# Genomics-HSE/VGsim

Measured on AMD Instinct MI355X. Metric: simulated events/sec (direct + tau-leap) at 1/2/4/8 MI355X vs Cython CPU, higher is better.
Workload: dtype f64; 1 GPU; BASELINE config 3: 65536 haplotypes (8 sites) x 64 populations x 1 susceptibility group, direct Gillespie, bit-exact mode (PCG64 stream, reference summation order), index-case start, b=2.5 d=0.9 s=0.1 m=0.01/site, total migration 0.01, N=1e7; replicates_per_gpu=16384, events_per_replicate=100000, trajectory_points=1001

## Files before the change

include/vgx.h:

```cpp
#ifndef VGX_H
#define VGX_H
#include <stdint.h>

#ifdef __cplusplus
extern "C" {
#endif

typedef struct vgx_engine vgx_engine;

enum {
    VGX_OK = 0,
    VGX_ERR_ARG = 1,
    VGX_ERR_HIP = 2,
    VGX_ERR_ZERO_WEIGHT = 3,
    VGX_ERR_CAPACITY = 4,
    VGX_ERR_LOOP_GUARD = 5,
    VGX_ERR_CLASSES = 6
};

enum { VGX_BIRTH = 0, VGX_DEATH = 1, VGX_SAMPLING = 2, VGX_MUTATION = 3, VGX_SUSCCHANGE = 4,
       VGX_MIGRATION = 5, VGX_MULTITYPE = 6 };

typedef struct vgx_dims {
    int64_t sites, hapNum, popNum, susNum;
} vgx_dims;

typedef struct vgx_params {
    const double *bRate, *dRate, *sRate;
    const double *mRate;
    const double *hapMutType;
    const double *susceptibility;
    const int64_t *suscType;
    const double *suscepTransition;
    const int64_t *sizes;
    const double *contactDensityBeforeLockdown;
    const double *contactDensityAfterLockdown;
    const double *startLD, *endLD;
    const double *samplingMultiplier;
    const double *migrationRates;
} vgx_params;

typedef struct vgx_state {
    int64_t *susceptible;
    int64_t *infectious;
    int64_t *initial_susceptible;
    int64_t *initial_infectious;
    int64_t *totalSusceptible, *totalInfectious, *lockdownON;
    double *contactDensity;
    int64_t first_simulation;
    int64_t globalInfectious;
    int64_t bCounter, dCounter, sCounter, mCounter, iCounter, swapLockdown, migPlus, migNonPlus;
    int64_t good_attempt;
    double currentTime, totalRate, totalMigrationRate, tau_l;
    int64_t ev_ptr, ev_size;
} vgx_state;

typedef struct vgx_run_opts {
    int64_t record_events;
    int64_t max_loop_factor;
    int64_t traj_points;
    double traj_t0, traj_t1;
    int64_t mode;
    int64_t kernel;
    int64_t reserved[2];
} vgx_run_opts;

typedef struct vgx_counters {
    int64_t ev_ptr;
    int64_t ev_first_new;
    int64_t loop_iterations;
    int64_t restarts;
    int64_t lockdown_records;
    int64_t error;
    int64_t multievent_rows;
    int64_t reserved[5];
} vgx_counters;

int vgx_create(const vgx_dims *dims, int64_t n_replicates, int device, vgx_engine **out);
void vgx_destroy(vgx_engine *e);
const char *vgx_last_error(const vgx_engine *e);
int vgx_device_count(void);

int vgx_set_params(vgx_engine *e, const vgx_params *p);
int vgx_set_recombination(vgx_engine *e, double recombination_probability, int64_t genome_length,
                          const int64_t *sitesPosition );
int vgx_set_state(vgx_engine *e, const vgx_state *s);
int vgx_get_state(vgx_engine *e, int64_t replicate, vgx_state *out);
int vgx_set_seeds(vgx_engine *e, const int64_t *seeds );

int vgx_stage_tau(vgx_engine *e);

int vgx_simulate_direct(vgx_engine *e, int64_t iterations, int64_t sample_size, float time, int64_t attempts,
                        const vgx_run_opts *opts );
int vgx_simulate_tau(vgx_engine *e, int64_t iterations, int64_t sample_size, float time, int64_t attempts,
                     const vgx_run_opts *opts );

int vgx_get_counters(vgx_engine *e, int64_t replicate, vgx_counters *out);
int vgx_get_counters_all(vgx_engine *e, int64_t *out);
int vgx_get_events(vgx_engine *e, int64_t replicate, int64_t first, int64_t count, double *times,
                   int64_t *types, int64_t *haplotypes, int64_t *populations, int64_t *newHaplotypes,
                   int64_t *newPopulations);
int vgx_get_lockdowns(vgx_engine *e, int64_t replicate, int64_t cap, int64_t *states, int64_t *populations,
                      double *times, int64_t *n);
int vgx_get_recombinations(vgx_engine *e, int64_t replicate, int64_t cap, int64_t *idevents, int64_t *his,
                           int64_t *hi2s, int64_t *nhis, int64_t *posRecombs, int64_t *n);
int vgx_get_tau_tries(vgx_engine *e, int64_t replicate, int64_t first, int64_t count, int32_t *out);
int vgx_get_multievents(vgx_engine *e, int64_t replicate, int64_t cap, int64_t *num, double *times, int64_t *types,
                        int64_t *haplotypes, int64_t *populations, int64_t *newHaplotypes,
                        int64_t *newPopulations, int64_t *n);
int vgx_get_multievents_all(vgx_engine *e, int64_t cap, int64_t *offsets, int64_t *rows, int64_t *steps);
int vgx_get_tau_states_all(vgx_engine *e, int64_t *infectious, int64_t *susceptible, int64_t *counters, double *times);
int vgx_get_trajectories(vgx_engine *e, double *out, int out_is_device);
int vgx_get_trajectories_int(vgx_engine *e, int32_t *out_device);
int64_t vgx_clock_mismatches(const vgx_engine *e);

typedef struct vgx_genealogy_io {
    int64_t popNum, hapNum;
    int64_t sCounter;
    int64_t ev_ptr;
    const double *ev_times;
    const int64_t *ev_types, *ev_haplotypes, *ev_populations, *ev_newHaplotypes, *ev_newPopulations;
    int64_t mev_rows;
    const int64_t *mev_num; const double *mev_times;
    const int64_t *mev_types, *mev_haplotypes, *mev_populations, *mev_newHaplotypes, *mev_newPopulations;
    int64_t *infectious;
    uint64_t rng_state[4];
    int64_t rng_has_uint32;
    uint64_t rng_uinteger;
    int64_t *tree, *tree_pop; double *times;
    int64_t mut_cap, mut_n; int64_t *mut_node, *mut_AS, *mut_DS, *mut_site; double *mut_time;
    int64_t mig_cap, mig_n; int64_t *mig_node, *mig_old, *mig_new; double *mig_time;
    int64_t nodes_used;
} vgx_genealogy_io;
int vgx_get_genealogy(vgx_genealogy_io *io, char *errbuf, int64_t errcap);
void vgx_rng_position(int64_t seed, int64_t attempt, int64_t draws, uint64_t out[4]);

typedef struct vgx_genealogies_io {
    int64_t n;
    const int64_t *replicates;
    const uint64_t *rng_state;
    int64_t *node_off, *mut_off, *mig_off;
    int64_t *tree, *tree_pop; double *times;
    int64_t *mut_node, *mut_AS, *mut_DS, *mut_site; double *mut_time;
    int64_t *mig_node, *mig_old, *mig_new; double *mig_time;
    int64_t *status, *status_arg, *nodes_used, *mut_n, *mig_n;
    uint64_t *rng_out;
    int64_t layout;
    int64_t passes;
    double ms[3];
} vgx_genealogies_io;
int vgx_get_genealogies(vgx_engine *e, vgx_genealogies_io *io);
int vgx_genealogy_message(int64_t status, int64_t arg, char *errbuf, int64_t errcap);
int vgx_test_genealogy_walk(vgx_genealogy_io *io, char *errbuf, int64_t errcap);

typedef struct vgx_tau_genealogy_prefix {
    int64_t ev_ptr;
    const double *ev_times;
    const int64_t *ev_types, *ev_haplotypes, *ev_populations, *ev_newHaplotypes, *ev_newPopulations;
    int64_t mev_rows;
    const int64_t *mev_num; const double *mev_times;
    const int64_t *mev_types, *mev_haplotypes, *mev_populations, *mev_newHaplotypes, *mev_newPopulations;
} vgx_tau_genealogy_prefix;
typedef struct vgx_tau_genealogies_io {
    int64_t n;
    const int64_t *replicates;
    const uint64_t *rng_state;
    int64_t *node_off, *mut_off, *mig_off;
    int64_t *tree, *tree_pop; double *times;
    int64_t *mut_node, *mut_AS, *mut_DS, *mut_site; double *mut_time;
    int64_t *mig_node, *mig_old, *mig_new; double *mig_time;
    int64_t *status, *status_arg, *nodes_used, *mut_n, *mig_n;
    uint64_t *rng_out;
    int64_t passes;
    double ms[3];
} vgx_tau_genealogies_io;
int vgx_get_tau_genealogies(vgx_engine *e, vgx_tau_genealogies_io *io, const vgx_tau_genealogy_prefix *prefix);
int vgx_test_tau_genealogy_walk(vgx_genealogy_io *io, int64_t sites, char *errbuf, int64_t errcap);
int vgx_test_hypergeometric(int on_device, int64_t good, int64_t bad, int64_t sample, int64_t n, uint64_t state[6], int64_t *out);

typedef struct vgx_timelines_io {
    int64_t n;
    const int64_t *replicates;
    int64_t step_num, semantics;
    int64_t n_inf; const int64_t *inf_pop, *inf_hap;
    int64_t n_sus; const int64_t *sus_pop, *sus_grp;
    double *time_points;
    double *inf_data, *inf_sample;
    double *sus_data;
    int64_t *last_point;
    int64_t loc_cap;
    int64_t *loc_n, *loc_state, *loc_pop;
    double *loc_time;
    int64_t passes;
    double ms[3];
} vgx_timelines_io;
int vgx_get_timelines(vgx_engine *e, vgx_timelines_io *io);
typedef struct vgx_timelines_chain {
    int64_t popNum, hapNum, susNum;
    int64_t ev_ptr;
    const double *ev_times;
    const int64_t *ev_types, *ev_haplotypes, *ev_populations, *ev_newHaplotypes, *ev_newPopulations;
    double currentTime;
    int64_t step_num, semantics;
    int64_t n_inf; const int64_t *inf_pop, *inf_hap, *inf_start;
    int64_t n_sus; const int64_t *sus_pop, *sus_grp, *sus_start;
    double *time_points;
    double *inf_data, *inf_sample;
    double *sus_data;
    int64_t last_point;
} vgx_timelines_chain;
int vgx_test_timelines(vgx_timelines_chain *io, char *errbuf, int64_t errcap);

typedef struct vgx_timelines_prefix {
    int64_t ev_ptr;
    const double *ev_times;
    const int64_t *ev_types, *ev_haplotypes, *ev_populations, *ev_newHaplotypes, *ev_newPopulations;
    int64_t mev_rows;
    const int64_t *mev_num, *mev_types, *mev_haplotypes, *mev_populations, *mev_newHaplotypes, *mev_newPopulations;
    int64_t loc_n;
    const int64_t *loc_state, *loc_pop; const double *loc_time;
} vgx_timelines_prefix;
int vgx_get_tau_timelines(vgx_engine *e, vgx_timelines_io *io, const vgx_timelines_prefix *prefix);
typedef struct vgx_tau_timelines_chain {
    vgx_timelines_chain chain;
    int64_t mev_rows;
    const int64_t *mev_num, *mev_types, *mev_haplotypes, *mev_populations, *mev_newHaplotypes, *mev_newPopulations;
} vgx_tau_timelines_chain;
int vgx_test_tau_timelines(vgx_tau_timelines_chain *io, char *errbuf, int64_t errcap);

typedef struct vgx_direct_shape {
    int64_t P, H, S, sites;
    int64_t R;
    int64_t C, CB;
    int64_t cap;
    int64_t n_seg, n_solo_seg;
    int64_t solo_npass0, solo_npass1;
    int64_t solo_ncls, solo_maxnnz;
    int64_t start_lone_rows;
    int64_t start_max_nocc;
    int64_t max_size;
    int64_t hosts_below_2p53;
    int64_t ld_possible;
    int64_t recomb;
    int64_t fresh_state;
    int64_t suscep_cumul0_zero;
    int64_t have_counts32;
    int64_t tot_sus_is_sus;
    int64_t no_lone, solo_general;
} vgx_direct_shape;
typedef struct vgx_direct_plan {
    int64_t kernel;
    int64_t mode;
    int64_t fast, philox;
    int64_t solo_mig_in_lds;
    int64_t solo_compact;
    int64_t lone_general;
    int64_t lone_lds_bytes;
    int64_t long_lists;
    int64_t leaves32;
    int64_t fallback_kernel, fallback_mode;
} vgx_direct_plan;
int vgx_test_direct_plan(const vgx_direct_shape *shape, const vgx_run_opts *opts, vgx_direct_plan *plan, char *errbuf, int64_t errcap);

double vgx_last_kernel_ms(const vgx_engine *e);
int vgx_last_direct_kernel(const vgx_engine *e);
int64_t vgx_last_kernel_launches(const vgx_engine *e);
int64_t vgx_device_bytes(const vgx_engine *e);
int vgx_get_profile(vgx_engine *e, int64_t replicate, int64_t *out16);
int vgx_get_list_counts_quad(vgx_engine *e, int64_t replicate, int64_t population, int64_t count, int32_t *out, int64_t *list_cap);

typedef struct vgx_rowscan {
    int64_t rows, H, S;
    const int64_t *infectious;
    const double *eventRates123;
    const int64_t *numToHap;
    const double *bRate;
    const double *susceptibility;
    const double *rowSusceptible;
    const double *rowContact;
    const double *u;
    double *birthRate, *tEvent, *hapPopRate;
    double *susceptHapPopRate;
    double *rowTotal;
    int64_t *chosen;
    double *rnOut;
} vgx_rowscan;
int vgx_propensity_scan(const vgx_rowscan *io);
int vgx_propensity_scan_bench(const vgx_rowscan *first_row, int64_t rows, int repeats, double *ms_update, double *ms_choose);
const char *vgx_propensity_scan_error(void);

int vgx_test_philox(int on_device, const uint32_t ctr[4], const uint32_t key[2], uint32_t out[4]);
int vgx_test_poisson(double lam, int64_t n, uint64_t seed, int64_t *out);

int vgx_test_div_by_const(const double *n, const double *b, int64_t count, double *q_seq, double *q_lean, double *q_div);

int vgx_test_row_scans(const double *w, const double *carry, int64_t rows, double *pre16, double *tot16, double *pre64);

#ifdef __cplusplus
}
#endif
#endif
```

vgsim_amd/_capi.py:

```python
import ctypes as C
import os

import numpy as np

HERE = os.path.dirname(os.path.abspath(__file__))
LIB_PATH = os.environ.get("VGX_LIBRARY", os.path.join(HERE, "libvgx.so"))

_F = C.POINTER(C.c_double)
_I = C.POINTER(C.c_int64)

VGX_OK = 0


class VgxDims(C.Structure):
    _fields_ = [("sites", C.c_int64), ("hapNum", C.c_int64), ("popNum", C.c_int64), ("susNum", C.c_int64)]


class VgxParams(C.Structure):
    _fields_ = [("bRate", _F), ("dRate", _F), ("sRate", _F), ("mRate", _F), ("hapMutType", _F),
                ("susceptibility", _F), ("suscType", _I), ("suscepTransition", _F), ("sizes", _I),
                ("contactDensityBeforeLockdown", _F), ("contactDensityAfterLockdown", _F), ("startLD", _F),
                ("endLD", _F), ("samplingMultiplier", _F), ("migrationRates", _F)]


class VgxState(C.Structure):
    _fields_ = [("susceptible", _I), ("infectious", _I), ("initial_susceptible", _I), ("initial_infectious", _I),
                ("totalSusceptible", _I), ("totalInfectious", _I), ("lockdownON", _I), ("contactDensity", _F),
                ("first_simulation", C.c_int64), ("globalInfectious", C.c_int64),
                ("bCounter", C.c_int64), ("dCounter", C.c_int64), ("sCounter", C.c_int64), ("mCounter", C.c_int64),
                ("iCounter", C.c_int64), ("swapLockdown", C.c_int64), ("migPlus", C.c_int64), ("migNonPlus", C.c_int64),
                ("good_attempt", C.c_int64),
                ("currentTime", C.c_double), ("totalRate", C.c_double), ("totalMigrationRate", C.c_double),
                ("tau_l", C.c_double), ("ev_ptr", C.c_int64), ("ev_size", C.c_int64)]


class VgxRunOpts(C.Structure):
    _fields_ = [("record_events", C.c_int64), ("max_loop_factor", C.c_int64), ("traj_points", C.c_int64),
                ("traj_t0", C.c_double), ("traj_t1", C.c_double), ("mode", C.c_int64), ("kernel", C.c_int64),
                ("reserved", C.c_int64 * 2)]


class VgxCounters(C.Structure):
    _fields_ = [("ev_ptr", C.c_int64), ("ev_first_new", C.c_int64), ("loop_iterations", C.c_int64),
                ("restarts", C.c_int64), ("lockdown_records", C.c_int64), ("error", C.c_int64),
                ("multievent_rows", C.c_int64), ("reserved", C.c_int64 * 5)]


class VgxGenealogyIO(C.Structure):
    _fields_ = [("popNum", C.c_int64), ("hapNum", C.c_int64), ("sCounter", C.c_int64), ("ev_ptr", C.c_int64),
                ("ev_times", _F), ("ev_types", _I), ("ev_haplotypes", _I), ("ev_populations", _I),
                ("ev_newHaplotypes", _I), ("ev_newPopulations", _I),
                ("mev_rows", C.c_int64), ("mev_num", _I), ("mev_times", _F), ("mev_types", _I), ("mev_haplotypes", _I),
                ("mev_populations", _I), ("mev_newHaplotypes", _I), ("mev_newPopulations", _I),
                ("infectious", _I), ("rng_state", C.c_uint64 * 4), ("rng_has_uint32", C.c_int64), ("rng_uinteger", C.c_uint64),
                ("tree", _I), ("tree_pop", _I), ("times", _F),
                ("mut_cap", C.c_int64), ("mut_n", C.c_int64), ("mut_node", _I), ("mut_AS", _I), ("mut_DS", _I),
                ("mut_site", _I), ("mut_time", _F),
                ("mig_cap", C.c_int64), ("mig_n", C.c_int64), ("mig_node", _I), ("mig_old", _I), ("mig_new", _I),
                ("mig_time", _F), ("nodes_used", C.c_int64)]


class VgxGenealogiesIO(C.Structure):
    _fields_ = [("n", C.c_int64), ("replicates", _I), ("rng_state", C.POINTER(C.c_uint64)),
                ("node_off", _I), ("mut_off", _I), ("mig_off", _I),
                ("tree", _I), ("tree_pop", _I), ("times", _F),
                ("mut_node", _I), ("mut_AS", _I), ("mut_DS", _I), ("mut_site", _I), ("mut_time", _F),
                ("mig_node", _I), ("mig_old", _I), ("mig_new", _I), ("mig_time", _F),
                ("status", _I), ("status_arg", _I), ("nodes_used", _I), ("mut_n", _I), ("mig_n", _I),
                ("rng_out", C.POINTER(C.c_uint64)), ("layout", C.c_int64), ("passes", C.c_int64), ("ms", C.c_double * 3)]


class VgxTauGenealogyPrefix(C.Structure):
    _fields_ = [("ev_ptr", C.c_int64), ("ev_times", _F), ("ev_types", _I), ("ev_haplotypes", _I), ("ev_populations", _I),
                ("ev_newHaplotypes", _I), ("ev_newPopulations", _I),
                ("mev_rows", C.c_int64), ("mev_num", _I), ("mev_times", _F), ("mev_types", _I), ("mev_haplotypes", _I),
                ("mev_populations", _I), ("mev_newHaplotypes", _I), ("mev_newPopulations", _I)]


class VgxTauGenealogiesIO(C.Structure):
    _fields_ = [("n", C.c_int64), ("replicates", _I), ("rng_state", C.POINTER(C.c_uint64)),
                ("node_off", _I), ("mut_off", _I), ("mig_off", _I),
                ("tree", _I), ("tree_pop", _I), ("times", _F),
                ("mut_node", _I), ("mut_AS", _I), ("mut_DS", _I), ("mut_site", _I), ("mut_time", _F),
                ("mig_node", _I), ("mig_old", _I), ("mig_new", _I), ("mig_time", _F),
                ("status", _I), ("status_arg", _I), ("nodes_used", _I), ("mut_n", _I), ("mig_n", _I),
                ("rng_out", C.POINTER(C.c_uint64)), ("passes", C.c_int64), ("ms", C.c_double * 3)]


TAU_STEP_ROWS_MAX = 8192
GW_STEP_ROWS = 10


class VgxTimelinesIO(C.Structure):
    _fields_ = [("n", C.c_int64), ("replicates", _I), ("step_num", C.c_int64), ("semantics", C.c_int64),
                ("n_inf", C.c_int64), ("inf_pop", _I), ("inf_hap", _I), ("n_sus", C.c_int64), ("sus_pop", _I), ("sus_grp", _I),
                ("time_points", _F), ("inf_data", _F), ("inf_sample", _F), ("sus_data", _F), ("last_point", _I),
                ("loc_cap", C.c_int64), ("loc_n", _I), ("loc_state", _I), ("loc_pop", _I), ("loc_time", _F),
                ("passes", C.c_int64), ("ms", C.c_double * 3)]


class VgxTimelinesChain(C.Structure):
    _fields_ = [("popNum", C.c_int64), ("hapNum", C.c_int64), ("susNum", C.c_int64), ("ev_ptr", C.c_int64),
                ("ev_times", _F), ("ev_types", _I), ("ev_haplotypes", _I), ("ev_populations", _I),
                ("ev_newHaplotypes", _I), ("ev_newPopulations", _I),
                ("currentTime", C.c_double), ("step_num", C.c_int64), ("semantics", C.c_int64),
                ("n_inf", C.c_int64), ("inf_pop", _I), ("inf_hap", _I), ("inf_start", _I),
                ("n_sus", C.c_int64), ("sus_pop", _I), ("sus_grp", _I), ("sus_start", _I),
                ("time_points", _F), ("inf_data", _F), ("inf_sample", _F), ("sus_data", _F), ("last_point", C.c_int64)]


class VgxTimelinesPrefix(C.Structure):
    _fields_ = [("ev_ptr", C.c_int64), ("ev_times", _F), ("ev_types", _I), ("ev_haplotypes", _I), ("ev_populations", _I),
                ("ev_newHaplotypes", _I), ("ev_newPopulations", _I),
                ("mev_rows", C.c_int64), ("mev_num", _I), ("mev_types", _I), ("mev_haplotypes", _I), ("mev_populations", _I),
                ("mev_newHaplotypes", _I), ("mev_newPopulations", _I),
                ("loc_n", C.c_int64), ("loc_state", _I), ("loc_pop", _I), ("loc_time", _F)]


class VgxTauTimelinesChain(C.Structure):
    _fields_ = [("chain", VgxTimelinesChain), ("mev_rows", C.c_int64), ("mev_num", _I), ("mev_types", _I), ("mev_haplotypes", _I),
                ("mev_populations", _I), ("mev_newHaplotypes", _I), ("mev_newPopulations", _I)]


TIMELINE_SEMANTICS = {'reference': 0, 'compartment': 1}


class VgxDirectShape(C.Structure):
    _fields_ = [(n, C.c_int64) for n in (
        "P", "H", "S", "sites", "R", "C", "CB", "cap", "n_seg", "n_solo_seg", "solo_npass0", "solo_npass1", "solo_ncls",
        "solo_maxnnz", "start_lone_rows", "start_max_nocc", "max_size", "hosts_below_2p53", "ld_possible", "recomb",
        "fresh_state", "suscep_cumul0_zero", "have_counts32", "tot_sus_is_sus", "no_lone", "solo_general")]


class VgxDirectPlan(C.Structure):
    _fields_ = [(n, C.c_int64) for n in (
        "kernel", "mode", "fast", "philox", "solo_mig_in_lds", "solo_compact", "lone_general", "lone_lds_bytes", "long_lists",
        "leaves32", "fallback_kernel", "fallback_mode")]


class VgxRowScan(C.Structure):
    _fields_ = [("rows", C.c_int64), ("H", C.c_int64), ("S", C.c_int64), ("infectious", _I), ("eventRates123", _F),
                ("numToHap", _I), ("bRate", _F), ("susceptibility", _F), ("rowSusceptible", _F), ("rowContact", _F), ("u", _F),
                ("birthRate", _F), ("tEvent", _F), ("hapPopRate", _F), ("susceptHapPopRate", _F), ("rowTotal", _F),
                ("chosen", _I), ("rnOut", _F)]


_H = C.c_void_p
SIGNATURES = {
    "vgx_create": (C.c_int, [C.POINTER(VgxDims), C.c_int64, C.c_int, C.POINTER(_H)]),
    "vgx_destroy": (None, [_H]),
    "vgx_last_error": (C.c_char_p, [_H]),
    "vgx_device_count": (C.c_int, []),
    "vgx_set_params": (C.c_int, [_H, C.POINTER(VgxParams)]),
    "vgx_set_recombination": (C.c_int, [_H, C.c_double, C.c_int64, _I]),
    "vgx_get_recombinations": (C.c_int, [_H, C.c_int64, C.c_int64, _I, _I, _I, _I, _I, _I]),
    "vgx_set_state": (C.c_int, [_H, C.POINTER(VgxState)]),
    "vgx_get_state": (C.c_int, [_H, C.c_int64, C.POINTER(VgxState)]),
    "vgx_set_seeds": (C.c_int, [_H, _I]),
    "vgx_stage_tau": (C.c_int, [_H]),
    "vgx_simulate_direct": (C.c_int, [_H, C.c_int64, C.c_int64, C.c_float, C.c_int64, C.POINTER(VgxRunOpts)]),
    "vgx_simulate_tau": (C.c_int, [_H, C.c_int64, C.c_int64, C.c_float, C.c_int64, C.POINTER(VgxRunOpts)]),
    "vgx_get_counters": (C.c_int, [_H, C.c_int64, C.POINTER(VgxCounters)]),
    "vgx_get_counters_all": (C.c_int, [_H, _I]),
    "vgx_get_events": (C.c_int, [_H, C.c_int64, C.c_int64, C.c_int64, _F, _I, _I, _I, _I, _I]),
    "vgx_get_lockdowns": (C.c_int, [_H, C.c_int64, C.c_int64, _I, _I, _F, _I]),
    "vgx_get_tau_tries": (C.c_int, [_H, C.c_int64, C.c_int64, C.c_int64, C.POINTER(C.c_int32)]),
    "vgx_get_multievents": (C.c_int, [_H, C.c_int64, C.c_int64, _I, _F, _I, _I, _I, _I, _I, _I]),
    "vgx_get_multievents_all": (C.c_int, [_H, C.c_int64, _I, _I, _I]),
    "vgx_get_tau_states_all": (C.c_int, [_H, _I, _I, _I, _F]),
    "vgx_get_trajectories": (C.c_int, [_H, C.c_void_p, C.c_int]),
    "vgx_get_trajectories_int": (C.c_int, [_H, C.c_void_p]),
    "vgx_clock_mismatches": (C.c_int64, [_H]),
    "vgx_last_kernel_ms": (C.c_double, [_H]),
    "vgx_last_kernel_launches": (C.c_int64, [_H]),
    "vgx_last_direct_kernel": (C.c_int, [_H]),
    "vgx_device_bytes": (C.c_int64, [_H]),
    "vgx_get_profile": (C.c_int, [_H, C.c_int64, _I]),
    "vgx_get_list_counts_quad": (C.c_int, [_H, C.c_int64, C.c_int64, C.c_int64, C.POINTER(C.c_int32), _I]),
    "vgx_get_genealogy": (C.c_int, [C.POINTER(VgxGenealogyIO), C.c_char_p, C.c_int64]),
    "vgx_get_genealogies": (C.c_int, [_H, C.POINTER(VgxGenealogiesIO)]),
    "vgx_genealogy_message": (C.c_int, [C.c_int64, C.c_int64, C.c_char_p, C.c_int64]),
    "vgx_test_genealogy_walk": (C.c_int, [C.POINTER(VgxGenealogyIO), C.c_char_p, C.c_int64]),
    "vgx_get_tau_genealogies": (C.c_int, [_H, C.POINTER(VgxTauGenealogiesIO), C.POINTER(VgxTauGenealogyPrefix)]),
    "vgx_test_tau_genealogy_walk": (C.c_int, [C.POINTER(VgxGenealogyIO), C.c_int64, C.c_char_p, C.c_int64]),
    "vgx_test_hypergeometric": (C.c_int, [C.c_int, C.c_int64, C.c_int64, C.c_int64, C.c_int64, C.POINTER(C.c_uint64 * 6), _I]),
    "vgx_get_timelines": (C.c_int, [_H, C.POINTER(VgxTimelinesIO)]),
    "vgx_test_timelines": (C.c_int, [C.POINTER(VgxTimelinesChain), C.c_char_p, C.c_int64]),
    "vgx_get_tau_timelines": (C.c_int, [_H, C.POINTER(VgxTimelinesIO), C.POINTER(VgxTimelinesPrefix)]),
    "vgx_test_tau_timelines": (C.c_int, [C.POINTER(VgxTauTimelinesChain), C.c_char_p, C.c_int64]),
    "vgx_test_direct_plan": (C.c_int, [C.POINTER(VgxDirectShape), C.POINTER(VgxRunOpts), C.POINTER(VgxDirectPlan), C.c_char_p, C.c_int64]),
    "vgx_rng_position": (None, [C.c_int64, C.c_int64, C.c_int64, C.POINTER(C.c_uint64 * 4)]),
    "vgx_propensity_scan": (C.c_int, [C.POINTER(VgxRowScan)]),
    "vgx_propensity_scan_bench": (C.c_int, [C.POINTER(VgxRowScan), C.c_int64, C.c_int, C.POINTER(C.c_double), C.POINTER(C.c_double)]),
    "vgx_propensity_scan_error": (C.c_char_p, []),
    "vgx_test_philox": (C.c_int, [C.c_int, C.POINTER(C.c_uint32 * 4), C.POINTER(C.c_uint32 * 2), C.POINTER(C.c_uint32 * 4)]),
    "vgx_test_poisson": (C.c_int, [C.c_double, C.c_int64, C.c_uint64, _I]),
    "vgx_test_div_by_const": (C.c_int, [_F, _F, C.c_int64, _F, _F, _F]),
    "vgx_test_row_scans": (C.c_int, [_F, _F, C.c_int64, _F, _F, _F]),
}

_lib = None


def load_library():
    global _lib
    if _lib is None:
        if not os.path.exists(LIB_PATH):
            raise RuntimeError(
                "vgsim_amd: the HIP extension %s is not built (run `python -c 'import __graft_entry__ as g; g.build()'` "
                "or `make -C vgsim_amd/csrc`). There is no CPU fallback." % LIB_PATH)
        lib = C.CDLL(LIB_PATH)
        for name, (res, args) in SIGNATURES.items():
            fn = getattr(lib, name)
            fn.restype = res
            fn.argtypes = args
        _lib = lib
    return _lib


def _p(a):
    if a is None:
        return None
    assert a.flags["C_CONTIGUOUS"]
    if a.dtype == np.float64:
        return a.ctypes.data_as(_F)
    if a.dtype == np.int64:
        return a.ctypes.data_as(_I)
    raise TypeError(a.dtype)


class VgxError(RuntimeError):
    def __init__(self, code, msg):
        super().__init__("libvgx error %d: %s" % (code, msg))
        self.code = code


class HipEngine:

    def __init__(self, sites, hapNum, popNum, susNum, n_replicates=1, device=0):
        self.lib = load_library()
        self.dims = VgxDims(sites, hapNum, popNum, susNum)
        self.R = int(n_replicates)
        self.handle = _H()
        rc = self.lib.vgx_create(C.byref(self.dims), self.R, int(device), C.byref(self.handle))
        if rc != VGX_OK:
            self.handle = None
            raise VgxError(rc, self.lib.vgx_last_error(None).decode())
        self.P, self.H, self.S = popNum, hapNum, susNum

    def close(self):
        if getattr(self, "handle", None):
            self.lib.vgx_destroy(self.handle)
            self.handle = None

    def __del__(self):
        try:
            self.close()
        except Exception:
            pass

    def _check(self, rc):
        if rc != VGX_OK:
            raise VgxError(rc, self.lib.vgx_last_error(self.handle).decode())

    def set_params(self, m):
        p = VgxParams()
        conv = []
        for name, ctype in VgxParams._fields_:
            a = np.ascontiguousarray(getattr(m, name), dtype=np.int64 if ctype is _I else np.float64)
            conv.append(a)
            setattr(p, name, _p(a))
        self._keep = conv
        self._check(self.lib.vgx_set_params(self.handle, C.byref(p)))
        pos = np.ascontiguousarray(getattr(m, "sitesPosition", np.zeros(0)), dtype=np.int64)
        self._check(self.lib.vgx_set_recombination(self.handle, float(getattr(m, "recombination", 0.0)),
                                                   int(getattr(m, "genome_length", 0)), _p(pos) if len(pos) else None))

    def recombinations(self, replicate=0):
        n = C.c_int64(0)
        self._check(self.lib.vgx_get_recombinations(self.handle, replicate, 0, None, None, None, None, None, C.byref(n)))
        cols = [np.zeros(n.value, dtype=np.int64) for _ in range(5)]
        if n.value:
            self._check(self.lib.vgx_get_recombinations(self.handle, replicate, n.value, *[_p(c) for c in cols], C.byref(n)))
        return cols

    def _state_struct(self, m):
        s = VgxState()
        for name in ("susceptible", "infectious", "initial_susceptible", "initial_infectious", "totalSusceptible",
                     "totalInfectious", "lockdownON", "contactDensity"):
            setattr(s, name, _p(getattr(m, name)))
        return s

    def set_state(self, m):
        s = self._state_struct(m)
        s.first_simulation = int(m.first_simulation)
        s.globalInfectious = int(m.globalInfectious)
        for c in m.COUNTERS + ("good_attempt",):
            setattr(s, c, int(getattr(m, c)))
        s.currentTime, s.totalRate, s.totalMigrationRate, s.tau_l = m.currentTime, m.totalRate, m.totalMigrationRate, m.tau_l
        s.ev_ptr, s.ev_size = m.events.ptr, m.events.size
        self._snapshot_call = not bool(m.first_simulation)
        self._check(self.lib.vgx_set_state(self.handle, C.byref(s)))

    def get_state(self, m, replicate=0):
        s = self._state_struct(m)
        if not getattr(self, "_snapshot_call", True):
            s.initial_susceptible = None
            s.initial_infectious = None
        self._check(self.lib.vgx_get_state(self.handle, replicate, C.byref(s)))
        m.first_simulation = bool(s.first_simulation)
        m.globalInfectious = s.globalInfectious
        for c in m.COUNTERS + ("good_attempt",):
            setattr(m, c, getattr(s, c))
        m.currentTime, m.totalRate, m.totalMigrationRate, m.tau_l = s.currentTime, s.totalRate, s.totalMigrationRate, s.tau_l

    def stage_tau(self):
        self._check(self.lib.vgx_stage_tau(self.handle))

    def set_seeds(self, seeds):
        a = np.ascontiguousarray(np.asarray(seeds, dtype=np.int64))
        assert a.shape == (self.R,)
        self._check(self.lib.vgx_set_seeds(self.handle, _p(a)))

    def counters(self, replicate=0):
        c = VgxCounters()
        self._check(self.lib.vgx_get_counters(self.handle, replicate, C.byref(c)))
        return c

    def fetch_events(self, events, replicate, first, count):
        if count <= 0:
            return
        sl = slice(first, first + count)
        bufs = [np.zeros(count, dtype=np.float64)] + [np.zeros(count, dtype=np.int64) for _ in range(5)]
        self._check(self.lib.vgx_get_events(self.handle, replicate, first, count, *[_p(b) for b in bufs]))
        events.times[sl] = bufs[0]
        for name, b in zip(events.COLUMNS, bufs[1:]):
            getattr(events, name)[sl] = b

    def lockdowns(self, replicate=0, cap=4096):
        st, pp = np.zeros(cap, dtype=np.int64), np.zeros(cap, dtype=np.int64)
        tt = np.zeros(cap, dtype=np.float64)
        n = C.c_int64(0)
        self._check(self.lib.vgx_get_lockdowns(self.handle, replicate, cap, _p(st), _p(pp), _p(tt), C.byref(n)))
        k = min(n.value, cap)
        return st[:k], pp[:k], tt[:k]

    def simulate_direct(self, m, iterations, sample_size, time, attempts, opts=None):
        self.set_params(m)
        self.set_state(m)
        self.set_seeds([m.user_seed] * self.R)
        rc = self.lib.vgx_simulate_direct(self.handle, iterations, sample_size, float(time), attempts,
                                          C.byref(opts) if opts is not None else None)
        self._check(rc)
        self._absorb(m)

    def simulate_tau(self, m, iterations, sample_size, time, attempts, opts=None):
        self.set_params(m)
        self.set_state(m)
        self.set_seeds([m.user_seed] * self.R)
        rc = self.lib.vgx_simulate_tau(self.handle, iterations, sample_size, float(time), attempts,
                                       C.byref(opts) if opts is not None else None)
        self._check(rc)
        mev_base = m.multievents.ptr
        self._absorb(m, tau=True, mev_base=mev_base)

    def multievents(self, replicate=0):
        n = C.c_int64(0)
        self._check(self.lib.vgx_get_multievents(self.handle, replicate, 0, None, None, None, None, None, None, None, C.byref(n)))
        k = n.value
        cols = {name: np.zeros(k, dtype=np.int64) for name in ("num", "types", "haplotypes", "populations", "newHaplotypes", "newPopulations")}
        times = np.zeros(k, dtype=np.float64)
        if k:
            self._check(self.lib.vgx_get_multievents(self.handle, replicate, k, _p(cols["num"]), _p(times), _p(cols["types"]),
                                                     _p(cols["haplotypes"]), _p(cols["populations"]), _p(cols["newHaplotypes"]),
                                                     _p(cols["newPopulations"]), C.byref(n)))
        cols["times"] = times
        return cols

    def multievents_all(self):
        off = np.zeros(self.R + 1, dtype=np.int64)
        self._check(self.lib.vgx_get_multievents_all(self.handle, 0, _p(off), None, None))
        n = int(off[-1])
        rows = np.zeros((max(n, 1), 6), dtype=np.int64)
        steps = np.zeros(max(n, 1), dtype=np.int64)
        if n:
            self._check(self.lib.vgx_get_multievents_all(self.handle, n, _p(off), _p(rows), _p(steps)))
        cols = {name: np.ascontiguousarray(rows[:n, j]) for j, name in enumerate(("num", "types", "haplotypes", "populations", "newHaplotypes", "newPopulations"))}
        cols["steps"] = steps[:n]
        return off, cols

    def tau_states_all(self):
        inf = np.zeros((self.R, self.P, self.H), dtype=np.int64)
        sus = np.zeros((self.R, self.P, self.S), dtype=np.int64)
        cnt = np.zeros((self.R, 8), dtype=np.int64)
        t = np.zeros(self.R, dtype=np.float64)
        self._check(self.lib.vgx_get_tau_states_all(self.handle, _p(inf), _p(sus), _p(cnt), _p(t)))
        return inf, sus, cnt, t

    def counters_all(self):
        out = np.zeros((self.R, 4), dtype=np.int64)
        self._check(self.lib.vgx_get_counters_all(self.handle, _p(out)))
        return out

    def _absorb(self, m, replicate=0, tau=False, mev_base=0):
        self.get_state(m, replicate)
        c = self.counters(replicate)
        first = c.ev_first_new
        self.fetch_events(m.events, replicate, first, c.ev_ptr - first)
        m.events.ptr = c.ev_ptr
        if tau:
            rows = self.multievents(replicate)
            if len(rows["times"]) == 0:
                m.events.haplotypes[first:c.ev_ptr] = 0
                m.events.populations[first:c.ev_ptr] = 0
            rows = canonical_multievents(rows, m.events.haplotypes[first:c.ev_ptr], m.events.populations[first:c.ev_ptr],
                                         m.sites, m.susNum)
            if c.restarts > 0:
                m.multievents.ptr = 0
                mev_base = 0
            m.events.haplotypes[first:c.ev_ptr] += mev_base
            m.events.populations[first:c.ev_ptr] += mev_base
            m.multievents.extend(rows.pop("times"), **rows)
            self.last_events_drawn = c.reserved[0]
        st, pp, tt = self.lockdowns(replicate)
        for k in range(len(st)):
            m.loc.AddLockdown(st[k], pp[k], tt[k])
        if not tau and getattr(m, "recombination", 0.0) and hasattr(m, "rec"):
            for row in zip(*self.recombinations(replicate)):
                m.rec.AddRecombination_forward(*row)
        self.last_counters = c

    def tau_tries(self, replicate, first, count):
        out = np.zeros(count, dtype=np.int32)
        self._check(self.lib.vgx_get_tau_tries(self.handle, replicate, first, count, out.ctypes.data_as(C.POINTER(C.c_int32))))
        return out

    @property
    def last_kernel_ms(self):
        return self.lib.vgx_last_kernel_ms(self.handle)

    @property
    def last_kernel(self):
        return {1: "wave", 2: "lane", 3: "quad", 4: "quadg", 5: "solo", 6: "lone"}[self.lib.vgx_last_direct_kernel(self.handle)]

    @property
    def device_bytes(self):
        return self.lib.vgx_device_bytes(self.handle)


def canonical_multievents(rows, starts, ends, sites, susNum):
    n = len(rows["times"])
    if n == 0:
        return rows
    num, typ, hap = rows["num"], rows["types"], rows["haplotypes"]
    pop, nh, npop = rows["populations"], rows["newHaplotypes"], rows["newPopulations"]
    step = np.searchsorted(np.asarray(ends), np.arange(n), side="right")
    mig = typ == 5
    k1 = np.where(mig, 0, 1)
    k2 = pop.copy()
    k3 = np.where(mig, npop, np.where(typ == 4, 0, 1))
    k4 = np.where(mig, nh, hap)
    k5 = np.zeros(n, dtype=np.int64)
    k5[mig] = hap[mig]
    k5[typ == 4] = nh[typ == 4]
    k5[typ == 1] = 0
    k5[typ == 2] = 1
    mu = typ == 3
    if mu.any():
        d = np.abs(nh[mu] - hap[mu])
        low = np.zeros(d.shape, dtype=np.int64)
        t = d.copy()
        while (t >= 4).any():
            big = t >= 4
            t[big] //= 4
            low[big] += 1
        digit4 = 4 ** low
        AS, DS = (hap[mu] // digit4) % 4, (nh[mu] // digit4) % 4
        k5[mu] = 2 + (sites - 1 - low) * 3 + np.where(DS > AS, DS - 1, DS)
    k5[typ == 0] = 2 + 3 * sites + nh[typ == 0]
    order = np.lexsort((k5, k4, k3, k2, k1, step))
    key = np.stack([step, k1, k2, k3, k4, k5])[:, order]
    first = np.ones(n, dtype=bool)
    first[1:] = (key[:, 1:] != key[:, :-1]).any(axis=0)
    idx = np.nonzero(first)[0]
    out = {c: rows[c][order][idx] for c in ("types", "haplotypes", "populations", "newHaplotypes", "newPopulations")}
    out["num"] = np.add.reduceat(num[order], idx)
    out["times"] = rows["times"][order][idx]
    per_step = np.bincount(key[0, idx], minlength=len(starts))
    e = np.cumsum(per_step)
    starts[:] = e - per_step
    ends[:] = e
    return out


def get_genealogy(m, seed=None, rng_position=None, rng_raw=None):
    return _genealogy("vgx_get_genealogy", m, seed, rng_position, rng_raw)


def genealogy_walk(m, seed=None, rng_position=None, rng_raw=None):
    return _genealogy("vgx_test_genealogy_walk", m, seed, rng_position, rng_raw)

# ... 194 lines not shown
```

vgsim_amd/csrc/vgx_api.hip:

```cpp
#include "vgx_engine.h"
#include "vgx_rng.h"

static std::string g_create_error;

extern "C" int vgx_device_count(void) {
    int n = 0;
    if (hipGetDeviceCount(&n) != hipSuccess) return 0;
    return n;
}

extern "C" int vgx_create(const vgx_dims *dims, int64_t n_replicates, int device, vgx_engine **out) {
    if (!dims || !out || n_replicates < 1) { g_create_error = "vgx_create: bad argument"; return VGX_ERR_ARG; }
    int64_t h = 1;
    for (int64_t s = 0; s < dims->sites; s++) h *= 4;
    if (dims->sites < 0 || dims->sites > 15 || dims->hapNum != h || dims->popNum < 1 || dims->susNum < 1) {
        g_create_error = "vgx_create: hapNum must equal 4^sites (sites <= 15), popNum >= 1, susNum >= 1";
        return VGX_ERR_ARG;
    }
    int n = 0;
    hipError_t he = hipGetDeviceCount(&n);
    if (he != hipSuccess || n == 0) {
        g_create_error = std::string("vgx_create: no HIP device available (") + hipGetErrorString(he) +
                         "); this engine has no CPU fallback";
        return VGX_ERR_HIP;
// ... 611 lines not shown
        for (int64_t i = 0; i < count; i++) {
            const auto &st = lg[(size_t)(i0 + i)];
            if (times) times[i] = st.time;
            if (types) types[i] = VGX_MULTITYPE;
            if (haplotypes) haplotypes[i] = st.m0;
            if (populations) populations[i] = st.m1;
            if (newHaplotypes) newHaplotypes[i] = 0;
            if (newPopulations) newPopulations[i] = 0;
        }
        return VGX_OK;
    }
    int64_t slot0 = first - e->ev_base;
    if (slot0 < 0 || slot0 + count > e->evcap) return fail(e, VGX_ERR_ARG, "vgx_get_events: range outside the device log of the last call");
    if (!e->call_recorded) return fail(e, VGX_ERR_ARG, "vgx_get_events: the last call did not record events");
    std::vector<int32_t> cols((size_t)count * VGX_EV_COLS);
    HIPCHECK(e, hipMemcpy(cols.data(), (int32_t *)e->r_evcols.p + (replicate * e->evcap + slot0) * VGX_EV_COLS,
                          (size_t)count * VGX_EV_COLS * 4, hipMemcpyDeviceToHost));
    if (times) {
        int rc = host_clock(e, replicate);
        if (rc) return rc;
        const int64_t i0 = first - e->hc.e0;
        if (i0 < 0 || i0 + count > (int64_t)e->hc.times.size())
            return fail(e, VGX_ERR_ARG, "vgx_get_events: times exist for the events of the last call only");
        memcpy(times, e->hc.times.data() + i0, (size_t)count * 8);
    }
    int64_t *dst[5] = {types, haplotypes, populations, newHaplotypes, newPopulations};
    for (int c = 0; c < 5; c++)
        if (dst[c])
            for (int64_t i = 0; i < count; i++) dst[c][i] = cols[(size_t)(i * VGX_EV_COLS + c)];
    return VGX_OK;
}

extern "C" int vgx_get_tau_tries(vgx_engine *e, int64_t replicate, int64_t first, int64_t count, int32_t *out) {
    if (!e || !out || replicate < 0 || replicate >= e->R || first < 0 || count < 0) return VGX_ERR_ARG;
    if (!e->last_was_tau || (size_t)replicate >= e->tau_log.size()) return fail(e, VGX_ERR_ARG, "vgx_get_tau_tries: the last call was not vgx_simulate_tau");
    const auto &lg = e->tau_log[(size_t)replicate];
    if (first + count > (int64_t)lg.size()) return fail(e, VGX_ERR_ARG, "vgx_get_tau_tries: the last call made fewer steps");
    for (int64_t i = 0; i < count; i++) out[i] = lg[(size_t)(first + i)].tries;
    return VGX_OK;
}

extern "C" int vgx_get_lockdowns(vgx_engine *e, int64_t replicate, int64_t cap, int64_t *states, int64_t *populations,
                                 double *times, int64_t *n) {
    if (!e || !n || replicate < 0 || replicate >= e->R) return VGX_ERR_ARG;
    if (!e->sc_host_valid) return fail(e, VGX_ERR_ARG, "vgx_get_lockdowns: no simulate call yet");
    HIPCHECK(e, hipSetDevice(e->device));
    if (e->last_was_tau) {
        const auto &tt = e->tau_loc_time[(size_t)replicate];
        *n = (int64_t)tt.size();
        for (int64_t i = 0; i < std::min<int64_t>(*n, cap); i++) {
            if (states) states[i] = e->tau_loc_state[(size_t)replicate][(size_t)i];
            if (populations) populations[i] = e->tau_loc_pop[(size_t)replicate][(size_t)i];
            if (times) times[i] = tt[(size_t)i];
        }
        return VGX_OK;
    }
    int64_t cnt = std::min<int64_t>(e->sc_host[(size_t)replicate].loc_n, e->loc_cap);
    *n = cnt;
    cnt = std::min(cnt, cap);
    if (cnt <= 0) return VGX_OK;
    std::vector<int32_t> rec((size_t)cnt * 2);
    HIPCHECK(e, hipMemcpy(rec.data(), (int32_t *)e->r_locrec.p + replicate * e->loc_cap * 2, (size_t)cnt * 8, hipMemcpyDeviceToHost));
    int rch = host_clock(e, replicate);
    if (rch) return rch;
    const std::vector<double> &tt = e->hc.loc_times;
    for (int64_t i = 0; i < cnt; i++) {
        if (states) states[i] = rec[(size_t)(i * 2)];
        if (populations) populations[i] = rec[(size_t)(i * 2 + 1)];
        if (times) times[i] = tt[(size_t)i];
    }
    return VGX_OK;
}

extern "C" int vgx_get_multievents(vgx_engine *e, int64_t replicate, int64_t cap, int64_t *num, double *times,
                                   int64_t *types, int64_t *haplotypes, int64_t *populations, int64_t *newHaplotypes,
                                   int64_t *newPopulations, int64_t *n) {
    if (!e || !n || replicate < 0 || replicate >= e->R) return VGX_ERR_ARG;
    *n = 0;
    if (!e->last_was_tau) return VGX_OK;
    HIPCHECK(e, hipSetDevice(e->device));
    const auto &lg = e->tau_log[(size_t)replicate];
    int64_t rows = (lg.empty() || e->tau_mev_cap <= 0) ? 0 : lg.back().m1;
    *n = rows;
    rows = std::min(rows, cap);
    if (rows <= 0) return VGX_OK;
    const int64_t mev_cap = e->tau_mev_cap;
    if (mev_cap <= 0) return VGX_OK;
    std::vector<int64_t> buf((size_t)rows * 6);
    HIPCHECK(e, hipMemcpy(buf.data(), (int64_t *)e->t_mev.p + replicate * mev_cap * 6, (size_t)rows * 48, hipMemcpyDeviceToHost));
    size_t st = 0;
    for (int64_t i = 0; i < rows; i++) {
        while (st + 1 < lg.size() && i >= lg[st].m1) st++;
        if (num) num[i] = buf[(size_t)(i * 6)];
        if (times) times[i] = lg[st].time;
        if (types) types[i] = buf[(size_t)(i * 6 + 1)];
        if (haplotypes) haplotypes[i] = buf[(size_t)(i * 6 + 2)];
        if (populations) populations[i] = buf[(size_t)(i * 6 + 3)];
        if (newHaplotypes) newHaplotypes[i] = buf[(size_t)(i * 6 + 4)];
        if (newPopulations) newPopulations[i] = buf[(size_t)(i * 6 + 5)];
    }
    return VGX_OK;
}

extern "C" int vgx_get_multievents_all(vgx_engine *e, int64_t cap, int64_t *offsets , int64_t *rows ,
                                       int64_t *steps ) {
    if (!e || !offsets || cap < 0) return VGX_ERR_ARG;
    const int64_t R = e->R;
    for (int64_t r = 0; r <= R; r++) offsets[r] = 0;
    if (!e->last_was_tau || e->tau_mev_cap <= 0 || (int64_t)e->tau_log.size() < R) return VGX_OK;
    int64_t most = 0;
    for (int64_t r = 0; r < R; r++) {
        const auto &lg = e->tau_log[(size_t)r];
        const int64_t n = lg.empty() ? 0 : lg.back().m1;
        offsets[r + 1] = offsets[r] + n;
        most = std::max(most, n);
    }
    if (!rows) return VGX_OK;
    if (cap < offsets[R]) return fail(e, VGX_ERR_ARG, "vgx_get_multievents_all: room for fewer rows than the call recorded");
    if (most == 0) return VGX_OK;
    HIPCHECK(e, hipSetDevice(e->device));
    const int64_t mev_cap = e->tau_mev_cap;
    if (most > mev_cap) return fail(e, VGX_ERR_ARG, "vgx_get_multievents_all: a replicate logged more rows than its block holds");
    const int64_t batch = std::max<int64_t>(1, std::min<int64_t>(R, ((int64_t)1 << 28) / (most * 48)));
    std::vector<int64_t> buf((size_t)(batch * most * 6));
    for (int64_t r0 = 0; r0 < R; r0 += batch) {
        const int64_t nr = std::min(batch, R - r0);
        HIPCHECK(e, hipMemcpy2D(buf.data(), (size_t)most * 48, (int64_t *)e->t_mev.p + r0 * mev_cap * 6, (size_t)mev_cap * 48, (size_t)most * 48,
                                (size_t)nr, hipMemcpyDeviceToHost));
        for (int64_t r = r0; r < r0 + nr; r++) {
            const int64_t n = offsets[r + 1] - offsets[r];
            if (n <= 0) continue;
            memcpy(rows + offsets[r] * 6, buf.data() + (r - r0) * most * 6, (size_t)n * 48);
            if (steps) {
                const auto &lg = e->tau_log[(size_t)r];
                size_t st = 0;
                for (int64_t i = 0; i < n; i++) {
                    while (st + 1 < lg.size() && i >= lg[st].m1) st++;
                    steps[offsets[r] + i] = (int64_t)st;
                }
            }
        }
    }
    return VGX_OK;
}

extern "C" int vgx_get_tau_states_all(vgx_engine *e, int64_t *infectious , int64_t *susceptible ,
                                      int64_t *counters , double *times ) {
    if (!e) return VGX_ERR_ARG;
    if (!e->last_was_tau || !e->sc_host_valid) return fail(e, VGX_ERR_ARG, "vgx_get_tau_states_all: the last call was not vgx_simulate_tau");
    HIPCHECK(e, hipSetDevice(e->device));
    const int64_t R = e->R, H = e->d.hapNum, P = e->d.popNum, S = e->d.susNum;
    if (susceptible) HIPCHECK(e, hipMemcpy(susceptible, e->t_S.p, (size_t)(R * P * S) * 8, hipMemcpyDeviceToHost));
    if (infectious) {
        const int64_t n = R * P * H, part = std::min<int64_t>(n, (int64_t)1 << 26);
        std::unique_ptr<int32_t[]> inf32(new int32_t[(size_t)part]);
        for (int64_t i0 = 0; i0 < n; i0 += part) {
            const int64_t k = std::min(part, n - i0);
            HIPCHECK(e, hipMemcpy(inf32.get(), (int32_t *)e->t_I.p + i0, (size_t)k * 4, hipMemcpyDeviceToHost));
            for (int64_t i = 0; i < k; i++) infectious[i0 + i] = inf32[(size_t)i];
        }
    }
    for (int64_t r = 0; r < R; r++) {
        const VgxRepScalars &s = e->sc_host[(size_t)r];
        if (counters) {
            int64_t *c = counters + r * 8;
            c[0] = s.bCounter; c[1] = s.dCounter; c[2] = s.sCounter; c[3] = s.mCounter; c[4] = s.iCounter; c[5] = s.migPlus;
            c[6] = s.globalInfectious; c[7] = s.ev_ptr;
        }
        if (times) times[r] = s.currentTime;
    }
    return VGX_OK;
}

extern "C" int vgx_get_trajectories(vgx_engine *e, double *out, int out_is_device) {
    if (!e || !out) return VGX_ERR_ARG;
    if (e->traj_points <= 0) return fail(e, VGX_ERR_ARG, "vgx_get_trajectories: the last call recorded none");
    HIPCHECK(e, hipSetDevice(e->device));
    size_t bytes = (size_t)(e->R * e->traj_points * e->d.popNum * 2) * 8;
    HIPCHECK(e, hipMemcpy(out, e->r_traj.p, bytes, out_is_device ? hipMemcpyDeviceToDevice : hipMemcpyDeviceToHost));
    return VGX_OK;
}

extern "C" hipError_t vgxi_launch_traj_i32(const double *src, int32_t *dst, int64_t n, hipStream_t stream);
extern "C" int vgx_get_trajectories_int(vgx_engine *e, int32_t *out_device) {
    if (!e || !out_device) return VGX_ERR_ARG;
    if (e->traj_points <= 0) return fail(e, VGX_ERR_ARG, "vgx_get_trajectories_int: the last call recorded none");
    for (int64_t pn = 0; pn < e->d.popNum; pn++)
        if (e->sizes[(size_t)pn] >= ((int64_t)1 << 31)) return fail(e, VGX_ERR_ARG, "vgx_get_trajectories_int: population sizes of 2^31 or more");
    HIPCHECK(e, hipSetDevice(e->device));
    HIPCHECK(e, vgxi_launch_traj_i32((const double *)e->r_traj.p, out_device, e->R * e->traj_points * e->d.popNum * 2, e->stream));
    HIPCHECK(e, hipStreamSynchronize(e->stream));
    return VGX_OK;
}

extern "C" int64_t vgx_clock_mismatches(const vgx_engine *e) { return e ? e->clock_mismatches : 0; }

extern "C" int vgx_get_state(vgx_engine *e, int64_t replicate, vgx_state *out) {
    if (!e || !out || replicate < 0 || replicate >= e->R) return VGX_ERR_ARG;
    if (e->last_was_tau && e->sc_host_valid) {
        HIPCHECK(e, hipSetDevice(e->device));
        const int64_t H = e->d.hapNum, P = e->d.popNum, S = e->d.susNum;
        const VgxRepScalars &s = e->sc_host[(size_t)replicate];
        HostState &h = e->hs;
        if (out->susceptible) HIPCHECK(e, hipMemcpy(out->susceptible, (int64_t *)e->t_S.p + replicate * P * S, (size_t)(P * S) * 8, hipMemcpyDeviceToHost));
        if (out->infectious) {
            std::unique_ptr<int32_t[]> inf32(new int32_t[(size_t)(P * H)]);
            HIPCHECK(e, hipMemcpy(inf32.get(), (int32_t *)e->t_I.p + replicate * P * H, (size_t)(P * H) * 4, hipMemcpyDeviceToHost));
            int64_t *dst = out->infectious;
            const int32_t *src = inf32.get();
            for_parts(P * H, [&](int64_t b0, int64_t en, unsigned) { for (int64_t i = b0; i < en; i++) dst[i] = src[i]; });
        }
        if (out->initial_susceptible) memcpy(out->initial_susceptible, h.initial_susceptible.data(), (size_t)(P * S) * 8);
        if (out->initial_infectious) memcpy(out->initial_infectious, h.initial_infectious.data(), (size_t)(P * H) * 8);
        std::vector<int64_t> tot((size_t)P);
        std::vector<double> cd((size_t)P);
        std::vector<int32_t> lk((size_t)P);
        HIPCHECK(e, hipMemcpy(tot.data(), (int64_t *)e->t_totInf.p + replicate * P, (size_t)P * 8, hipMemcpyDeviceToHost));
        HIPCHECK(e, hipMemcpy(cd.data(), (double *)e->t_cd.p + replicate * P, (size_t)P * 8, hipMemcpyDeviceToHost));
        HIPCHECK(e, hipMemcpy(lk.data(), (int32_t *)e->t_lock.p + replicate * P, (size_t)P * 4, hipMemcpyDeviceToHost));
        std::vector<int64_t> sus((size_t)(P * S));
        HIPCHECK(e, hipMemcpy(sus.data(), (int64_t *)e->t_S.p + replicate * P * S, (size_t)(P * S) * 8, hipMemcpyDeviceToHost));
        for (int64_t pn = 0; pn < P; pn++) {
            if (out->totalInfectious) out->totalInfectious[pn] = tot[(size_t)pn];
            if (out->totalSusceptible) {
                int64_t t = 0;
                for (int64_t sn = 0; sn < S; sn++) t += sus[(size_t)(pn * S + sn)];
                out->totalSusceptible[pn] = t;
            }
            if (out->lockdownON) out->lockdownON[pn] = lk[(size_t)pn];
            if (out->contactDensity) out->contactDensity[pn] = cd[(size_t)pn];
        }
        out->first_simulation = h.first_simulation;
        out->globalInfectious = s.globalInfectious;
        out->bCounter = s.bCounter; out->dCounter = s.dCounter; out->sCounter = s.sCounter; out->mCounter = s.mCounter;
        out->iCounter = s.iCounter; out->swapLockdown = s.swapLockdown; out->migPlus = s.migPlus;
        out->migNonPlus = s.migNonPlus; out->good_attempt = s.good_attempt;
        out->currentTime = s.currentTime; out->totalRate = s.totalRate; out->totalMigrationRate = s.totalMig;
        out->tau_l = s.tau_l;
        out->ev_ptr = s.ev_ptr; out->ev_size = e->last_ev_size;
        return VGX_OK;
    }
    if (!e->dev_state_valid || !e->sc_host_valid) return fail(e, VGX_ERR_ARG, "vgx_get_state: no device state");
    HIPCHECK(e, hipSetDevice(e->device));
    const int64_t H = e->d.hapNum, P = e->d.popNum, S = e->d.susNum, cap = e->cap;
    const VgxRepScalars &s = e->sc_host[(size_t)replicate];
    std::vector<int64_t> popI((size_t)(PI_COUNT * P));
    std::vector<double> popD((size_t)(PD_COUNT * P));
    HIPCHECK(e, hipMemcpy(popI.data(), (int64_t *)e->r_popI.p + replicate * PI_COUNT * P, popI.size() * 8, hipMemcpyDeviceToHost));
    HIPCHECK(e, hipMemcpy(popD.data(), (double *)e->r_popD.p + replicate * PD_COUNT * P, popD.size() * 8, hipMemcpyDeviceToHost));
    if (out->susceptible)
        HIPCHECK(e, hipMemcpy(out->susceptible, (int64_t *)e->r_sus.p + replicate * P * S, (size_t)(P * S) * 8, hipMemcpyDeviceToHost));
    if (out->infectious) {
        if (!e->counts64_valid) {
            HIPCHECK(e, vgxi_launch_counts64(e->dr.lcnt32, e->dr.lcnt, e->R * P * cap, e->stream));
            HIPCHECK(e, hipStreamSynchronize(e->stream));
            e->counts64_valid = true;
        }
        std::vector<int32_t> nocc((size_t)P);
        HIPCHECK(e, hipMemcpy(nocc.data(), (int32_t *)e->r_nocc.p + replicate * P, (size_t)P * 4, hipMemcpyDeviceToHost));
        memset(out->infectious, 0, (size_t)(P * H) * 8);
        std::vector<int32_t> hap;
        std::vector<int64_t> cnt;
        for (int64_t pn = 0; pn < P; pn++) {
            int64_t n = nocc[(size_t)pn];
            if (n <= 0) continue;
            hap.resize((size_t)n);
            cnt.resize((size_t)n);
            HIPCHECK(e, hipMemcpy(hap.data(), (int32_t *)e->r_lhap.p + (replicate * P + pn) * cap, (size_t)n * 4, hipMemcpyDeviceToHost));
            HIPCHECK(e, hipMemcpy(cnt.data(), (int64_t *)e->r_lcnt.p + (replicate * P + pn) * cap, (size_t)n * 8, hipMemcpyDeviceToHost));
            for (int64_t k = 0; k < n; k++) out->infectious[pn * H + hap[(size_t)k]] = cnt[(size_t)k];
        }
    }
    HostState &h = e->hs;
    if (out->initial_susceptible) memcpy(out->initial_susceptible, h.initial_susceptible.data(), (size_t)(P * S) * 8);
    if (out->initial_infectious) memcpy(out->initial_infectious, h.initial_infectious.data(), (size_t)(P * H) * 8);
    for (int64_t pn = 0; pn < P; pn++) {
        if (out->totalSusceptible) out->totalSusceptible[pn] = popI[(size_t)(PI_TOTSUS * P + pn)];
        if (out->totalInfectious) out->totalInfectious[pn] = popI[(size_t)(PI_TOTINF * P + pn)];
        if (out->lockdownON) out->lockdownON[pn] = popI[(size_t)(PI_LOCK * P + pn)];
        if (out->contactDensity) out->contactDensity[pn] = popD[(size_t)(PD_CD * P + pn)];
    }
    out->first_simulation = h.first_simulation;
    out->globalInfectious = s.globalInfectious;
    out->bCounter = s.bCounter; out->dCounter = s.dCounter; out->sCounter = s.sCounter; out->mCounter = s.mCounter;
    out->iCounter = s.iCounter; out->swapLockdown = s.swapLockdown; out->migPlus = s.migPlus;
    out->migNonPlus = s.migNonPlus; out->good_attempt = s.good_attempt;
    {
        int rch = host_clock(e, replicate);
        if (rch) return rch;
    }
    out->currentTime = e->hc.final_time; out->totalRate = s.totalRate; out->totalMigrationRate = s.totalMig;
    out->tau_l = s.tau_l;
    out->ev_ptr = s.ev_ptr; out->ev_size = e->last_ev_size;
    return VGX_OK;
}

extern "C" int vgx_get_list_counts_quad(vgx_engine *e, int64_t replicate, int64_t population, int64_t count, int32_t *out, int64_t *list_cap) {
    if (!e || replicate < 0 || replicate >= e->R || population < 0 || population >= e->d.popNum || count < 0) return VGX_ERR_ARG;
    if (list_cap) *list_cap = e->dev_state_valid ? e->cap : 0;
    if (count == 0) return VGX_OK;
    if (!out || !e->dev_state_valid || !e->counts32_valid || !e->dr.lcnt32 || count > e->cap) return VGX_ERR_ARG;
    HIPCHECK(e, hipSetDevice(e->device));
    HIPCHECK(e, hipMemcpy(out, e->dr.lcnt32 + (replicate * e->d.popNum + population) * e->cap, (size_t)count * 4, hipMemcpyDeviceToHost));
    return VGX_OK;
}

extern "C" int vgx_get_profile(vgx_engine *e, int64_t replicate, int64_t *out16) {
    if (!e || !out16 || replicate < 0 || replicate >= e->R || !e->r_prof.p) return VGX_ERR_ARG;
    HIPCHECK(e, hipSetDevice(e->device));
    HIPCHECK(e, hipMemcpy(out16, (unsigned long long *)e->r_prof.p + replicate * VGX_PROF_SLOTS, VGX_PROF_SLOTS * 8, hipMemcpyDeviceToHost));
    return VGX_OK;
}

extern "C" int vgx_get_genealogies(vgx_engine *e, vgx_genealogies_io *io) {
    if (!e || !io || io->n < 0 || (io->n > 0 && (!io->replicates || !io->node_off || !io->mut_off || !io->mig_off)))
        return VGX_ERR_ARG;
    const auto t_call = std::chrono::steady_clock::now();
    io->passes = 0;
    io->ms[0] = io->ms[1] = io->ms[2] = 0.0;
    if (!e->sc_host_valid || !e->dev_state_valid) return fail(e, VGX_ERR_ARG, "vgx_get_genealogies: no direct simulate call yet");
    if (e->last_was_tau) return fail(e, VGX_ERR_ARG, "vgx_get_genealogies: the last call was vgx_simulate_tau (direct chains only)");
    if (!e->call_recorded) return fail(e, VGX_ERR_ARG, "vgx_get_genealogies: the last call did not record events");
    const int64_t n = io->n, P = e->d.popNum, H = e->d.hapNum;
    std::vector<int64_t> n_ev((size_t)n), sC((size_t)n);
    for (int64_t i = 0; i < n; i++) {
        const int64_t r = io->replicates[i];
        if (r < 0 || r >= e->R) return fail(e, VGX_ERR_ARG, "vgx_get_genealogies: replicate index out of range");
        const VgxRepScalars &s = e->sc_host[(size_t)r];
        const int64_t first = s.restarts > 0 ? 0 : ((size_t)r < e->call_ev0.size() ? e->call_ev0[(size_t)r] : e->ev_ptr0);
        if (first != 0 || e->ev_base != 0)
            return fail(e, VGX_ERR_ARG, "vgx_get_genealogies: the chain of replicate " + std::to_string(r) +
                                            " does not start in the last call's device log (events.ptr was not 0 at its start)");
        if (s.ev_ptr < 0 || s.ev_ptr > e->evcap || s.ev_ptr >= ((int64_t)1 << 30))
            return fail(e, VGX_ERR_ARG, "vgx_get_genealogies: event range of replicate " + std::to_string(r) + " outside the device log");
        n_ev[(size_t)i] = s.ev_ptr;
        sC[(size_t)i] = s.sCounter;
    }
    if (n == 0) return VGX_OK;
    HIPCHECK(e, hipSetDevice(e->device));
    const int32_t *log = (const int32_t *)e->r_evcols.p;

    if (!io->tree) {
        int64_t *d_rep = nullptr, *d_n = nullptr, *d_out = nullptr;
        std::vector<int64_t> cnt((size_t)n * 2);
        hipError_t er = hipMalloc(&d_rep, (size_t)n * 8 * 4);
        if (er != hipSuccess) return fail(e, VGX_ERR_HIP, std::string("vgx_get_genealogies: hipMalloc: ") + hipGetErrorString(er));
        d_n = d_rep + n;
        d_out = d_rep + 2 * n;
        er = hipMemcpy(d_rep, io->replicates, (size_t)n * 8, hipMemcpyHostToDevice);
        if (er == hipSuccess) er = hipMemcpy(d_n, n_ev.data(), (size_t)n * 8, hipMemcpyHostToDevice);
        if (er == hipSuccess) er = vgxi_gw_count(log, e->evcap, d_rep, d_n, n, d_out, e->stream);
        if (er == hipSuccess) er = hipStreamSynchronize(e->stream);
        if (er == hipSuccess) er = hipMemcpy(cnt.data(), d_out, (size_t)n * 16, hipMemcpyDeviceToHost);
        (void)hipFree(d_rep);
        if (er != hipSuccess) return fail(e, VGX_ERR_HIP, std::string("vgx_get_genealogies: counting pass: ") + hipGetErrorString(er));
        io->node_off[0] = io->mut_off[0] = io->mig_off[0] = 0;
        for (int64_t i = 0; i < n; i++) {
            const int64_t nodes = sC[(size_t)i] >= 2 ? 2 * sC[(size_t)i] - 1 : 0;
            io->node_off[i + 1] = io->node_off[i] + nodes;
            io->mut_off[i + 1] = io->mut_off[i] + cnt[(size_t)(2 * i)];
            io->mig_off[i + 1] = io->mig_off[i] + cnt[(size_t)(2 * i + 1)] + nodes;
        }
        io->ms[2] = std::chrono::duration<double, std::milli>(std::chrono::steady_clock::now() - t_call).count();
        return VGX_OK;
    }

    if (!io->rng_state || !io->tree_pop || !io->times || !io->status || !io->status_arg || !io->nodes_used || !io->mut_n || !io->mig_n ||
        !io->rng_out || (io->mut_off[n] > 0 && (!io->mut_node || !io->mut_AS || !io->mut_DS || !io->mut_site || !io->mut_time)) ||
        (io->mig_off[n] > 0 && (!io->mig_node || !io->mig_old || !io->mig_new || !io->mig_time)))
        return fail(e, VGX_ERR_ARG, "vgx_get_genealogies: null output");
    for (int64_t i = 0; i < n; i++) {
        const int64_t nodes = sC[(size_t)i] >= 2 ? 2 * sC[(size_t)i] - 1 : 0;
        if (io->node_off[i + 1] - io->node_off[i] < nodes || io->mut_off[i + 1] < io->mut_off[i] || io->mig_off[i + 1] < io->mig_off[i])
            return fail(e, VGX_ERR_ARG, "vgx_get_genealogies: output capacities smaller than the sizing call gave");
    }
    if (!e->counts64_valid) {
        HIPCHECK(e, vgxi_launch_counts64(e->dr.lcnt32, e->dr.lcnt, e->R * P * e->cap, e->stream));
        HIPCHECK(e, hipStreamSynchronize(e->stream));
        e->counts64_valid = true;
    }
    std::vector<VgxGwDesc> desc((size_t)n);
    std::vector<int64_t> bytes((size_t)n);
    for (int64_t i = 0; i < n; i++) {
        VgxGwDesc &d = desc[(size_t)i];
        d.rep = io->replicates[i];
        d.n_ev = n_ev[(size_t)i];
        d.sCounter = sC[(size_t)i];
        d.tsize = d.sCounter >= 2 ? vgx_gw_table_size(d.n_ev, P * H) : 0;
        d.arena_cap = d.sCounter >= 2 ? d.n_ev : 0;
        d.mut_cap = io->mut_off[i + 1] - io->mut_off[i];
        d.mig_cap = io->mig_off[i + 1] - io->mig_off[i];
        for (int k = 0; k < 4; k++) d.rng[k] = io->rng_state[i * 4 + k];
        const int64_t nodes = d.sCounter >= 2 ? 2 * d.sCounter - 1 : 0;
        bytes[(size_t)i] = d.tsize * 28 + d.arena_cap * 4 + nodes * 12 + d.mut_cap * 20 + d.mig_cap * 16 + (int64_t)sizeof(VgxGwDesc) + 72;
    }
    size_t free_b = 0, total_b = 0;
    HIPCHECK(e, hipMemGetInfo(&free_b, &total_b));
    int64_t share = (int64_t)(free_b / 2);
    if (const char *cb = getenv("VGX_GENEALOGY_CHUNK_BYTES")) share = std::min<int64_t>(share, std::max<int64_t>(atoll(cb), 1));
    const bool wave = io->layout == 1;
    std::vector<int64_t> mism((size_t)n, 0);
    int64_t i0 = 0;
    while (i0 < n) {
        int64_t i1 = i0, sum = 0;
        while (i1 < n && (i1 == i0 || sum + bytes[(size_t)i1] <= share)) sum += bytes[(size_t)i1++];
        const int64_t m = i1 - i0;
        int64_t T = 0, A = 0, N = 0, M = 0, G = 0;
        std::vector<VgxGwDesc> dp(desc.begin() + i0, desc.begin() + i1);
        for (int64_t j = 0; j < m; j++) {
            VgxGwDesc &d = dp[(size_t)j];
            d.tab_off = T; d.arena_off = A; d.node_off = N; d.mut_off = M; d.mig_off = G;
            T += d.tsize; A += d.arena_cap; N += d.sCounter >= 2 ? 2 * d.sCounter - 1 : 0; M += d.mut_cap; G += d.mig_cap;
        }
        auto up8 = [](int64_t b) { return (b + 255) / 256 * 256; };
        const int64_t o_desc = 0, o_res = o_desc + up8(m * (int64_t)sizeof(VgxGwDesc)), o_rng = o_res + up8(m * 40),
                      o_key = o_rng + up8(m * 32), o_cnt = o_key + up8(T * 8), o_base = o_cnt + up8(T * 8), o_len = o_base + up8(T * 4),
                      o_lcap = o_len + up8(T * 4), o_arena = o_lcap + up8(T * 4), o_out = o_arena + up8(A * 4),
                      out_bytes = up8((3 * N + 5 * M + 4 * G) * 4), total = o_out + out_bytes;
        char *ws = nullptr;
        hipError_t er = hipMalloc((void **)&ws, (size_t)total);
        if (er != hipSuccess)
            return fail(e, VGX_ERR_HIP, "vgx_get_genealogies: hipMalloc of " + std::to_string(total) + " bytes: " + hipGetErrorString(er));
        std::unique_ptr<char, void (*)(char *)> hold(ws, [](char *p) { (void)hipFree(p); });
        VgxGwLaunch a{};
        a.n = m;
        a.desc = (const VgxGwDesc *)(ws + o_desc);
        a.log = log; a.evcap = e->evcap;
        a.nocc = e->dr.nocc; a.lhap = e->dr.lhap; a.lcnt = e->dr.lcnt;
        a.P = P; a.H = H; a.cap = e->cap;
        a.key = (int64_t *)(ws + o_key); a.cnt = (int64_t *)(ws + o_cnt);
        a.base = (int32_t *)(ws + o_base); a.len = (int32_t *)(ws + o_len); a.lcap = (int32_t *)(ws + o_lcap);
        a.arena = (int32_t *)(ws + o_arena);
        int32_t *o32 = (int32_t *)(ws + o_out);
        a.tree = o32; a.tree_pop = o32 + N; a.node_ev = o32 + 2 * N;
        int32_t *mu = o32 + 3 * N;
        a.mut_node = mu; a.mut_AS = mu + M; a.mut_DS = mu + 2 * M; a.mut_site = mu + 3 * M; a.mut_ev = mu + 4 * M;
        int32_t *mg = mu + 5 * M;
        a.mig_node = mg; a.mig_old = mg + G; a.mig_new = mg + 2 * G; a.mig_ev = mg + 3 * G;
        a.res = (int64_t *)(ws + o_res);
        a.rng_out = (uint64_t *)(ws + o_rng);
        HIPCHECK(e, hipMemcpyAsync(ws + o_desc, dp.data(), (size_t)m * sizeof(VgxGwDesc), hipMemcpyHostToDevice, e->stream));
        if (T > 0) HIPCHECK(e, hipMemsetAsync(a.key, 0xFF, (size_t)T * 8, e->stream));
        HIPCHECK(e, hipEventRecord(e->ev0, e->stream));
        HIPCHECK(e, vgxi_gw_walk(&a, wave ? 1 : 0, e->stream));
        HIPCHECK(e, hipEventRecord(e->ev1, e->stream));
        if ((er = hipStreamSynchronize(e->stream)) != hipSuccess)
            return fail(e, VGX_ERR_HIP, std::string("vgx_get_genealogies: walk kernel failed: ") + hipGetErrorString(er));
        float kms = 0.f;
        HIPCHECK(e, hipEventElapsedTime(&kms, e->ev0, e->ev1));
        io->ms[0] += kms;
        std::vector<int64_t> res((size_t)m * 5);
        std::vector<uint64_t> rng((size_t)m * 4);
        std::vector<int32_t> out((size_t)(3 * N + 5 * M + 4 * G));
        HIPCHECK(e, hipMemcpy(res.data(), a.res, (size_t)m * 40, hipMemcpyDeviceToHost));
        HIPCHECK(e, hipMemcpy(rng.data(), a.rng_out, (size_t)m * 32, hipMemcpyDeviceToHost));
        if (!out.empty()) HIPCHECK(e, hipMemcpy(out.data(), o32, out.size() * 4, hipMemcpyDeviceToHost));
        hold.reset();
        const auto t_clock = std::chrono::steady_clock::now();
        const int32_t *h_tree = out.data(), *h_pop = h_tree + N, *h_nev = h_tree + 2 * N, *h_mu = h_tree + 3 * N, *h_mg = h_mu + 5 * M;
        std::vector<std::string> errs((size_t)m);
        std::vector<int> rcs((size_t)m, 0);
        int64_t work = 0;
        for (int64_t j = 0; j < m; j++) work += dp[(size_t)j].n_ev;
        for_parts(m, [&](int64_t j0, int64_t j1, unsigned) {
            if (hipSetDevice(e->device) != hipSuccess) { for (int64_t j = j0; j < j1; j++) { rcs[(size_t)j] = VGX_ERR_HIP; errs[(size_t)j] = "hipSetDevice"; } return; }
            vgx_engine::HostClock hc;
            for (int64_t j = j0; j < j1; j++) {
                const VgxGwDesc &d = dp[(size_t)j];
                const int64_t gi = i0 + j;
                int rc = clock_build(e, d.rep, hc, errs[(size_t)j]);
                if (rc) { rcs[(size_t)j] = rc; continue; }
                mism[(size_t)gi] = hc.limit_mismatch ? 1 : 0;
                const int64_t *r5 = res.data() + j * 5;
                io->status[gi] = r5[0]; io->status_arg[gi] = r5[1]; io->nodes_used[gi] = r5[2];
                io->mut_n[gi] = r5[0] == VGX_GW_OK ? r5[3] : 0;
                io->mig_n[gi] = r5[0] == VGX_GW_OK ? r5[4] : 0;
                for (int k = 0; k < 4; k++) io->rng_out[gi * 4 + k] = rng[(size_t)(j * 4 + k)];
                if (r5[0] != VGX_GW_OK) continue;
                auto time_of = [&](int32_t ev, double &t) {
                    if (ev < 0) { t = 0.0; return true; }
                    const int64_t k = (int64_t)ev - hc.e0;
                    if (k < 0 || k >= (int64_t)hc.times.size()) return false;
                    t = hc.times[(size_t)k];
                    return true;
                };
                bool ok = true;
                const int64_t nodes = 2 * d.sCounter - 1, no = io->node_off[gi];
                for (int64_t k = 0; k < nodes; k++) {
                    io->tree[no + k] = h_tree[d.node_off + k];
                    io->tree_pop[no + k] = h_pop[d.node_off + k];
                    ok &= time_of(h_nev[d.node_off + k], io->times[no + k]);
                }
                const int64_t mo = io->mut_off[gi];
                for (int64_t k = 0; k < r5[3]; k++) {
                    const int64_t q = d.mut_off + k;
                    io->mut_node[mo + k] = h_mu[q]; io->mut_AS[mo + k] = h_mu[M + q]; io->mut_DS[mo + k] = h_mu[2 * M + q];
                    io->mut_site[mo + k] = h_mu[3 * M + q];
                    ok &= time_of(h_mu[4 * M + q], io->mut_time[mo + k]);
                }
                const int64_t go = io->mig_off[gi];
                for (int64_t k = 0; k < r5[4]; k++) {
                    const int64_t q = d.mig_off + k;
                    io->mig_node[go + k] = h_mg[q]; io->mig_old[go + k] = h_mg[G + q]; io->mig_new[go + k] = h_mg[2 * G + q];
                    ok &= time_of(h_mg[3 * G + q], io->mig_time[go + k]);
                }
                if (!ok) { rcs[(size_t)j] = VGX_ERR_ARG; errs[(size_t)j] = "vgx_get_genealogies: an event index outside the host clock's range"; }
            }
        }, std::max<int64_t>(work / std::max<int64_t>(m, 1), 1) * 64);
        for (int64_t j = 0; j < m; j++)
            if (rcs[(size_t)j]) return fail(e, rcs[(size_t)j], errs[(size_t)j]);
        io->ms[1] += std::chrono::duration<double, std::milli>(std::chrono::steady_clock::now() - t_clock).count();
        io->passes += 1;
        i0 = i1;
    }
    for (int64_t i = 0; i < n; i++) e->clock_mismatches += mism[(size_t)i];
    io->ms[2] = std::chrono::duration<double, std::milli>(std::chrono::steady_clock::now() - t_call).count();
    return VGX_OK;
}

extern "C" int vgx_get_timelines(vgx_engine *e, vgx_timelines_io *io) {
    if (!e || !io || io->n < 0 || (io->n > 0 && !io->replicates) || io->n_inf < 0 || io->n_sus < 0) return VGX_ERR_ARG;
    const auto t_call = std::chrono::steady_clock::now();
    io->passes = 0;
    io->ms[0] = io->ms[1] = io->ms[2] = 0.0;
    if (!e->sc_host_valid || !e->dev_state_valid) return fail(e, VGX_ERR_ARG, "vgx_get_timelines: needs a direct vgx_simulate_direct call with the event log first");
    if (e->last_was_tau) return fail(e, VGX_ERR_ARG, "vgx_get_timelines: the last call was vgx_simulate_tau (replays direct chains only)");
    if (!e->call_recorded) return fail(e, VGX_ERR_ARG, "vgx_get_timelines: the last call did not record events");
    const int64_t n = io->n, P = e->d.popNum, H = e->d.hapNum, S = e->d.susNum, step = io->step_num, T = step + 1;
    const int64_t n_inf = io->n_inf, n_sus = io->n_sus;
    if (step < 1) return fail(e, VGX_ERR_ARG, "vgx_get_timelines: step_num must be at least 1");
    if (io->semantics != VGX_TL_REFERENCE && io->semantics != VGX_TL_COMPARTMENT)
        return fail(e, VGX_ERR_ARG, "vgx_get_timelines: semantics must be 0 (reference) or 1 (compartment)");
    if ((n_inf > 0 && (!io->inf_pop || !io->inf_hap)) || (n_sus > 0 && (!io->sus_pop || !io->sus_grp)) || n_inf + n_sus >= ((int64_t)1 << 20))
        return fail(e, VGX_ERR_ARG, "vgx_get_timelines: bad query list");
    {
        std::vector<std::pair<int64_t, int64_t>> qi, qs;
        for (int64_t k = 0; k < n_inf; k++) {
            if (io->inf_pop[k] < 0 || io->inf_pop[k] >= P) return fail(e, VGX_ERR_ARG, "vgx_get_timelines: population index out of range");
            if (io->inf_hap[k] < 0 || io->inf_hap[k] >= H) return fail(e, VGX_ERR_ARG, "vgx_get_timelines: haplotype index out of range");
            qi.emplace_back(io->inf_pop[k], io->inf_hap[k]);
        }
        for (int64_t k = 0; k < n_sus; k++) {
            if (io->sus_pop[k] < 0 || io->sus_pop[k] >= P) return fail(e, VGX_ERR_ARG, "vgx_get_timelines: population index out of range");
            if (io->sus_grp[k] < 0 || io->sus_grp[k] >= S) return fail(e, VGX_ERR_ARG, "vgx_get_timelines: susceptibility group index out of range");
            qs.emplace_back(io->sus_pop[k], io->sus_grp[k]);
        }
        std::sort(qi.begin(), qi.end());
        std::sort(qs.begin(), qs.end());
        if (std::adjacent_find(qi.begin(), qi.end()) != qi.end() || std::adjacent_find(qs.begin(), qs.end()) != qs.end())
            return fail(e, VGX_ERR_ARG, "vgx_get_timelines: a query is given twice");
    }
    std::vector<int32_t> n_ev((size_t)n);
    int64_t loc_need = 1;
    {
        std::vector<char> seen((size_t)e->R, 0);
        for (int64_t i = 0; i < n; i++) {
            const int64_t r = io->replicates[i];
            if (r < 0 || r >= e->R) return fail(e, VGX_ERR_ARG, "vgx_get_timelines: replicate index out of range");
            if (seen[(size_t)r]) return fail(e, VGX_ERR_ARG, "vgx_get_timelines: replicates must be distinct");
            seen[(size_t)r] = 1;
            const VgxRepScalars &s = e->sc_host[(size_t)r];
            const int64_t first = s.restarts > 0 ? 0 : ((size_t)r < e->call_ev0.size() ? e->call_ev0[(size_t)r] : e->ev_ptr0);
            if (first != 0 || e->ev_base != 0)
                return fail(e, VGX_ERR_ARG, "vgx_get_timelines: replicate " + std::to_string(r) + ": its chain does not start in the last call's device log (the model held " +
                                                std::to_string(e->ev_base != 0 ? e->ev_base : first) + " events when the ensemble started)");
            if (s.ev_ptr < 0 || s.ev_ptr > e->evcap || s.ev_ptr >= ((int64_t)1 << 30))
                return fail(e, VGX_ERR_ARG, "vgx_get_timelines: event range of replicate " + std::to_string(r) + " outside the device log");
            n_ev[(size_t)i] = (int32_t)s.ev_ptr;
            loc_need = std::max(loc_need, std::min<int64_t>(s.loc_n, e->loc_cap));
        }
    }
    if (!io->time_points) {
        io->loc_cap = loc_need;
        io->ms[2] = std::chrono::duration<double, std::milli>(std::chrono::steady_clock::now() - t_call).count();
        return VGX_OK;
    }
    if (n == 0) {
        io->ms[2] = std::chrono::duration<double, std::milli>(std::chrono::steady_clock::now() - t_call).count();
        return VGX_OK;
    }
    if (!io->last_point || !io->loc_n || !io->loc_state || !io->loc_pop || !io->loc_time || (n_inf > 0 && (!io->inf_data || !io->inf_sample)) ||
        (n_sus > 0 && !io->sus_data))
        return fail(e, VGX_ERR_ARG, "vgx_get_timelines: null output");
    if (io->loc_cap < loc_need) return fail(e, VGX_ERR_ARG, "vgx_get_timelines: loc_cap smaller than the sizing call gave");
    const int64_t loc_cap = io->loc_cap;

    int64_t budget = VGX_TL_LDS_DEFAULT;
    if (const char *lb = getenv("VGX_TIMELINES_LDS_BYTES")) budget = std::min<int64_t>(std::max<int64_t>(atoll(lb), 1), VGX_TL_LDS_MAX);
    const int64_t need1 = std::max(n_inf > 0 ? vgx_tl_lds_bytes(step, 1, 0) : 0, n_sus > 0 ? vgx_tl_lds_bytes(step, 0, 1) : vgx_tl_lds_bytes(step, 0, 0));
    if (need1 > VGX_TL_LDS_MAX)
        return fail(e, VGX_ERR_ARG, "vgx_get_timelines: step_num " + std::to_string(step) + " is too large: the counters of one query exceed a workgroup's LDS");
    budget = std::max(budget, need1);
    struct Group { int64_t i0, ni, s0, ns, tab_off, start_off; };
    std::vector<Group> groups;
    std::vector<int32_t> h_tab;
    std::vector<int64_t> h_start;
    for (int64_t i = 0, s = 0; i < n_inf || s < n_sus;) {
        Group g{i, 0, s, 0, (int64_t)h_tab.size(), (int64_t)h_start.size()};
        while (i + g.ni < n_inf && vgx_tl_lds_bytes(step, g.ni + 1, g.ns) <= budget) g.ni++;
        while (s + g.ns < n_sus && vgx_tl_lds_bytes(step, g.ni, g.ns + 1) <= budget) g.ns++;
        const int ts = vgx_tl_table_size((int)(g.ni + g.ns));
        h_tab.resize(h_tab.size() + (size_t)(3 * ts), -1);
        int32_t *tab = h_tab.data() + g.tab_off;
        for (int64_t k = 0; k < g.ni; k++) {
            vgx_tl_insert(tab, ts, 0, (int32_t)io->inf_pop[i + k], (int32_t)io->inf_hap[i + k], (int32_t)k);
            h_start.push_back(e->hs.initial_infectious[(size_t)(io->inf_pop[i + k] * H + io->inf_hap[i + k])]);
// ... 152 lines not shown
```

vgsim_amd/csrc/vgx_direct_run.hip:

```cpp
#include "vgx_engine.h"

#define DIRECT_TRY(call) do { const int rc__ = (call); if (rc__) return rc__; } while (0)


static bool one_class(int64_t P, int64_t S, int64_t C, int64_t CB) { return P <= 64 && S == 1 && C == 1 && CB == 1; }
static bool one_class_shape(const vgx_direct_shape *s) { return one_class(s->P, s->S, s->C, s->CB) && !s->ld_possible; }

static bool general_row_shape(const vgx_direct_shape *s) {
    return s->P <= VGX_QG_MAX_P && s->S <= VGX_QG_MAX_S && s->C <= VGX_QG_MAX_C && s->CB <= VGX_QG_MAX_CB &&
           3 * s->S + s->CB <= VGX_QG_MAX_W && s->n_seg <= VGX_QG_MAX_SEG;
}

static int64_t solo_compact(const vgx_direct_shape *s) {
    const int64_t maxterms = s->solo_maxnnz * s->P;
    if (s->solo_ncls > VGX_SOLO_ROWS || s->S > VGX_SOLO_MAX_S || s->P > 64 || maxterms > 32) return 0;
    return maxterms <= 16 ? 1 : 2;
}

static int64_t solo_lds_bytes(const vgx_direct_shape *s, int64_t *mig_in_lds) {
    const int64_t with_mig = vgx_solo_layout((int)s->P, (int)s->H, (int)s->S, (int)s->sites, 1).total;
    *mig_in_lds = with_mig <= VGX_SOLO_MAX_LDS ? 1 : 0;
    return *mig_in_lds ? with_mig : vgx_solo_layout((int)s->P, (int)s->H, (int)s->S, (int)s->sites, 0).total;
}

// ... 192 lines not shown
    HIPCHECK(e, hipMemsetAsync(e->r_effMig.p, 0, (size_t)(R * P * P) * 8, e->stream));
    HIPCHECK(e, hipMemsetAsync(e->r_popD.p, 0, (size_t)(R * PD_COUNT * P) * 8, e->stream));
    HIPCHECK(e, hipMemsetAsync(e->r_immSrc.p, 0, (size_t)(R * P * S) * 8, e->stream));

    rc |= upload(e, e->s_nocc, nocc.data(), nocc.size());
    rc |= upload(e, e->s_hap, hap.data(), hap.size());
    rc |= upload(e, e->s_cls, cl.data(), cl.size());
    rc |= upload(e, e->s_cnt, cnt.data(), cnt.size());
    rc |= upload(e, e->s_sus, h.susceptible.data(), h.susceptible.size());
    rc |= upload(e, e->s_cd, h.contactDensity.data(), h.contactDensity.size());
    std::vector<int64_t> tot((size_t)(3 * P));
    for (int64_t pn = 0; pn < P; pn++) {
        tot[(size_t)pn] = h.totalSusceptible[(size_t)pn];
        tot[(size_t)(P + pn)] = h.totalInfectious[(size_t)pn];
        tot[(size_t)(2 * P + pn)] = h.lockdownON[(size_t)pn];
    }
    rc |= upload(e, e->s_tot, tot.data(), tot.size());
    rc |= upload(e, e->i_nocc, i_nocc.data(), i_nocc.size());
    rc |= upload(e, e->i_hap, i_hap.data(), i_hap.size());
    rc |= upload(e, e->i_cls, i_cl.data(), i_cl.size());
    rc |= upload(e, e->i_cnt, i_cnt.data(), i_cnt.size());
    rc |= upload(e, e->i_sus, h.initial_susceptible.data(), h.initial_susceptible.size());
    rc |= upload(e, e->r_seeds, e->seeds.data(), e->seeds.size());
    if (rc) return VGX_ERR_HIP;

    e->sc_host.assign((size_t)R, VgxRepScalars{});
    for (int64_t r = 0; r < R; r++) {
        VgxRepScalars &s = e->sc_host[(size_t)r];
        s.currentTime = h.currentTime; s.totalRate = h.totalRate; s.totalMig = h.totalMigrationRate; s.tau_l = h.tau_l;
        s.globalInfectious = h.globalInfectious;
        s.bCounter = h.bCounter; s.dCounter = h.dCounter; s.sCounter = h.sCounter; s.mCounter = h.mCounter;
        s.iCounter = h.iCounter; s.swapLockdown = h.swapLockdown; s.migPlus = h.migPlus; s.migNonPlus = h.migNonPlus;
        s.good_attempt = h.good_attempt;
        s.ev_ptr = h.ev_ptr;
    }
    HIPCHECK(e, hipMemcpyAsync(e->r_sc.p, e->sc_host.data(), (size_t)R * sizeof(VgxRepScalars), hipMemcpyHostToDevice, e->stream));

    VgxDevRep &d = e->dr;
    d.popD = (double *)e->r_popD.p; d.popI = (int64_t *)e->r_popI.p; d.sus = (int64_t *)e->r_sus.p;
    d.immSrc = (double *)e->r_immSrc.p; d.birthC = (double *)e->r_birthC.p; d.xC = (double *)e->r_xC.p;
    d.effMig = (double *)e->r_effMig.p; d.nocc = (int32_t *)e->r_nocc.p; d.lhap = (int32_t *)e->r_lhap.p;
    d.lcls = (int32_t *)e->r_lcls.p; d.lcnt = (int64_t *)e->r_lcnt.p; d.cap = cap;
    d.lcnt32 = want32 ? (int32_t *)e->r_lcnt32.p : nullptr;
    d.ltsum = (int64_t *)e->r_ltsum.p; d.capT = capT;
    HIPCHECK(e, hipMemsetAsync(e->r_ltsum.p, 0, (size_t)(R * P * capT) * 8, e->stream));
    d.i_nocc = (const int32_t *)e->i_nocc.p; d.i_hap = (const int32_t *)e->i_hap.p;
    d.i_cls = (const int32_t *)e->i_cls.p; d.i_cnt = (const int64_t *)e->i_cnt.p; d.i_cap = i_cap;
    d.i_sus = (const int64_t *)e->i_sus.p;
    d.sc = (VgxRepScalars *)e->r_sc.p; d.seeds = (const int64_t *)e->r_seeds.p;
    d.prof = (unsigned long long *)e->r_prof.p;
    HIPCHECK(e, hipMemsetAsync(e->r_prof.p, 0, (size_t)(R * VGX_PROF_SLOTS) * 8, e->stream));

    HIPCHECK(e, vgxi_launch_init_reps(&d, (int)P, (int)S, R, (const int32_t *)e->s_nocc.p, (const int32_t *)e->s_hap.p,
                                      (const int32_t *)e->s_cls.p, (const int64_t *)e->s_cnt.p, s_cap,
                                      (const int64_t *)e->s_sus.p, (const double *)e->s_cd.p,
                                      (const int64_t *)e->s_tot.p, e->stream));
    HIPCHECK(e, hipStreamSynchronize(e->stream));
    e->dev_state_valid = true;
    e->counts32_valid = want32;
    e->counts64_valid = true;
    (void)traj_points;
    return VGX_OK;
}

struct __attribute__((visibility("hidden"))) DirectRun {
    vgx_engine *const e;
    HostState &h;
    const int64_t P, R, iterations, sample_size, attempts;
    const float time;
    vgx_run_opts o;
    size_t lds = 0;
    bool fresh_state = false;
    std::vector<double> cont_t0;
    int64_t ev_size = 0, evcap = 0;
    bool ld_possible = false;
    vgx_direct_shape shape{};
    vgx_direct_plan plan{};
    VgxDirectArgs a{};
    VgxSoloArgs soa{};
    VgxLoneArgs loa{};
    VgxQuadgArgs qga{};
    VgxLaneWs ws{};
    bool dev_clock = true;
    int exact_rcp_div = 1;
    bool heap_full = false;

    int check_call() {
        if (!e->have_params || !e->have_state) return fail(e, VGX_ERR_ARG, "vgx_simulate_direct: set params and state first");
        if (iterations < 0 || attempts < 0) return fail(e, VGX_ERR_ARG, "vgx_simulate_direct: negative iterations/attempts");
        HIPCHECK(e, hipSetDevice(e->device));
        if (o.max_loop_factor <= 0) o.max_loop_factor = 1024;
        if (o.mode < 0 || o.mode > 2) return fail(e, VGX_ERR_ARG, "vgx_simulate_direct: mode must be 0 (exact), 1 (fast) or 2 (fast, Philox stream)");
        lds = lds_bytes_for(e);
        if (lds > 160 * 1024)
            return fail(e, VGX_ERR_ARG, "vgx_simulate_direct: the population/class tables need " + std::to_string(lds) +
                                            " bytes of LDS per wavefront (limit 163840): too many populations x rate classes");
        return VGX_OK;
    }

    int ensure_device_state() {
        fresh_state = !e->dev_state_valid;
        if (!fresh_state) return VGX_OK;
        prepare_first(e);
        return init_device_state(e, o.traj_points);
    }

    int continue_clock() {
        std::vector<double> &t0 = cont_t0;
        t0.assign((size_t)R, h.currentTime);
        if (fresh_state || !e->sc_host_valid || e->sc_host.size() != (size_t)R) return VGX_OK;
        int64_t work = 0;
        for (int64_t r = 0; r < R; r++) work += e->sc_host[(size_t)r].loop_iterations;
        const bool stale = e->dev_clock_stale;
        const bool rebuild = e->direct_logs_valid && (work <= 50000000 || stale);
        if (stale && !rebuild)
            return fail(e, VGX_ERR_ARG, "vgx_simulate_direct: the previous call ran without a device clock and left no event log to "
                                        "rebuild it from: set the state again (vgx_set_state) before continuing");
        const int64_t mism = e->clock_mismatches;
        for (int64_t r = 0; r < R; r++) {
            t0[(size_t)r] = e->sc_host[(size_t)r].currentTime;
            const bool ok = rebuild && host_clock(e, r) == VGX_OK && e->hc.exact;
            if (ok) t0[(size_t)r] = e->hc.final_time;
            else if (stale)
                return fail(e, VGX_ERR_ARG, "vgx_simulate_direct: cannot rebuild the clock of replicate " + std::to_string(r) +
                                            " after a call without a device clock");
        }
        e->clock_mismatches = mism;
        e->hc.rep = -1;
        if (stale) {
            for (int64_t r = 0; r < R; r++) e->sc_host[(size_t)r].currentTime = t0[(size_t)r];
            HIPCHECK(e, hipMemcpy(e->r_sc.p, e->sc_host.data(), (size_t)R * sizeof(VgxRepScalars), hipMemcpyHostToDevice));
            e->dev_clock_stale = false;
        }
        return VGX_OK;
    }

    int size_logs() {
        const int64_t ev_ptr0 = h.ev_ptr;
        ev_size = h.ev_size;
        if (ev_size < ev_ptr0) return fail(e, VGX_ERR_ARG, "vgx_simulate_direct: ev_size < ev_ptr");
        e->call_ev0.assign((size_t)R, ev_ptr0);
        if (!fresh_state && e->sc_host_valid && e->sc_host.size() == (size_t)R)
            for (int64_t r = 0; r < R; r++) e->call_ev0[(size_t)r] = e->sc_host[(size_t)r].ev_ptr;
        const int64_t ev_min = *std::min_element(e->call_ev0.begin(), e->call_ev0.end());
        const bool may_restart = ev_min <= 100 && iterations > 100;
        e->ev_base = may_restart ? 0 : ev_min;
        e->ev_ptr0 = ev_ptr0;
        evcap = o.record_events ? std::max<int64_t>(ev_size - e->ev_base, 1) : 1;
        for (int64_t pn = 0; pn < P; pn++)
            if (e->h_startLD[(size_t)pn] * (double)e->sizes[(size_t)pn] < (double)e->sizes[(size_t)pn] || h.lockdownON[(size_t)pn] != 0)
                ld_possible = true;
        e->loc_cap = ld_possible ? VGX_LOC_CAP : 1;
        e->fa_cap = (ld_possible && may_restart && o.record_events) ? VGX_FA_CAP : 0;
        int rc = 0;
        rc |= ensure(e, e->r_locrec, (size_t)(R * e->loc_cap * 2) * 4);
        rc |= ensure(e, e->r_loctime, (size_t)(R * e->loc_cap) * 8);
        rc |= ensure(e, e->r_lociter, (size_t)(R * e->loc_cap) * 8);
        rc |= ensure(e, e->r_farate, (size_t)(R * e->fa_cap) * 8);
        rc |= ensure(e, e->r_fakey, (size_t)(R * e->fa_cap) * 8);
        rc |= ensure(e, e->r_evrate, (size_t)(R * evcap) * 8);
        rc |= ensure(e, e->r_evcols, (size_t)(R * evcap * VGX_EV_COLS) * 4);
        if (o.traj_points > 0) rc |= ensure(e, e->r_traj, (size_t)(R * o.traj_points * P * 2) * 8);
        if (rc) return rc;
        e->evcap = evcap;
        e->traj_points = o.traj_points;
        e->last_ev_size = ev_size;
        return VGX_OK;
    }

    void fill_args() {
        a.p = e->dp;
        a.r = e->dr;
        a.r.ev_rate = (double *)e->r_evrate.p;
        a.r.ev_cols = (int32_t *)e->r_evcols.p;
        a.r.loc_rec = (int32_t *)e->r_locrec.p; a.r.loc_time = (double *)e->r_loctime.p; a.r.loc_iter = (int64_t *)e->r_lociter.p;
        a.r.loc_cap = e->loc_cap;
        a.r.fa_rate = (double *)e->r_farate.p; a.r.fa_key = (int64_t *)e->r_fakey.p; a.r.fa_cap = e->fa_cap;
        e->call_t0 = cont_t0;
        e->call_recorded = o.record_events != 0;
        e->call_has_tlimit = !(time == -1.0f);
        e->call_tlimit = (double)time;
        e->hc.rep = -1;
        a.r.evcap = evcap;
        a.r.ev_base = e->ev_base;
        a.r.traj = o.traj_points > 0 ? (double *)e->r_traj.p : nullptr;
        a.r.traj_points = o.traj_points;
        a.r.traj_t0 = o.traj_t0;
        a.r.traj_dt = o.traj_points > 1 ? (o.traj_t1 - o.traj_t0) / (double)(o.traj_points - 1) : 0.0;
        a.n_replicates = R;
        a.iterations = iterations; a.sample_size = sample_size; a.attempts = attempts; a.time = time;
        a.ev_size = ev_size;
        a.max_loop = o.max_loop_factor * std::max<int64_t>(iterations, 1) + (1 << 20);
        a.record_events = o.record_events ? 1 : 0;
        a.lds_bytes = (int32_t)lds;
        dev_clock = e->call_has_tlimit || o.traj_points > 0 || !o.record_events;
    }

    void fill_shape() {
        vgx_direct_shape &s = shape;
        s.P = P; s.H = e->d.hapNum; s.S = e->d.susNum; s.sites = e->d.sites; s.R = R;
        s.C = e->C; s.CB = e->CB; s.cap = e->cap;
        s.n_seg = (int64_t)e->h_seg_par.size(); s.n_solo_seg = (int64_t)e->h_so_sn.size();
        s.solo_npass0 = e->h_so_npass0; s.solo_npass1 = e->h_so_npass1;
        s.solo_ncls = e->h_so_ncls; s.solo_maxnnz = e->h_so_maxnnz;
        s.start_lone_rows = e->start_lone_rows; s.start_max_nocc = e->start_max_nocc;
        double hosts = 0.0;
        s.tot_sus_is_sus = s.S == 1;
        for (int64_t pn = 0; pn < P; pn++) {
            s.max_size = std::max(s.max_size, e->sizes[(size_t)pn]);
            hosts += (double)e->sizes[(size_t)pn];
            if (s.S == 1 && h.totalSusceptible[(size_t)pn] != h.susceptible[(size_t)pn]) s.tot_sus_is_sus = 0;
        }
        s.hosts_below_2p53 = hosts < 9007199254740992.0;
        s.ld_possible = ld_possible;
        s.recomb = e->recombination != 0.0;
        s.fresh_state = fresh_state;
        s.suscep_cumul0_zero = e->suscepCumul[0] == 0.0;
        s.have_counts32 = e->dr.lcnt32 != nullptr;
        s.no_lone = getenv("VGX_NO_LONE") != nullptr;
        s.solo_general = getenv("VGX_SOLO_GENERAL") != nullptr;
    }

    int choose() {
        e->call_philox = o.mode == 2;
        fill_shape();
        std::string msg;
        const int rc = vgx_choose_direct(&shape, &o, &plan, msg);
        if (rc) return fail(e, rc, msg);
        a.fast = (int32_t)plan.fast;
        a.rng_philox = (int32_t)plan.philox;
        return VGX_OK;
    }

    int alloc_workspace() {
        a.r.rec = nullptr; a.r.rec_cap = 0;
        e->rec_cap = 0;
        if (shape.recomb) {
            const int64_t rec_cap = evcap + 101 * std::max<int64_t>(attempts, 1);
            DIRECT_TRY(ensure(e, e->r_rec, (size_t)(R * rec_cap * 5) * 8));
            a.r.rec = (int64_t *)e->r_rec.p; a.r.rec_cap = rec_cap;
            e->rec_cap = rec_cap;
        }
        const int64_t H = shape.H, S = shape.S, k = plan.kernel;
        if (k == VGX_K_LANES) {
            const int64_t PH = P * H;
            const int64_t n_i = PH + P * S + 3 * P, n_d = P + 3 * PH + PH * S + P * S + 5 * P + P * P;
            DIRECT_TRY(ensure(e, e->r_lanews, (size_t)((n_i + n_d) * R) * 8));
            int64_t *wi = (int64_t *)e->r_lanews.p;
            ws.inf = wi; wi += PH * R; ws.sus = wi; wi += P * S * R; ws.totS = wi; wi += P * R; ws.totI = wi; wi += P * R; ws.lock = wi; wi += P * R;
            double *wd = (double *)wi;
            ws.cd = wd; wd += P * R; ws.birth = wd; wd += PH * R; ws.tE = wd; wd += PH * R; ws.hpr = wd; wd += PH * R;
            ws.shpr = wd; wd += PH * S * R; ws.immSrc = wd; wd += P * S * R; ws.infP = wd; wd += P * R; ws.immP = wd; wd += P * R;
            ws.popR = wd; wd += P * R; ws.migR = wd; wd += P * R; ws.maxEBM = wd; wd += P * R; ws.effMig = wd; wd += P * P * R;
        }
        e->last_kernel = k;
        if (k == VGX_K_QUADG) DIRECT_TRY(ensure(e, e->r_cold, (size_t)(R * P * (3 * S + e->CB)) * 8));
        if (k == VGX_K_QUAD || k == VGX_K_QUADG || k == VGX_K_QUADF || k == VGX_K_LONE) {
            int rcq = 0;
            rcq |= ensure(e, e->r_qeff, (size_t)(P * P) * 8);
            rcq |= ensure(e, e->r_qmebm, (size_t)P * 8);
            rcq |= ensure(e, e->r_qflag, 8);
            if (rcq) return rcq;
        }
        return VGX_OK;
    }

    void fill_kernel_args() {
        exact_rcp_div = getenv("VGX_SOLO_PLAIN_DIV") ? 0 : 1;
        if (plan.kernel == VGX_K_SOLO) {
            soa.mig_in_lds = (int32_t)plan.solo_mig_in_lds;
            soa.seg_sn = (const int32_t *)e->so_sn.p; soa.seg_sig = (const double *)e->so_sig.p; soa.nseg = (int32_t)e->h_so_sn.size();
            soa.rcpAs = (const double *)e->so_rcp.p;
            soa.tseg_par = (const int32_t *)e->q_segpar.p; soa.tseg_sn = (const int32_t *)e->q_segsn.p; soa.tseg_sig = (const double *)e->q_segsig.p;
            soa.cb_seg = (const int32_t *)e->q_cbseg.p; soa.pass = (const int32_t *)e->so_pass.p;
            soa.tnseg = (int32_t)e->h_seg_par.size(); soa.npass0 = e->h_so_npass0; soa.npass1 = e->h_so_npass1;
            soa.exact_rcp_div = exact_rcp_div;
            soa.hap_cls = (const int32_t *)e->so_hapcls.p; soa.cls_nnz = (const int32_t *)e->so_nnz.p; soa.cls_tsn = (const int32_t *)e->so_tsn.p;
            soa.cls_tsig = (const double *)e->so_tsig.p; soa.cls_sigma = (const double *)e->so_clssig.p;
            soa.n_cls = e->h_so_ncls;
            soa.maxterms = (int32_t)(e->h_so_maxnnz * P);
            soa.compact = (int32_t)plan.solo_compact;
        }
        if (plan.kernel == VGX_K_LONE) {
            loa.lds_bytes = (int32_t)plan.lone_lds_bytes;
            loa.general = (int32_t)plan.lone_general;
            loa.effMig = (const double *)e->r_qeff.p; loa.maxEBM = (const double *)e->r_qmebm.p; loa.has_mig = (const int32_t *)e->r_qflag.p;
            loa.rcpAs = (const double *)e->so_rcp.p;
            loa.exact_rcp_div = exact_rcp_div;
            loa.mut_uniform = (e->h_mut_uniform && !getenv("VGX_LONE_NO_MUTUNI")) ? 1 : 0;
            loa.seg_par = (const int32_t *)e->q_segpar.p; loa.seg_sn = (const int32_t *)e->q_segsn.p;
            loa.seg_sig = (const double *)e->q_segsig.p; loa.cb_seg = (const int32_t *)e->q_cbseg.p;
            loa.nseg = (int32_t)e->h_seg_par.size();
        }
        if (plan.kernel == VGX_K_QUADG) {
            qga.effMig0 = (const double *)e->r_qeff.p; qga.mebm0 = (const double *)e->r_qmebm.p; qga.has_mig0 = (const int32_t *)e->r_qflag.p;
            qga.cd0 = (const double *)e->s_cd.p;
            qga.seg_par = (const int32_t *)e->q_segpar.p; qga.seg_sn = (const int32_t *)e->q_segsn.p;
            qga.seg_sig = (const double *)e->q_segsig.p; qga.cb_seg = (const int32_t *)e->q_cbseg.p;
            qga.nseg = (int32_t)e->h_seg_par.size(); qga.W = (int32_t)(3 * shape.S + e->CB);
            qga.cold = (int64_t *)e->r_cold.p;
        }
    }

    int sync_counts() {
        const bool row32 = plan.kernel == VGX_K_QUAD || plan.kernel == VGX_K_QUADF;
        if (!e->counts64_valid && !(plan.leaves32 && e->counts32_valid)) {
            HIPCHECK(e, vgxi_launch_counts64(e->dr.lcnt32, e->dr.lcnt, R * P * e->cap, e->stream));
            e->counts64_valid = true;
        }
        if (row32 && !e->counts32_valid) {
            HIPCHECK(e, vgxi_launch_counts32(e->dr.lcnt, e->dr.lcnt32, R * P * e->cap, e->stream));
            e->counts32_valid = true;
        }
        return VGX_OK;
    }

    int launch() {
        const double *cd0 = (const double *)e->s_cd.p;
        double *qeff = (double *)e->r_qeff.p, *qmebm = (double *)e->r_qmebm.p;
        int32_t *qflag = (int32_t *)e->r_qflag.p;
        HIPCHECK(e, hipEventRecord(e->ev0, e->stream));
        switch (plan.kernel) {
        case VGX_K_SOLO: HIPCHECK(e, vgxi_launch_solo(&a, &soa, dev_clock ? 1 : 0, e->stream)); break;
        case VGX_K_LONE:
            HIPCHECK(e, vgxi_launch_quad_prep(&a.p, cd0, qeff, qmebm, qflag, e->stream));
            HIPCHECK(e, vgxi_launch_lone(&a, &loa, dev_clock ? 1 : 0, e->stream));
            break;
        case VGX_K_LANES: HIPCHECK(e, vgxi_launch_lanes(&a, &ws, e->stream)); break;
        case VGX_K_QUAD: HIPCHECK(e, vgxi_launch_quad(&a, cd0, qeff, qmebm, qflag, (int)plan.long_lists, exact_rcp_div ? 0 : 1, e->stream)); break;
        case VGX_K_QUADF: HIPCHECK(e, vgxi_launch_quadf(&a, cd0, qeff, qmebm, qflag, e->stream)); break;
        case VGX_K_QUADG:
            HIPCHECK(e, vgxi_launch_quad_prep(&a.p, cd0, qeff, qmebm, qflag, e->stream));
            HIPCHECK(e, vgxi_launch_quadg(&a, &qga, e->stream));
            break;
        default: HIPCHECK(e, vgxi_launch_direct(&a, lds, e->stream)); break;
        }
        e->counts32_valid = plan.kernel == VGX_K_QUAD || plan.kernel == VGX_K_QUADF;
        if (plan.leaves32) e->counts64_valid = false;
        e->dev_clock_stale = (plan.kernel == VGX_K_SOLO || plan.kernel == VGX_K_LONE) && !dev_clock;
        HIPCHECK(e, hipEventRecord(e->ev1, e->stream));
        if (hipStreamSynchronize(e->stream) != hipSuccess) {
            e->dev_state_valid = false;
            return fail(e, VGX_ERR_HIP, std::string("vgx_simulate_direct: kernel failed: ") + hipGetErrorString(hipGetLastError()));
        }
        HIPCHECK(e, hipEventElapsedTime(&e->last_ms, e->ev0, e->ev1));
        e->last_launches = 1;
        return VGX_OK;
    }

    int collect() {
        e->sc_host.resize((size_t)R);
        HIPCHECK(e, hipMemcpy(e->sc_host.data(), e->r_sc.p, (size_t)R * sizeof(VgxRepScalars), hipMemcpyDeviceToHost));
        e->sc_host_valid = true;
        if (plan.kernel == VGX_K_LONE && o.kernel == 0) {
            for (int64_t r = 0; r < R; r++) heap_full = heap_full || e->sc_host[(size_t)r].error == (VGX_ERR_CAPACITY | (VGX_LONE_FULL_SITE << 8));
            if (heap_full) {
                if (getenv("VGX_TIMING")) fprintf(stderr, "vgx_lone: LDS heap full, the call runs again on the row kernel\n");
                e->dev_state_valid = false;
                e->sc_host_valid = false;
                e->lone_fallbacks += 1;
                return VGX_OK;
            }
        }
        e->direct_logs_valid = e->call_recorded;
        h.ev_ptr = e->sc_host[0].ev_ptr;
        for (int64_t r = 0; r < R; r++) {
            int64_t er = e->sc_host[(size_t)r].error;
            if (er) {
                const int64_t where = er >> 8;
                er &= 255;
                const char *what = er == VGX_ERR_ZERO_WEIGHT ? "zero weight sampled (fastChoose alert)"
                                   : er == VGX_ERR_CAPACITY  ? "capacity exceeded (occupancy list / event or lockdown log)"
                                   : er == VGX_ERR_LOOP_GUARD ? "loop guard tripped"
                                                              : "kernel error";
                return fail(e, (int)er, std::string("vgx_simulate_direct: replicate ") + std::to_string(r) + ": " + what +
                                            (where ? " [site " + std::to_string(where) + "]" : std::string()));
            }
        }
        return VGX_OK;
    }

    int run() {
        DIRECT_TRY(check_call());
        DIRECT_TRY(ensure_device_state());
        DIRECT_TRY(continue_clock());
        DIRECT_TRY(size_logs());
        fill_args();
        DIRECT_TRY(choose());
        DIRECT_TRY(alloc_workspace());
        fill_kernel_args();
        DIRECT_TRY(sync_counts());
        DIRECT_TRY(launch());
        return collect();
    }
};

int direct_core(vgx_engine *e, int64_t iterations, int64_t sample_size, float time, int64_t attempts,
                const vgx_run_opts *opts) {
    vgx_run_opts o{};
    o.record_events = 1;
    if (opts) o = *opts;
    DirectRun first{e, e->hs, e->d.popNum, e->R, iterations, sample_size, attempts, time, o};
    const int rc = first.run();
    if (rc || !first.heap_full) return rc;
    vgx_run_opts again = first.o;
    again.kernel = first.plan.fallback_kernel;
    again.mode = first.plan.fallback_mode;
    DirectRun second{e, e->hs, e->d.popNum, e->R, iterations, sample_size, attempts, time, again};
    return second.run();
}

extern "C" int vgx_simulate_direct(vgx_engine *e, int64_t iterations, int64_t sample_size, float time,
                                   int64_t attempts, const vgx_run_opts *opts) {
    if (!e) return VGX_ERR_ARG;
    e->last_was_tau = false;
    return direct_core(e, iterations, sample_size, time, attempts, opts);
}
```

vgsim_amd/csrc/vgx_quad.hip:

```cpp
#include <hip/hip_runtime.h>
#include <stdint.h>
#include "vgx_dev.h"
#include "vgx_rng.h"
#include "vgx_wave.h"
#include "vgx_rowprim.h"
#include "vgx_rowlist.h"
#include "vgx_flat.h"

#ifndef VGX_QUAD_WAVES
#define VGX_QUAD_WAVES 2
#endif

#ifdef VGX_PROFILE
#define QPROF(i)                                                        \
    do {                                                                \
        unsigned long long prof_t1 = __builtin_readcyclecounter();      \
        prof_acc[i] += prof_t1 - prof_t0;                               \
        prof_t0 = prof_t1;                                              \
    } while (0)
#else
#define QPROF(i)
#endif

namespace {

enum { Q_ERR_ZERO_WEIGHT = 3, Q_ERR_CAPACITY = 4, Q_ERR_LOOP_GUARD = 5 };
enum { QEV_BIRTH = 0, QEV_DEATH, QEV_SAMPLING, QEV_MUTATION, QEV_SUSCCHANGE, QEV_MIGRATION };
enum { ST_REBUILD = 0, ST_RUN = 1, ST_DONE = 2 };

#define Q_CONST_BYTES 2560
#define Q_RNG_BYTES 512
#define Q_REP_BYTES 2912
#define Q_LDS_BYTES (Q_CONST_BYTES + Q_RNG_BYTES + 4 * Q_REP_BYTES)
enum { QC_B = 0, QC_D, QC_M, QC_MIGP, QC_MIGN };

#define QFM4(K) "v_fmac_f64_dpp %0, %1, %5 row_newbcast:" #K " row_mask:0xf bank_mask:0xf\n\t" \
                "v_fmac_f64_dpp %0, %2, %5 row_newbcast:" #K " row_mask:0xf bank_mask:0xf\n\t" \
                "v_fmac_f64_dpp %0, %3, %5 row_newbcast:" #K " row_mask:0xf bank_mask:0xf\n\t" \
                "v_fmac_f64_dpp %0, %4, %5 row_newbcast:" #K " row_mask:0xf bank_mask:0xf\n\t"
static __device__ __forceinline__ double row_sum64(double w0, double w1, double w2, double w3, double acc) {
    const double one = 1.0;
    asm volatile("s_nop 1\n\t" QFM4(0) QFM4(1) QFM4(2) QFM4(3) QFM4(4) QFM4(5) QFM4(6) QFM4(7) QFM4(8) QFM4(9) QFM4(10) QFM4(11)
                     QFM4(12) QFM4(13) QFM4(14) QFM4(15)
                 : "+v"(acc)
                 : "v"(w0), "v"(w1), "v"(w2), "v"(w3), "v"(one));
    return acc;
}
#define QSG4(K, NOP, M)                                                                                                         \
    asm volatile(NOP QFM4(K) : "+v"(acc) : "v"(w0), "v"(w1), "v"(w2), "v"(w3), "v"(__hiloint2double(M, 0)));
#define QSG12(K0, K1, K2) QSG4(K0, "", ma) ma = QMUL_SHR(ma, 3); QSG4(K1, "", mb) mb = QMUL_SHR(mb, 3); QSG4(K2, "", mc) mc = QMUL_SHR(mc, 3);
static __device__ __forceinline__ void row_scan64(double w0, double w1, double w2, double w3, double carry, double &p0, double &p1,
                                                  double &p2, double &p3) {
    double acc = carry;
    int one_hi = 0x3FF00000;
    asm volatile("" : "+v"(one_hi));
    int ma = QMUL_SHR(one_hi, 1), mb = QMUL_SHR(one_hi, 2), mc = QMUL_SHR(one_hi, 3);
    QSG4(0, "s_nop 1\n\t", ma) ma = QMUL_SHR(ma, 3);
    QSG4(1, "", mb) mb = QMUL_SHR(mb, 3);
    QSG4(2, "", mc) mc = QMUL_SHR(mc, 3);
    QSG12(3, 4, 5) QSG12(6, 7, 8) QSG12(9, 10, 11)
    QSG4(12, "", ma) QSG4(13, "", mb) QSG4(14, "", mc)
    p0 = acc + w0; p1 = p0 + w1; p2 = p1 + w2; p3 = p2 + w3;
}
struct QTile { int c0, c1, c2, c3; };
static __device__ __forceinline__ QTile tile_load(const int32_t *l3, int t, int rl) {
    const int4 a = *(const int4 *)(l3 + (int64_t)t * 64 + 4 * rl);
    QTile q;
    q.c0 = a.x; q.c1 = a.y; q.c2 = a.z; q.c3 = a.w;
    return q;
}

static __device__ __forceinline__ void q_zero_tail(int32_t *l3, int n, int64_t cap, bool on) {
    const int rl = threadIdx.x & 15;
    const int end = (int)min((int64_t)((n >> 6) + 1) * 64, cap);
#pragma unroll
    for (int u = 0; u < 4; ++u) {
        const int k = n + u * 16 + rl;
        if (on && k < end) l3[k] = 0;
    }
}

struct QSel { int k_hit, hap_hit, err; double pre_hit, w_hit; int64_t cnt_hit; };
template <int QT>
static __device__ __forceinline__ void q_long_select(const int32_t *ln, const int32_t *lh, int n_sel, int maxn, double tE,
                                                               double r2, bool evn, int H, QSel &o, const double *ltp) {
    const int rl = threadIdx.x & 15;
    o.k_hit = -1; o.err = 0;
    QTile buf[QT];
    QTile kc = {0, 0, 0, 0};
    double carry = 0.0, carry_hit = 0.0;
    int t_hit = -1;
    const int nt = (n_sel + 63) >> 6, maxt = (maxn + 63) >> 6;
    const int full = QT >= 4 ? -rows_max(n_sel > 0 ? -n_sel : -0x7fffffff) >> 6 : 0;
    const double tEz = n_sel > 0 ? tE : 0.0;
    if (QT >= 4) {
        const int ntc = nt > 1 ? nt : 0;
        const int maxtc = rows_max(ntc);
        const int lastc = max(ntc - 1, 0);
        double gcarry = 0.0;
        for (int tb = 0; tb < maxtc; tb += 64) {
            const int j0 = tb + 4 * rl;
            const double q0 = ltp[min(j0 + 0, lastc)], q1 = ltp[min(j0 + 1, lastc)], q2 = ltp[min(j0 + 2, lastc)], q3 = ltp[min(j0 + 3, lastc)];
            const int kk = (j0 + 0 < ntc && !(q0 < r2)) ? 0 : (j0 + 1 < ntc && !(q1 < r2)) ? 1 : (j0 + 2 < ntc && !(q2 < r2)) ? 2
                         : (j0 + 3 < ntc && !(q3 < r2)) ? 3 : 4;
            const int q = row_min(t_hit < 0 && kk < 4 ? 4 * rl + kk : 64);
            double pl = q3;
            {
                const int lo = VGX_DPP_SHR(__double2loint(q3), 1), hi = VGX_DPP_SHR(__double2hiint(q3), 1);
                pl = rl == 0 ? gcarry : __hiloint2double(hi, lo);
            }
            if (t_hit < 0 && q < 64) {
                const int k = q & 3;
                t_hit = tb + q;
                carry_hit = rowget_f64(k == 0 ? pl : k == 1 ? q0 : k == 2 ? q1 : q2, q >> 2);
            }
            gcarry = rowget_f64(q3, 15);
            if (!__ballot(ntc > tb + 64 && t_hit < 0)) break;
        }
        if (ntc > 0) carry = ltp[lastc];
        else if (n_sel > 0) { t_hit = 0; carry_hit = 0.0; }
    } else {
#pragma unroll
    for (int d = 0; d < QT; ++d) buf[d] = tile_load(ln, d < nt ? d : 0, rl);
    for (int tb = 0; tb < maxt; tb += QT) {
#pragma unroll
        for (int d = 0; d < QT; ++d) {
            const int t = tb + d;
            const QTile c = buf[d];
            buf[d] = tile_load(ln, (t + QT < nt && t_hit < 0) ? t + QT : 0, rl);
            double w0, w1, w2, w3;
            if (QT < 4) {
                const double tEt = t < nt ? tEz : 0.0;
                w0 = tEt * (double)c.c0; w1 = tEt * (double)c.c1; w2 = tEt * (double)c.c2; w3 = tEt * (double)c.c3;
            } else if (t < full) {
                w0 = tEz * (double)c.c0; w1 = tEz * (double)c.c1; w2 = tEz * (double)c.c2; w3 = tEz * (double)c.c3;
            } else {
                const int e0 = t * 64 + 4 * rl;
                w0 = e0 + 0 < n_sel ? tE * (double)c.c0 : 0.0; w1 = e0 + 1 < n_sel ? tE * (double)c.c1 : 0.0;
                w2 = e0 + 2 < n_sel ? tE * (double)c.c2 : 0.0; w3 = e0 + 3 < n_sel ? tE * (double)c.c3 : 0.0;
            }
            const double acc = row_sum64(w0, w1, w2, w3, carry);
            const bool own = t_hit < 0 && t < nt;
            if (QT < 4 && own) kc = c;
            if (own && !(acc < r2)) { t_hit = t; carry_hit = carry; }
            carry = acc;
        }
        if (!__ballot(nt > tb + QT && t_hit < 0)) break;
    }
    }
    const int tt = t_hit >= 0 ? t_hit : max((n_sel - 1) >> 6, 0);
    const QTile c = QT < 4 ? kc : tile_load(ln, tt, rl);
    const int4 hv = *(const int4 *)(lh + (int64_t)tt * 64 + 4 * rl);
    const int e0 = tt * 64 + 4 * rl;
    double w0, w1, w2, w3;
    if (QT < 4) {
        w0 = tEz * (double)c.c0; w1 = tEz * (double)c.c1; w2 = tEz * (double)c.c2; w3 = tEz * (double)c.c3;
    } else {
        w0 = e0 + 0 < n_sel ? tE * (double)c.c0 : 0.0; w1 = e0 + 1 < n_sel ? tE * (double)c.c1 : 0.0;
        w2 = e0 + 2 < n_sel ? tE * (double)c.c2 : 0.0; w3 = e0 + 3 < n_sel ? tE * (double)c.c3 : 0.0;
    }
    double p0, p1, p2, p3;
    row_scan64(w0, w1, w2, w3, t_hit >= 0 ? carry_hit : 0.0, p0, p1, p2, p3);
    int mine = 64;
    if (t_hit >= 0) {
        if (e0 + 3 < n_sel && !(p3 < r2)) mine = 4 * rl + 3;
        if (e0 + 2 < n_sel && !(p2 < r2)) mine = 4 * rl + 2;
        if (e0 + 1 < n_sel && !(p1 < r2)) mine = 4 * rl + 1;
        if (e0 + 0 < n_sel && !(p0 < r2)) mine = 4 * rl + 0;
    }
    const int q = row_min(mine);
    const int qe = q < 64 ? q : ((n_sel - 1) & 63);
    const int ql = qe >> 2, qj = qe & 3;
    const double psel = qj == 0 ? p0 : qj == 1 ? p1 : qj == 2 ? p2 : p3;
    const double wsel = qj == 0 ? w0 : qj == 1 ? w1 : qj == 2 ? w2 : w3;
    const int64_t csel = (int64_t)(qj == 0 ? c.c0 : qj == 1 ? c.c1 : qj == 2 ? c.c2 : c.c3);
    o.pre_hit = q < 64 ? rowget_f64(psel, ql) : (QT >= 4 && nt <= 1) ? rowget_f64(p3, 15) : carry;
    o.w_hit = rowget_f64(wsel, ql);
    o.cnt_hit = rowget_i64(csel, ql);
    o.hap_hit = rowget_i32(qj == 0 ? hv.x : qj == 1 ? hv.y : qj == 2 ? hv.z : hv.w, ql);
    if (q < 64) o.k_hit = tt * 64 + q;
    else if (evn) {
        if (n_sel > 0 && o.hap_hit == H - 1 && (QT < 4 || o.cnt_hit != 0)) o.k_hit = n_sel - 1; else o.err = Q_ERR_ZERO_WEIGHT + 256 * 3;
    }
            
}

#define VGX_QB8 6
template <int QT>
static __device__ __forceinline__ double q_long_sum(const int32_t *ln, const uint8_t *l8, int n, int maxn, double tE, double *ltp) {
    const int rl = threadIdx.x & 15;
    double acc = 0.0;
    const int nt = (n + 63) >> 6, maxt = (maxn + 63) >> 6;
    const double tEz = n > 0 ? tE : 0.0;
    if (QT >= 4) {
        const int full = -rows_max(n > 0 ? -n : -0x7fffffff) >> 6;
        uint32_t buf8[VGX_QB8];
#pragma unroll
        for (int d = 0; d < VGX_QB8; ++d) buf8[d] = *(const uint32_t *)(l8 + (int64_t)(d < nt ? d : 0) * 64 + 4 * rl);
        for (int tb = 0; tb < maxt; tb += VGX_QB8) {
#pragma unroll
            for (int d = 0; d < VGX_QB8; ++d) {
                const int t = tb + d;
                const uint32_t w = buf8[d];
                buf8[d] = *(const uint32_t *)(l8 + (int64_t)(t + VGX_QB8 < nt ? t + VGX_QB8 : 0) * 64 + 4 * rl);
                if (t >= maxt) continue;
                int c0 = (int)(w & 255u), c1 = (int)((w >> 8) & 255u), c2 = (int)((w >> 16) & 255u), c3 = (int)(w >> 24);
                const bool sat = t < nt && ((((w & 0x7F7F7F7Fu) + 0x01010101u) & w & 0x80808080u) != 0u);
                if (__builtin_expect(__ballot(sat) != 0, 0)) {
                    const QTile q = tile_load(ln, t < nt ? t : 0, rl);
                    if (row_max(sat ? 1 : 0)) { c0 = q.c0; c1 = q.c1; c2 = q.c2; c3 = q.c3; }
                }
                double w0, w1, w2, w3;
                if (t < full) {
                    w0 = tEz * (double)c0; w1 = tEz * (double)c1; w2 = tEz * (double)c2; w3 = tEz * (double)c3;
                } else {
                    const int e0 = t * 64 + 4 * rl;
                    w0 = e0 + 0 < n ? tE * (double)c0 : 0.0; w1 = e0 + 1 < n ? tE * (double)c1 : 0.0;
                    w2 = e0 + 2 < n ? tE * (double)c2 : 0.0; w3 = e0 + 3 < n ? tE * (double)c3 : 0.0;
                }
                acc = row_sum64(w0, w1, w2, w3, acc);
                if (t < nt && rl == (t & 15)) ltp[t] = acc;
            }
        }
        return acc;
    }
    QTile buf[QT];
#pragma unroll
    for (int d = 0; d < QT; ++d) buf[d] = tile_load(ln, d < nt ? d : 0, rl);
    for (int tb = 0; tb < maxt; tb += QT) {
#pragma unroll
        for (int d = 0; d < QT; ++d) {
            const int t = tb + d;
            const QTile c = buf[d];
            buf[d] = tile_load(ln, t + QT < nt ? t + QT : 0, rl);
            const double tEt = t < nt ? tEz : 0.0;
            acc = row_sum64(tEt * (double)c.c0, tEt * (double)c.c1, tEt * (double)c.c2, tEt * (double)c.c3, acc);
        }
    }
    return acc;
}

struct QArgs {
    const double *effMig;
    const double *maxEBM;
    const int32_t *has_mig;
};

}

extern "C" __global__ void __launch_bounds__(64) vgx_quad_prep_kernel(VgxDevParams p, const double *cd, double *effMig,
                                                                     double *maxEBM, int32_t *has_mig) {
    const int P = p.P;
    bool anyf = false;
    for (int base = 0; base < P; base += 64) {
        const int pn2 = base + (int)threadIdx.x;
        double mx = 0.0;
        if (pn2 < P) {
            const double *m2 = p.mig + (int64_t)pn2 * P;
            for (int pn1 = 0; pn1 < P; ++pn1) {
                if (pn1 == pn2) continue;
                const double *m1 = p.mig + (int64_t)pn1 * P;
                double e = 0.0;
                for (int pn3 = 0; pn3 < P; ++pn3) e += m1[pn3] * m2[pn3] * cd[pn3] / p.actualSizes[pn3];
                effMig[(int64_t)pn1 * P + pn2] = e;
                if (e > mx) mx = e;
            }
            maxEBM[pn2] = mx * p.maxEffectiveBirth;
        }
        anyf = anyf || (__ballot(pn2 < P && mx * p.maxEffectiveBirth != 0.0) != 0ull);
    }
    if (threadIdx.x == 0) *has_mig = anyf ? 1 : 0;
}
extern "C" __attribute__((visibility("hidden"))) hipError_t vgxi_launch_quad_prep(const VgxDevParams *p, const double *cd, double *effMig,
                                                                                 double *maxEBM, int32_t *has_mig, hipStream_t stream) {
    hipLaunchKernelGGL(vgx_quad_prep_kernel, dim3(1), dim3(64), 0, stream, *p, cd, effMig, maxEBM, has_mig);
    return hipGetLastError();
}

struct VgxQuadKArgs { VgxDirectArgs a; QArgs qa; };
typedef const VgxQuadKArgs __attribute__((address_space(4))) *QuadKA;
template <int QT, bool RCPDIV>
static __device__ __forceinline__ void quad_body() {
    const QuadKA ka = (QuadKA)__builtin_amdgcn_kernarg_segment_ptr();
    const auto &a = ka->a;
    const auto &qa = ka->qa;
    const int lane = threadIdx.x, row = lane >> 4, rl = lane & 15;
    const auto &p = a.p;
    const auto &r = a.r;
    const int P = p.P, sites = p.sites, H = p.H;
    const int64_t R = a.n_replicates;
    const int64_t rep_raw = (int64_t)blockIdx.x * 4 + row;
    const bool live = rep_raw < R;
    const int64_t rep = live ? rep_raw : R - 1;
    const int nslot = (P + 15) >> 4;
    const bool has_mig = qa.has_mig[0] != 0;

    extern __shared__ __attribute__((aligned(16))) unsigned char smem[];
    double *k_cd = (double *)smem, *k_as = k_cd + 64, *k_smul = k_as + 64, *k_mebm = k_smul + 64, *k_rcp = k_mebm + 64;
    uint64_t *k_jump = (uint64_t *)(smem + Q_CONST_BYTES) + rl * 4;
    unsigned char *blk = smem + Q_CONST_BYTES + Q_RNG_BYTES + row * Q_REP_BYTES;
    double *s_inf = (double *)blk, *s_bc = s_inf + 64;
    double *s_ts = s_bc + 64, *s_ti = s_ts + 64;
    int32_t *s_nocc = (int32_t *)(s_ti + 64);
    double *s_cc = (double *)(s_nocc + 64);
    int64_t *s_cnt = (int64_t *)(s_cc + 4);
    uint64_t *s_inc = (uint64_t *)(s_cnt + 6);
    int32_t *s_zero = (int32_t *)(s_inc + 2);
    uint32_t *s_stage = (uint32_t *)(s_zero + 64);
    int stage_n = 0;
    int64_t stage_slot0 = 0;
    auto stage_flush = [&](bool f) {
        WSYNC();
        if (f && live) {
            const int n6 = stage_n * 6;
            int32_t *c = r.ev_cols + (rep * r.evcap + stage_slot0) * VGX_EV_COLS;
            uint32_t *q = (uint32_t *)(r.ev_rate + rep * r.evcap + stage_slot0);
#pragma unroll
            for (int j = 0; j < 3; ++j)
                if (rl + 16 * j < n6) c[rl + 16 * j] = (int32_t)s_stage[rl + 16 * j];
            if (rl < 2 * stage_n) q[rl] = s_stage[48 + rl];
        }
        if (f) stage_n = 0;
        WSYNC();
    };
#define QBUMP(i) do { if (rl == 0) s_cnt[i] += 1; } while (0)

    const double c_b = p.cb_b[0], c_sig = p.cb_sigma[0], c_d = p.c_d[0], c_s = p.c_s[0], c_tm = p.c_tm[0];

    {
        const double *gD = r.popD + rep * PD_COUNT * P;
        const int64_t *gI64 = r.popI + rep * PI_COUNT * P;
        const int32_t *gN = r.nocc + rep * P;
        const int pn = lane;
        k_cd[pn] = pn < P ? gD[PD_CD * P + pn] : 0.0;
        k_as[pn] = pn < P ? p.actualSizes[pn] : 1.0;
        k_rcp[pn] = pn < P ? 1.0 / p.actualSizes[pn] : 1.0;
        k_smul[pn] = pn < P ? c_s * p.sampMult[pn] : 0.0;
        k_mebm[pn] = pn < P ? qa.maxEBM[pn] : 0.0;
        for (int s = 0; s < 4; ++s) {
            const int pq = s * 16 + rl;
            const bool ok = pq < P;
            s_inf[pq] = 0.0; s_bc[pq] = 0.0;
            if (rl < 4) s_cc[rl] = 0.0;
            s_ts[pq] = ok ? (double)gI64[PI_TOTSUS * P + pq] : 0.0;
            s_ti[pq] = ok ? (double)gI64[PI_TOTINF * P + pq] : 0.0;
            s_nocc[pq] = ok ? gN[pq] : 0;
            s_zero[pq] = 0;
        }
    }
    WSYNC();

    const int64_t cap = r.cap, capT = r.capT;
    int32_t *lhap = r.lhap + rep * P * cap;
    int32_t *lcls = r.lcls + rep * P * cap;
    int64_t *lcnt = r.lcnt + rep * P * cap;
    int32_t *lcnt32 = r.lcnt32 + rep * P * cap;
#define L8(pop) ((uint8_t *)(r.lcnt32 + R * P * cap) + (rep * P + (int64_t)(pop)) * cap)
#define B8(v) ((uint8_t)((v) < 255 ? (v) : 255))
    int64_t *ltsum = r.ltsum + rep * P * capT;
    const bool has_traj = r.traj != nullptr;
    const VgxRepScalars *sc = r.sc + rep;
    if (QT < 4) {
        for (int pn = 0; pn < P; ++pn) q_zero_tail(lcnt32 + (int64_t)pn * cap, s_nocc[pn], cap, live);
        WSYNC();
    }

    double t_now = sc->currentTime, totalRate = 0.0, totalMig = 0.0;
    double gI = (double)sc->globalInfectious;
    int64_t ev_ptr = sc->ev_ptr;
    int64_t cS = sc->sCounter;
    if (rl == 0) {
        s_cnt[QC_B] = sc->bCounter; s_cnt[QC_D] = sc->dCounter; s_cnt[QC_M] = sc->mCounter;
        s_cnt[QC_MIGP] = sc->migPlus; s_cnt[QC_MIGN] = sc->migNonPlus;
    }
    int64_t loops = 0, att_loops = 0, good_attempt = sc->good_attempt;
    int att = 0, restarts = 0, last_att = -1, traj_next = 0;
    int st = live ? ST_REBUILD : ST_DONE, err = 0;
    bool open = false;
    const double tlimit = (double)a.time;
    const bool has_tl = !(a.time == -1.0f);

    if (row == 0) {
        const uint64_t MH = 0x2360ED051FC65DA4ull, ML = 0x4385DF649FCCF645ull;
        uint64_t Ah = MH, Al = ML, Gh = 0, Gl = 1;
        for (int j = 1; j < 16; ++j) {
            uint64_t nh, nl, gh, gl;
            vgx_mul128(Ah, Al, MH, ML, nh, nl);
            vgx_mul128(Gh, Gl, MH, ML, gh, gl);
            vgx_add128(gh, gl, 0, 1);
            if (j <= rl) { Ah = nh; Al = nl; Gh = gh; Gl = gl; }
        }
        k_jump[0] = Ah; k_jump[1] = Al; k_jump[2] = Gh; k_jump[3] = Gl;
    }
    WSYNC();
    uint64_t g_sh = 0, g_sl = 0;
    double g_val = 0.0;
    int pos = 8;
    int32_t ch_cn[4] = {0, 0, 0, 0};

#ifdef VGX_PROFILE
    unsigned long long prof_acc[VGX_PROF_SLOTS], prof_t0 = __builtin_readcyclecounter();
    for (int i = 0; i < VGX_PROF_SLOTS; ++i) prof_acc[i] = 0;
    int prof_tiles[7] = {0, 0, 0, 0, 0, 0, 0};
#endif
    while (true) {
        QPROF(0);
        const bool run = st != ST_DONE;
        if (!__ballot(run)) break;
        const bool rebuild = st == ST_REBUILD;

        bool end_attempt = false, ev = false;
        if (st == ST_RUN) {
            if (!open) {
                if (att >= a.attempts) {
                    st = ST_DONE;
                } else {
                    VgxPcg64 sd;
                    vgx_pcg64_seed(sd, (uint64_t)r.seeds[rep], (uint32_t)att);
                    g_sh = sd.sh; g_sl = sd.sl;
                    if (rl == 0) { s_inc[0] = sd.ih; s_inc[1] = sd.il; }
                    pos = 8;
                    open = true;
                    last_att = att; att_loops = 0;
                    if (!(totalRate + totalMig != 0.0 && gI != 0.0)) end_attempt = true;
                }
            }
            if (st == ST_RUN && !end_attempt &&
                !(ev_ptr < a.ev_size && (a.sample_size == -1 || cS <= a.sample_size) && (!has_tl || t_now < tlimit)))
                end_attempt = true;
            if (st == ST_RUN && !end_attempt) {
                if (loops >= a.max_loop) { err = Q_ERR_LOOP_GUARD; st = ST_DONE; }
                else ev = true;
            }
        }

        int u_lo = 0, u_hi = rebuild ? P : 0;
        int op_n = 0, op_pi = 0, op_h0 = 0, op_h1 = 0;
        int op_d0 = 0;
        int e_type = -1, e_hap = 0, e_pop = 0, e_nh = 0, e_np = 0;
        double den = 0.0;
        int ch_pi = -1;
        double m_pre[4] = {0.0, 0.0, 0.0, 0.0};
        int pm_pi = -1;

        QPROF(1);
        if (__ballot(ev)) {
            if (__builtin_expect(__ballot(ev && pos == 8) != 0, 0)) {
                const bool fill = ev && pos == 8;
                uint64_t h, l, ch, cl;
                vgx_mul128(k_jump[0], k_jump[1], g_sh, g_sl, h, l);
                vgx_mul128(k_jump[2], k_jump[3], s_inc[0], s_inc[1], ch, cl);
                vgx_add128(h, l, ch, cl);
                const double u = vgx_pcg64_output_double(h, l);
                const double v = (rl & 1) ? u : -vgx_log(u);
                const uint64_t nh = (uint64_t)rowget_i64((int64_t)h, 15), nl = (uint64_t)rowget_i64((int64_t)l, 15);
                if (fill) { g_val = v; g_sh = nh; g_sl = nl; pos = 0; }
            }
            const int pp = min(pos, 7);
            const double nlog = rowget_f64(g_val, 2 * pp), u2 = rowget_f64(g_val, 2 * pp + 1);
            if (ev) { pos += 1; loops += 1; att_loops += 1; }
            QPROF(2);
            den = totalRate + totalMig;
            const double t_new = t_now + (nlog / den);
            if (has_traj) {
                while (true) {
                    const double tg = r.traj_t0 + (double)traj_next * r.traj_dt;
                    const bool emit = ev && live && traj_next < r.traj_points && tg < t_new;
                    if (__builtin_expect(!__ballot(emit), 1)) break;
                    if (emit) {
                        double *o = r.traj + (rep * r.traj_points + traj_next) * (int64_t)P * 2;
                        for (int s = 0; s < nslot; ++s) {
                            const int pn = s * 16 + rl;
                            if (pn < P) { o[pn * 2 + 0] = s_ti[pn]; o[pn * 2 + 1] = s_ts[pn]; }
                        }
                        traj_next += 1;
                    }
                }
            }
            if (ev) t_now = t_new;

            QPROF(3);
            double rn = u2;
            const double choose0 = rn * den;
            double choose = choose0;
            const bool evn = ev && (totalRate > choose);
            const bool evm = ev && !evn;

            int pi = 0;
            {
                rn = choose / totalRate;
                const double rr_ = totalRate * rn;
                const double c0 = s_cc[0], c1 = s_cc[1], c2 = s_cc[2], c3 = s_cc[3];
                const int slot = !(c0 < rr_) ? 0 : !(c1 < rr_) ? 1 : !(c2 < rr_) ? 2 : 3;
                const bool any = !(c3 < rr_);
                const double cin = slot == 0 ? 0.0 : slot == 1 ? c0 : slot == 2 ? c1 : c2;
                const double w = s_inf[slot * 16 + rl];
                double tot_;
                const double pre = row_scan16(w, cin, tot_);
                const int q = row_min(any && slot * 16 + rl < P && !(pre < rr_) ? rl : 16);
                double total, wi;
                if (q < 16) { pi = slot * 16 + q; total = rowget_f64(pre, q); wi = rowget_f64(w, q); }
                else { pi = P - 1; total = c3; wi = s_inf[P - 1]; }
                if (evn && wi == 0.0) err = Q_ERR_ZERO_WEIGHT + 256 * 1;
                rn = (rr_ - (total - wi)) / wi;
                choose = rn * wi;
            }
            const double infect_pi = s_inf[pi];
            rn = (choose - 0.0) / infect_pi;
            const double bC = s_bc[pi];
            const double smul = k_smul[pi];
            const double tE = ((bC + c_d) + smul) + c_tm;
            const int n_sel = evn ? s_nocc[pi] : 0;
            const int32_t *lh = lhap + (int64_t)pi * cap;
            int64_t *ln = lcnt + (int64_t)pi * cap;
            int32_t *l3 = lcnt32 + (int64_t)pi * cap;
            int64_t *lt = ltsum + (int64_t)pi * capT;
            {
                const double *mrow = p.mig + (int64_t)pi * P;
#pragma unroll
                for (int s = 0; s < 4; ++s)
                    if (s < nslot) m_pre[s] = mrow[min(s * 16 + rl, P - 1)];
                pm_pi = evn ? pi : -1;
            }

            QPROF(4);
            const double r2 = infect_pi * rn;
            int k_hit = -1;
            double pre_hit = 0.0, w_hit = 0.0;
            int hap_hit = 0;
            int64_t cnt_hit = 0;
            const int maxn = rows_max(n_sel);
            if (__builtin_expect(maxn <= 64, QT < 4)) {
                const int nch = (maxn + 15) >> 4;
                const int last = max(n_sel - 1, 0);
                const double tEz = n_sel > 0 ? tE : 0.0;
                int32_t cn4[4];
                int hp4[4];
                double w4[4];
#pragma unroll
                for (int c = 0; c < 4; ++c) {
                    cn4[c] = 0; hp4[c] = 0; w4[c] = 0.0;
                    if (c < nch) {
                        const int k = c * 16 + rl;
                        hp4[c] = lh[min(k, last)];
                        if (QT < 4 && c > 0) {
                            cn4[c] = l3[k];
                            w4[c] = tEz * (double)cn4[c];
                        } else {
                            cn4[c] = l3[min(k, last)];
                            w4[c] = k < n_sel ? tE * (double)cn4[c] : 0.0;
                        }
                    }
                }
                double carry = 0.0, carry_hit = 0.0;
                int c_hit = nch == 1 ? 0 : -1;
                if (nch > 1) {
#pragma unroll
                    for (int c = 0; c < 4; ++c) {
                        if (c < nch) {
                            const double acc = row_sum16(w4[c], carry);
                            if (c_hit < 0 && c * 16 < n_sel && !(acc < r2)) { c_hit = c; carry_hit = carry; }
                            carry = acc;
                        }
                    }
                }
                const int cc = c_hit >= 0 ? c_hit : (last >> 4);
                const double w = cc == 0 ? w4[0] : cc == 1 ? w4[1] : cc == 2 ? w4[2] : w4[3];
                const int32_t cn = cc == 0 ? cn4[0] : cc == 1 ? cn4[1] : cc == 2 ? cn4[2] : cn4[3];
                const int hp = cc == 0 ? hp4[0] : cc == 1 ? hp4[1] : cc == 2 ? hp4[2] : hp4[3];
                double tot_;
                const double pre = row_scan16(w, c_hit >= 0 ? carry_hit : 0.0, tot_);
                if (nch == 1) carry = tot_;
                const int q = row_min(c_hit >= 0 && cc * 16 + rl < n_sel && !(pre < r2) ? rl : 16);
                const int qq = q < 16 ? q : (last & 15);
                pre_hit = q < 16 ? rowget_f64(pre, qq) : carry;
                w_hit = rowget_f64(w, qq);
                hap_hit = rowget_i32(hp, qq); cnt_hit = rowget_i32(cn, qq);
                if (q < 16) k_hit = cc * 16 + q;
                else if (evn) {
                    if (n_sel > 0 && hap_hit == H - 1 && (QT < 4 || cnt_hit != 0)) k_hit = n_sel - 1; else err = Q_ERR_ZERO_WEIGHT + 256 * 2;
                }
                if (evn) {
#pragma unroll
                    for (int c = 0; c < 4; ++c) ch_cn[c] = cn4[c];
                    ch_pi = pi;
                }
            } else {
#ifdef VGX_PROFILE
                prof_acc[15] += 1;
#endif
                QSel sel;
                q_long_select<QT>(l3, lh, n_sel, maxn, tE, r2, evn, H, sel, (double *)(ltsum + (int64_t)pi * capT + R * P * capT))   ;
                k_hit = sel.k_hit; pre_hit = sel.pre_hit; w_hit = sel.w_hit; hap_hit = sel.hap_hit; cnt_hit = sel.cnt_hit;
                if (sel.err) err = sel.err;
#ifdef VGX_PROFILE
                {
                    const int nt_ = (n_sel + 63) >> 6, need_ = k_hit >= 0 ? (k_hit >> 6) + 1 : nt_;
                    prof_tiles[0] += nt_; prof_tiles[1] += (maxn + 63) >> 6; prof_tiles[2] += need_; prof_tiles[3] += rows_max(need_);
                }
#endif
            }
            const bool evn_ok = evn && err == 0;
            if (evn && w_hit == 0.0 && err == 0) err = Q_ERR_ZERO_WEIGHT + 256 * 4;
            rn = (r2 - (pre_hit - w_hit)) / w_hit;

            QPROF(5);
            int ei = 0;
            {
                const double r3 = tE * rn;
                double total = bC, wi = bC;
                if (total < r3) { ei = 1; total += c_d; wi = c_d; }
                if (ei == 1 && total < r3) { ei = 2; total += smul; wi = smul; }
                if (ei == 2 && total < r3) { ei = 3; total += c_tm; wi = c_tm; }
                if (evn_ok && wi == 0.0) err = Q_ERR_ZERO_WEIGHT + 256 * 5;
                rn = (r3 - (total - wi)) / wi;
            }
            const bool go = evn && err == 0;
            const double ts_pi = s_ts[pi], ti_pi = s_ti[pi];
            const bool isB = go && ei == 0, isD = go && (ei == 1 || ei == 2), isM = go && ei == 3;
            if (isB) {
                if (ts_pi * c_sig == 0.0) err = Q_ERR_ZERO_WEIGHT + 256 * 6;
                if (rl == 0) { s_ts[pi] = ts_pi - 1.0; s_ti[pi] = ti_pi + 1.0; }
                gI += 1.0; QBUMP(QC_B);
                if (live && rl == 0) { if (QT < 4) ln[k_hit] = cnt_hit + 1; l3[k_hit] = (int32_t)(cnt_hit + 1); if (QT >= 4) L8(pi)[k_hit] = B8(cnt_hit + 1); if (n_sel > 64) lt[k_hit >> 6] += 1; }
#pragma unroll
                for (int c = 0; c < 4; ++c)
                    if (c == (k_hit >> 4) && rl == (k_hit & 15)) ch_cn[c] += 1;
                e_type = QEV_BIRTH; e_hap = hap_hit; e_pop = pi; e_nh = 0; e_np = H;
                u_lo = pi; u_hi = pi + 1;
            }
            if (isD) {
                if (rl == 0) { s_ts[pi] = ts_pi + 1.0; s_ti[pi] = ti_pi - 1.0; }
                gI -= 1.0;
                if (ei == 2) { cS += 1; e_type = QEV_SAMPLING; } else { QBUMP(QC_D); e_type = QEV_DEATH; }
                if (QT < 4 && cnt_hit == 1) { op_n = 1; op_pi = pi; op_h0 = hap_hit; op_d0 = -1; ch_pi = -1; }
                else {
                    if (live && rl == 0) { if (QT < 4) ln[k_hit] = cnt_hit - 1; l3[k_hit] = (int32_t)(cnt_hit - 1); if (QT >= 4) L8(pi)[k_hit] = B8(cnt_hit - 1); if (n_sel > 64) lt[k_hit >> 6] -= 1; }
                    if (QT >= 4 && cnt_hit == 1 && rl == 0) s_zero[pi] += 1;
#pragma unroll
                    for (int c = 0; c < 4; ++c)
                        if (c == (k_hit >> 4) && rl == (k_hit & 15)) ch_cn[c] -= 1;
                }
                e_hap = hap_hit; e_pop = pi; e_nh = 0; e_np = 0;
                u_lo = pi; u_hi = pi + 1;
            }
            QPROF(6);
            if (__builtin_expect(__ballot(isM) != 0, 0)) {
                const double *mr = p.mRate + (int64_t)hap_hit * sites;
                int mi = 0;
                {
                    const double rq = c_tm * rn;
                    double total = isM ? mr[0] : 1.0, wi = total;
                    for (int i = 1; i < sites; ++i) {
                        if (isM && mi == i - 1 && total < rq) { mi = i; wi = mr[i]; total += wi; }
                    }
                    if (isM && wi == 0.0) err = Q_ERR_ZERO_WEIGHT + 256 * 7;
                    rn = (rq - (total - wi)) / wi;
                }
                const double *hm = p.hapMutType + ((int64_t)hap_hit * sites + mi) * 3;
                int DS = 0;
                if (isM) {
                    const double h0 = hm[0], h1 = hm[1], h2 = hm[2];
                    const double rq = ((h0 + h1) + h2) * rn;
                    double total = h0, wi = h0;
                    if (total < rq) { DS = 1; total += h1; wi = h1; }
                    if (DS == 1 && total < rq) { DS = 2; total += h2; wi = h2; }
                    if (wi == 0.0) err = Q_ERR_ZERO_WEIGHT + 256 * 8;
                }
                if (isM && err == 0) {
                    const int digit4 = 1 << (2 * (sites - mi - 1));
                    const int AS = (hap_hit / digit4) % 4;
                    if (DS >= AS) DS += 1;
                    const int nhi = hap_hit + (DS - AS) * digit4;
                    if (QT >= 4) {
                        if (live && rl == 0) { l3[k_hit] = (int32_t)(cnt_hit - 1); L8(pi)[k_hit] = B8(cnt_hit - 1); if (n_sel > 64) lt[k_hit >> 6] -= 1; if (cnt_hit == 1) s_zero[pi] += 1; }
                        op_n = 1; op_pi = pi; op_h0 = nhi; op_d0 = +1; ch_pi = -1;
                    } else {
                        op_n = 2; op_pi = pi; op_h0 = nhi; op_d0 = +1; op_h1 = hap_hit; ch_pi = -1;
                    }
                    QBUMP(QC_M);
                    e_type = QEV_MUTATION; e_hap = hap_hit; e_pop = pi; e_nh = nhi; e_np = 0;
                    u_lo = pi; u_hi = pi + 1;
                }
            }
            QPROF(7);
            if (__builtin_expect(__ballot(evm) != 0, 0)) {
                double rm = (choose0 - totalRate) / totalMig;
                int tpi = 0;
                {
                    const double rr_ = totalMig * rm;
                    double carry = 0.0, tot_hit = 0.0, w_h = 0.0;
                    int cand = 64;
                    for (int s = 0; s < nslot; ++s) {
                        const int pn = s * 16 + rl;
                        const double w = pn < P ? k_mebm[pn] * s_ts[pn] * (gI - s_ti[pn]) : 0.0;
                        double tot_;
                        const double pre = row_scan16(w, carry, tot_);
                        const int q = row_min(cand == 64 && pn < P && !(pre < rr_) ? rl : 16);
                        if (cand == 64 && q < 16) { cand = s * 16 + q; tot_hit = rowget_f64(pre, q); w_h = rowget_f64(w, q); }
                        else if (s == nslot - 1 && cand == 64) {
                            const int ql = (P - 1) & 15;
                            tot_hit = rowget_f64(pre, ql); w_h = rowget_f64(w, ql);
                        }
                        carry = tot_;
                    }
                    tpi = cand < 64 ? cand : P - 1;
                    if (evm && w_h == 0.0) err = Q_ERR_ZERO_WEIGHT + 256 * 9;
                    rm = (rr_ - (tot_hit - w_h)) / w_h;
                }
                int spi = -1;
                {
                    const double rr_ = (gI - s_ti[tpi]) * rm;
                    const int start = tpi == 0 ? 1 : 0;
                    int64_t carry = 0, total = 0;
                    for (int s = 0; s < nslot; ++s) {
                        const int pn = s * 16 + rl;
                        const bool in = pn < P && pn != tpi && pn >= start;
                        const int64_t w = in ? (int64_t)s_ti[pn] : 0;
                        const int64_t pre = row_iscan(w) + carry;
                        const int q = row_min(spi < 0 && in && !((double)pre < rr_) ? rl : 16);
                        if (spi < 0 && q < 16) { spi = s * 16 + q; total = rowget_i64(pre, q); }
                        carry = rowget_i64(pre, 15);
                    }
                    if (spi < 0) { spi = P - 1; total = carry; }
                    const int64_t wi = (int64_t)s_ti[spi];
                    if (evm && wi == 0) err = Q_ERR_ZERO_WEIGHT + 256 * 10;
                    rm = (rr_ - (double)(total - wi)) / (double)wi;
                }
                int hi = 0;
                {
                    const int n = evm ? s_nocc[spi] : 0;
                    const int32_t *lh2 = lhap + (int64_t)spi * cap;
                    const int64_t *ln2 = lcnt + (int64_t)spi * cap;
                    const int32_t *l32 = lcnt32 + (int64_t)spi * cap;
#define CN2(k) (QT >= 4 ? (int64_t)l32[k] : ln2[k])
                    const int64_t *lt2 = ltsum + (int64_t)spi * capT;
                    const double rr_ = s_ti[spi] * rm;
                    int64_t before = 0;
                    int base = 0;
                    bool none = false;
                    const int maxn2 = rows_max(n);
                    if (__builtin_expect(maxn2 > 64, QT >= 4)) {
                        const int nt = n > 64 ? (n + 63) >> 6 : 0;
                        const int maxt = rows_max(nt);
                        int jt = -1;
                        int64_t carry = 0;
                        for (int tb = 0; tb < maxt; tb += 16) {
                            const int j = tb + rl;
                            const int64_t w = j < nt ? lt2[j] : 0;
                            const int64_t pre = row_iscan(w) + carry;
                            const int q = row_min(jt < 0 && j < nt && !((double)pre < rr_) ? rl : 16);
                            if (jt < 0 && q < 16) { jt = tb + q; before = rowget_i64(pre, q) - rowget_i64(w, q); }
                            carry = rowget_i64(pre, 15);
                        }
                        if (nt > 0) { if (jt < 0) { none = true; before = carry; } else base = jt * 64; }
                    }
                    int kq = -1;
                    int64_t total = before, wi = 0;
                    {
                        int64_t carry = before;
                        for (int c4 = 0; c4 < 4; ++c4) {
                            const int k = base + c4 * 16 + rl;
                            const bool in = !none && k < n;
                            const int64_t w = in ? CN2(k) : 0;
                            const int64_t pre = row_iscan(w) + carry;
                            const int q = row_min(kq < 0 && in && (QT < 4 || w != 0) && !((double)pre < rr_) ? rl : 16);
                            if (kq < 0 && q < 16) { kq = k - rl + q; total = rowget_i64(pre, q); wi = rowget_i64(w, q); }
                            carry = rowget_i64(pre, 15);
                            if (!__ballot(evm && kq < 0 && !none && base + (c4 + 1) * 16 < n)) break;
                        }
                        if (kq < 0) total = carry;
                    }
                    if (evm && kq < 0) {
                        if (n > 0 && lh2[n - 1] == H - 1 && (QT < 4 || CN2(n - 1) != 0)) { kq = n - 1; wi = CN2(n - 1); }
                        else {
                            err = Q_ERR_ZERO_WEIGHT + 256 * 11;
                            if (rl == 0 && r.prof) {
                                unsigned long long *d = r.prof + rep * VGX_PROF_SLOTS;
                                d[0] = n; d[1] = spi; d[2] = tpi; d[3] = (int64_t)s_ti[spi]; d[4] = __double_as_longlong(rr_); d[5] = __double_as_longlong(rm);
                                d[6] = total; d[7] = before; d[8] = maxn2; d[9] = (int64_t)gI; d[10] = (int64_t)s_ti[tpi]; d[11] = n > 0 ? CN2(0) : -1;
                                d[12] = ev_ptr; d[13] = loops; d[14] = __double_as_longlong(totalMig); d[15] = __double_as_longlong(choose);
                            }
                            kq = 0; wi = 1;
                        }
                    }
                    if (kq < 0) { kq = 0; wi = 1; }
                    rm = (rr_ - (double)(total - wi)) / (double)wi;
                    hi = (evm && n > 0) ? lh2[kq] : 0;
                }
                {
                    const double wi = s_ts[tpi];
                    const double rr_ = wi * rm;
                    if (evm && wi == 0.0 && err == 0) err = Q_ERR_ZERO_WEIGHT + 256 * 12;
                    rm = (rr_ - (wi - wi)) / wi;
                }
                const bool mgo = evm && err == 0;
                if (mgo) {
                    const double p_accept = qa.effMig[(int64_t)spi * P + tpi] * p.bRate[hi] * p.susc[hi] / k_mebm[tpi];
                    if (rm < p_accept) {
                        if (rl == 0) { s_ts[tpi] -= 1.0; s_ti[tpi] += 1.0; }
                        gI += 1.0; QBUMP(QC_MIGP);
                        op_n = 1; op_pi = tpi; op_h0 = hi; op_d0 = +1; ch_pi = -1;
                        e_type = QEV_MIGRATION; e_hap = hi; e_pop = spi; e_nh = 0; e_np = tpi;
                        u_lo = tpi; u_hi = tpi + 1;
                    } else {
                        QBUMP(QC_MIGN);
                    }
                }
            }
            WSYNC();
        }

        QPROF(8);
        if (err != 0) op_n = 0;
        if (QT >= 4) {
            if (__builtin_expect(__ballot(live && op_n > 0) != 0, 0)) {
                const bool act = live && op_n > 0;
                int n = act ? s_nocc[op_pi] : 0;
                const int n_was = n;
                WSYNC();
                int zeros = act ? s_zero[op_pi] : 0;
                const int z_was = zeros;
                const bool fits = q_list_add_one<true>(act, op_h0, lhap + (int64_t)op_pi * cap, lcls + (int64_t)op_pi * cap, lcnt32 + (int64_t)op_pi * cap,
                                                       ltsum + (int64_t)op_pi * capT, L8(op_pi), n, (int)cap, H, zeros);
                if (act && !fits) err = Q_ERR_CAPACITY;
                if (act && rl == 0) { if (n != n_was) s_nocc[op_pi] = n; if (zeros != z_was) s_zero[op_pi] = max(zeros, 0); }
                WSYNC();
            }
            {
                WSYNC();
                const int zp = (live && err == 0 && u_hi == u_lo + 1) ? u_lo : -1;
                const int nz = zp >= 0 ? s_zero[zp] : 0, nl = zp >= 0 ? s_nocc[zp] : 0;
                const bool sq = zp >= 0 && nz > max(16, nl >> 3);
                if (__builtin_expect(__ballot(sq) != 0, 0)) {
                    const int zq = sq ? zp : 0;
                    int32_t *l3z = lcnt32 + (int64_t)zq * cap;
                    const int n2 = q_compact_list<1>(lhap + (int64_t)zq * cap, l3z, ltsum + (int64_t)zq * capT, nl, sq);
                    uint8_t *l8z = L8(zq);
                    const int m8 = rows_max(sq ? n2 : 0);
                    for (int k = rl; k < m8; k += 16) if (sq && k < n2) l8z[k] = B8(l3z[k]);
                    if (sq && rl == 0) { s_nocc[zq] = n2; s_zero[zq] = 0; }
                    if (sq && ch_pi == zq) ch_pi = -1;
                    WSYNC();
                }
            }
        } else
        for (int oi = 0; oi < 2; ++oi) {
            const bool act = live && oi < op_n;
            if (!__ballot(act)) break;
            const int hap = oi == 0 ? op_h0 : op_h1;
            const int delta = oi == 0 ? op_d0 : -1;
            const int n = act ? s_nocc[op_pi] : 0;
            int32_t *lh = lhap + (int64_t)op_pi * cap;
            int32_t *lc = lcls + (int64_t)op_pi * cap;
            int64_t *ln = lcnt + (int64_t)op_pi * cap;
            int32_t *l3 = lcnt32 + (int64_t)op_pi * cap;
            int64_t *lt = ltsum + (int64_t)op_pi * capT;
            int posn = 0;
            bool found = false;
            int64_t cur = 0;
            {
                int lo = 0;
                const int maxn = rows_max(n);
                for (int stride = 1 << 20; stride >= 1; stride >>= 4) {
                    if (stride >= 16 && maxn <= stride) continue;
                    const int k = lo + rl * stride;
                    const int h = (act && k < n) ? lh[k] : 0x7fffffff;
                    const int nle = row_min(h <= hap ? 16 : rl);
                    if (stride == 1) {
                        const int q = row_min(h >= hap ? rl : 16);
                        posn = lo + q;
                        if (posn > n) posn = n;
                        const int hq = rowget_i32(h, min(q, 15));
                        found = q < 16 && hq == hap;
                    } else {
                        lo = lo + (nle > 0 ? (nle - 1) * stride : 0);
                    }
                }
                if (act && found) cur = ln[posn];
            }
            const bool bump = act && found && cur + delta != 0;
            const bool rem = act && found && cur + delta == 0;
            const bool ins = act && !found;
            if (ins && n >= cap) { err = Q_ERR_CAPACITY; }
            const bool ins_ok = ins && err == 0;
            if (bump && rl == 0) { ln[posn] = cur + delta; l3[posn] = (int32_t)(cur + delta); if (QT >= 4) L8(op_pi)[posn] = B8(cur + delta); if (n > 64) lt[posn >> 6] += delta; }
            if (__builtin_expect(__ballot((ins_ok || rem) && n > 64) != 0, 0)) {
                const bool tt = (ins_ok || rem) && n > 64;
                const int jp = posn >> 6, jl = ins_ok ? (n >> 6) : ((n - 1) >> 6);
                const int maxj = rows_max(tt ? jl + 1 : 0);
                for (int tb = 0; tb < maxj; tb += 16) {
                    const int j = tb + rl;
                    if (tt && j >= jp && j <= jl) {
                        int64_t in_, out_;
                        if (ins_ok) {
                            in_ = j == jp ? (int64_t)delta : ln[(int64_t)j * 64 - 1];
                            const int kout = j * 64 + 63;
                            out_ = kout < n ? ln[kout] : 0;
                        } else {
                            out_ = j == jp ? ln[posn] : ln[(int64_t)j * 64];
                            const int kin = j * 64 + 64;
                            in_ = kin < n ? ln[kin] : 0;
                        }
                        lt[j] += in_ - out_;
                    }
                }
                WSYNC();
            }
            if (__builtin_expect(__ballot(ins_ok) != 0, 0)) {
                enum { SU = 4 };
                int hi_ = ins_ok ? n : 0;
                const int lo_ = ins_ok ? posn : 0;
                while (__ballot(hi_ > lo_)) {
                    const int blo = max(lo_, hi_ - SU * 16);
                    int h[SU];
                    int64_t ct[SU];
#pragma unroll
                    for (int u = 0; u < SU; ++u) {
                        const int k = blo + u * 16 + rl;
                        h[u] = 0; ct[u] = 0;
                        if (k < hi_) { h[u] = lh[k]; ct[u] = ln[k]; }
                    }
                    WSYNC();
#pragma unroll
                    for (int u = 0; u < SU; ++u) {
                        const int k = blo + u * 16 + rl;
                        if (k < hi_) { lh[k + 1] = h[u]; lc[k + 1] = 0; ln[k + 1] = ct[u]; l3[k + 1] = (int32_t)ct[u]; if (QT >= 4) L8(op_pi)[k + 1] = B8(ct[u]); }
                    }
                    WSYNC();
                    hi_ = blo;
                }
                if (ins_ok && rl == 0) { lh[posn] = hap; lc[posn] = 0; ln[posn] = delta; l3[posn] = delta; if (QT >= 4) L8(op_pi)[posn] = B8(delta); s_nocc[op_pi] = n + 1; }
                q_zero_tail(l3, n + 1, cap, QT < 4 && ins_ok && ((n + 1) & 63) == 0);
                WSYNC();
                if (ins_ok && n == 64) {
                    int64_t s0 = 0;
                    for (int c4 = 0; c4 < 4; ++c4) s0 += rowget_i64(row_iscan(ln[c4 * 16 + rl]), 15);
                    if (rl == 0) { lt[0] = s0; lt[1] = ln[64]; }
                }
                WSYNC();
            }
            if (__builtin_expect(__ballot(rem) != 0, 0)) {
                enum { SU = 4 };
                int lo_ = rem ? posn + 1 : 0;
                const int hi_ = rem ? n : 0;
                while (__ballot(lo_ < hi_)) {
                    int h[SU];
                    int64_t ct[SU];
#pragma unroll
                    for (int u = 0; u < SU; ++u) {
                        const int k = lo_ + u * 16 + rl;
                        h[u] = 0; ct[u] = 0;
                        if (k < hi_) { h[u] = lh[k]; ct[u] = ln[k]; }
                    }
                    WSYNC();
#pragma unroll
                    for (int u = 0; u < SU; ++u) {
                        const int k = lo_ + u * 16 + rl;
                        if (k < hi_) { lh[k - 1] = h[u]; ln[k - 1] = ct[u]; l3[k - 1] = (int32_t)ct[u]; if (QT >= 4) L8(op_pi)[k - 1] = B8(ct[u]); }
                    }
                    WSYNC();
                    lo_ += SU * 16;
                }
                if (rem && rl == 0) { s_nocc[op_pi] = n - 1; if (QT < 4) l3[n - 1] = 0; }
                WSYNC();
            }
        }

        QPROF(9);
        if (err == 0 && e_type >= 0) {
            if (a.record_events) {
                const int64_t slot = ev_ptr - r.ev_base;
                if (slot >= 0 && slot < r.evcap) {
                    if (stage_n == 0) stage_slot0 = slot;
                    if (rl < 8) {
                        const int v = rl == 0 ? e_type : rl == 1 ? e_hap : rl == 2 ? e_pop : rl == 3 ? e_nh : rl == 4 ? e_np
                                      : rl == 5 ? (int)(uint32_t)att_loops : rl == 6 ? __double2loint(den) : __double2hiint(den);
                        s_stage[rl < 6 ? stage_n * 6 + rl : 48 + 2 * stage_n + (rl - 6)] = (uint32_t)v;
                    }
                    stage_n += 1;
                } else {
                    err = Q_ERR_CAPACITY;
                }
            }
            ev_ptr += 1;
        }
        if (__builtin_expect(__ballot(stage_n == 8) != 0, 0)) stage_flush(stage_n == 8);

        QPROF(10);
        if (err != 0) u_hi = u_lo;
        const int maxu = rows_max(u_hi - u_lo);
        if (maxu > 0) {
            for (int us = 0; us < maxu; ++us) {
                const int pn0 = u_lo + us;
                const bool act = pn0 < u_hi;
                const int pi = act ? pn0 : 0;
                const double x = s_ts[pi] * c_sig;
                const double *mrow = p.mig + (int64_t)pi * P;
                const bool mhave = act && pi == pm_pi;
                double tv4[4], ps = 0.0;
#pragma unroll
                for (int s = 0; s < 4; ++s) {
                    tv4[s] = 0.0;
                    if (s < nslot) {
                        const int pn = s * 16 + rl;
                        const double m = mhave ? m_pre[s] : mrow[min(pn, P - 1)];
                        const double t = x * m * m * k_cd[pn];
                        tv4[s] = RCPDIV ? div_by_const(t, k_as[pn], k_rcp[pn]) : t / k_as[pn];
                        if (pn >= P) tv4[s] = 0.0;
                    }
                }
#pragma unroll
                for (int s = 0; s < 4; ++s)
                    if (s < nslot) ps = row_sum16(tv4[s], ps);
                const double bC = c_b * ps;
                const double tE = ((bC + c_d) + k_smul[pi]) + c_tm;
                QPROF(11);
                const int n = act ? s_nocc[pi] : 0;
                const int32_t *l3 = lcnt32 + (int64_t)pi * cap;
                const int maxn = rows_max(n);
                double acc = 0.0;
                if (__builtin_expect(maxn <= 64, QT < 4)) {
                    const int nch = (maxn + 15) >> 4;
                    const bool chave = act && pi == ch_pi;
                    const double tEz = n > 0 ? tE : 0.0;
                    int32_t cn4[4];
#pragma unroll
                    for (int c = 0; c < 4; ++c) cn4[c] = ch_cn[c];
                    if (__ballot(act && !chave)) {
                        const int last = max(n - 1, 0);
#pragma unroll
                        for (int c = 0; c < 4; ++c)
                            if (c < nch) { const int32_t cl = l3[QT < 4 && c > 0 ? c * 16 + rl : min(c * 16 + rl, last)]; if (!chave) cn4[c] = cl; }
                    }
#pragma unroll
                    for (int c = 0; c < 4; ++c)
                        if (c < nch) acc = row_sum16(QT < 4 && c > 0 ? tEz * (double)cn4[c] : c * 16 + rl < n ? tE * (double)cn4[c] : 0.0, acc);
                } else {
#ifdef VGX_PROFILE
                    prof_tiles[4] += (n + 63) >> 6; prof_tiles[5] += (maxn + 63) >> 6; prof_tiles[6] += 1;
#endif
                    acc = q_long_sum<QT>(l3, L8(pi), n, maxn, tE, (double *)(ltsum + (int64_t)pi * capT + R * P * capT));
                }
                if (act && rl == 0) { s_bc[pi] = bC; s_inf[pi] = acc; }
                WSYNC();
                QPROF(12);
            }
            {
                double w4[4], carry = 0.0, cend[4];
#pragma unroll
                for (int s = 0; s < 4; ++s) w4[s] = s_inf[s * 16 + rl];
#pragma unroll
                for (int s = 0; s < 4; ++s) {
                    if (s < nslot) carry = row_sum16(w4[s], carry);
                    cend[s] = carry;
                }
                if (u_hi > u_lo) {
                    if (rl < 4) s_cc[rl] = rl == 0 ? cend[0] : rl == 1 ? cend[1] : rl == 2 ? cend[2] : cend[3];
                    totalRate = carry;
                }
                WSYNC();
            }
            QPROF(13);
            if (has_mig) {
                double w4[4], acc = 0.0;
#pragma unroll
                for (int s = 0; s < 4; ++s) {
                    w4[s] = 0.0;
                    if (s < nslot) {
                        const int pn = s * 16 + rl;
                        w4[s] = k_mebm[pn] * s_ts[pn] * (gI - s_ti[pn]);
                        if (pn >= P) w4[s] = 0.0;
                    }
                }
#pragma unroll
                for (int s = 0; s < 4; ++s)
                    if (s < nslot) acc = row_sum16(w4[s], acc);
                if (u_hi > u_lo) totalMig = acc;
            }
        }

        QPROF(14);
        if (rebuild && st == ST_REBUILD) st = err ? ST_DONE : ST_RUN;
        if (err != 0) st = ST_DONE;
        if (ev && st == ST_RUN && (totalRate == 0.0 || gI == 0.0)) end_attempt = true;
        if (st == ST_RUN && end_attempt) {
            open = false;
            if (ev_ptr <= 100 && a.iterations > 100) {
                ev_ptr = 0; cS = 0;
                stage_n = 0;
                if (rl < 6) s_cnt[rl] = 0;
                t_now = 0.0; traj_next = 0;
                restarts += 1; att += 1;
                st = ST_REBUILD;
            } else {
                good_attempt = (int64_t)att + 1;
                st = ST_DONE;
            }
        }
        if (__builtin_expect(__ballot(st == ST_REBUILD && restarts > 0 && !rebuild) != 0, 0)) {
            const bool rs = st == ST_REBUILD && restarts > 0 && !rebuild && live;
            int64_t g = 0;
            for (int pn = 0; pn < P; ++pn) {
                const int n = r.i_nocc[pn];
                const int n_old = rs ? s_nocc[pn] : 0;
                int64_t ti = 0;
                for (int base = 0; base < n; base += 64) {
                    int64_t tsum = 0;
                    for (int c4 = 0; c4 < 4; ++c4) {
                        const int k = base + c4 * 16 + rl;
                        int64_t ct = 0;
                        if (k < n) {
                            ct = r.i_cnt[(int64_t)pn * r.i_cap + k];
                            if (rs) {
                                lhap[(int64_t)pn * cap + k] = r.i_hap[(int64_t)pn * r.i_cap + k];
                                lcls[(int64_t)pn * cap + k] = r.i_cls[(int64_t)pn * r.i_cap + k];
                                lcnt[(int64_t)pn * cap + k] = ct;
                                lcnt32[(int64_t)pn * cap + k] = (int32_t)ct;
                                if (QT >= 4) L8(pn)[k] = B8(ct);
                            }
                        }
                        tsum += rowget_i64(row_iscan(ct), 15);
                    }
                    if (rs && rl == 0) ltsum[(int64_t)pn * capT + base / 64] = tsum;
                    ti += tsum;
                }
                if (rs)
                    for (int j = (n + 63) / 64 + rl; j <= n_old / 64 && j < capT; j += 16) ltsum[(int64_t)pn * capT + j] = 0;
                if (QT < 4) q_zero_tail(lcnt32 + (int64_t)pn * cap, n, cap, rs);
                if (rs && rl == 0) { s_nocc[pn] = n; s_zero[pn] = 0; s_ts[pn] = (double)r.i_sus[pn]; s_ti[pn] = (double)ti; }
                g += ti;
            }
            if (rs) gI = (double)g;
            WSYNC();
        }
    }

    if (has_traj) {
        while (true) {
            const bool emit = live && traj_next < r.traj_points;
            if (!__ballot(emit)) break;
            if (emit) {
                double *o = r.traj + (rep * r.traj_points + traj_next) * (int64_t)P * 2;
                for (int s = 0; s < nslot; ++s) {
                    const int pn = s * 16 + rl;
                    if (pn < P) { o[pn * 2 + 0] = s_ti[pn]; o[pn * 2 + 1] = s_ts[pn]; }
                }
                traj_next += 1;
            }
        }
    }

#ifdef VGX_PROFILE
    if (lane == 0 && r.prof)
        for (int i = 0; i < VGX_PROF_SLOTS; ++i) r.prof[rep * VGX_PROF_SLOTS + i] = prof_acc[i];
    for (int i = 0; i < 7; ++i) {
        const long long t4 = (long long)__builtin_amdgcn_readlane(prof_tiles[i], 0) + __builtin_amdgcn_readlane(prof_tiles[i], 16) +
                             __builtin_amdgcn_readlane(prof_tiles[i], 32) + __builtin_amdgcn_readlane(prof_tiles[i], 48);
        if (lane == 0 && r.prof && rep_raw + 1 < R) r.prof[(rep_raw + 1) * VGX_PROF_SLOTS + i] = (unsigned long long)t4;
    }
#endif
    stage_flush(stage_n > 0);
    WSYNC();
    if (live) {
        double *gD = r.popD + rep * PD_COUNT * P;
        int64_t *gI64 = r.popI + rep * PI_COUNT * P;
        int32_t *gN = r.nocc + rep * P;
        VgxRepScalars *sc = r.sc + rep;
        for (int s = 0; s < nslot; ++s) {
            const int pn = s * 16 + rl;
            if (pn < P) {
                gD[PD_POPRATE * P + pn] = s_inf[pn];
                gD[PD_INFECT * P + pn] = s_inf[pn];
                gD[PD_IMMUNE * P + pn] = 0.0;
                gD[PD_MIG * P + pn] = k_mebm[pn] * s_ts[pn] * (gI - s_ti[pn]);
                gD[PD_MAXEBM * P + pn] = k_mebm[pn];
                gI64[PI_TOTSUS * P + pn] = (int64_t)s_ts[pn];
                gI64[PI_TOTINF * P + pn] = (int64_t)s_ti[pn];
                gN[pn] = s_nocc[pn];
                r.sus[rep * P + pn] = (int64_t)s_ts[pn];
                r.immSrc[rep * P + pn] = 0.0;
            }
        }
        if (rl == 0) {
            sc->currentTime = t_now; sc->totalRate = totalRate; sc->totalMig = totalMig;
            sc->globalInfectious = (int64_t)gI;
            sc->bCounter = s_cnt[QC_B]; sc->dCounter = s_cnt[QC_D]; sc->sCounter = cS; sc->mCounter = s_cnt[QC_M];
            sc->migPlus = s_cnt[QC_MIGP]; sc->migNonPlus = s_cnt[QC_MIGN];
            sc->good_attempt = good_attempt;
            sc->ev_ptr = ev_ptr; sc->loop_iterations = loops; sc->restarts = restarts;
            sc->loc_n = 0; sc->error = err; sc->traj_next = traj_next;
            sc->last_attempt = last_att; sc->last_attempt_loops = att_loops;
            sc->fa_n = 0;
        }
    }
}

#ifndef VGX_QT_SHORT
#define VGX_QT_SHORT 1
#endif
extern "C" __global__ void __launch_bounds__(64, VGX_QUAD_WAVES) vgx_quad_kernel(VgxQuadKArgs) { quad_body<VGX_QT_SHORT, true>(); }
#ifndef VGX_QT_LONG
#define VGX_QT_LONG 7
#endif
extern "C" __global__ void __launch_bounds__(64, VGX_QUAD_WAVES) vgx_quad_long_kernel(VgxQuadKArgs) { quad_body<VGX_QT_LONG, true>(); }
extern "C" __global__ void __launch_bounds__(64, VGX_QUAD_WAVES) vgx_quad_kernel_plaindiv(VgxQuadKArgs) { quad_body<VGX_QT_SHORT, false>(); }
extern "C" __global__ void __launch_bounds__(64, VGX_QUAD_WAVES) vgx_quad_long_kernel_plaindiv(VgxQuadKArgs) { quad_body<VGX_QT_LONG, false>(); }

extern "C" __global__ void __launch_bounds__(256) vgx_quad_counts32_kernel(const int64_t *c64, int32_t *c32, int64_t n) {
    for (int64_t i = (int64_t)blockIdx.x * 256 + threadIdx.x; i < n; i += (int64_t)gridDim.x * 256) c32[i] = (int32_t)c64[i];
}
extern "C" __attribute__((visibility("hidden"))) hipError_t vgxi_launch_counts32(const int64_t *c64, int32_t *c32, int64_t n, hipStream_t stream) {
    hipLaunchKernelGGL(vgx_quad_counts32_kernel, dim3(4096), dim3(256), 0, stream, c64, c32, n);
    return hipGetLastError();
}

extern "C" __global__ void __launch_bounds__(256) vgx_quad_counts8_kernel(const int32_t *c32, uint8_t *c8, int64_t n4) {
    for (int64_t i = (int64_t)blockIdx.x * 256 + threadIdx.x; i < n4; i += (int64_t)gridDim.x * 256) {
        const int4 v = *(const int4 *)(c32 + 4 * i);
        *(uint32_t *)(c8 + 4 * i) = (uint32_t)min(max(v.x, 0), 255) | ((uint32_t)min(max(v.y, 0), 255) << 8) | ((uint32_t)min(max(v.z, 0), 255) << 16) |
                                    ((uint32_t)min(max(v.w, 0), 255) << 24);
    }
}

extern "C" __global__ void __launch_bounds__(256) vgx_traj_i32_kernel(const double *src, int32_t *dst, int64_t n) {
    for (int64_t i = (int64_t)blockIdx.x * 256 + threadIdx.x; i < n; i += (int64_t)gridDim.x * 256) dst[i] = (int32_t)src[i];
}
extern "C" __attribute__((visibility("hidden"))) hipError_t vgxi_launch_traj_i32(const double *src, int32_t *dst, int64_t n, hipStream_t stream) {
    hipLaunchKernelGGL(vgx_traj_i32_kernel, dim3(8192), dim3(256), 0, stream, src, dst, n);
    return hipGetLastError();
}

extern "C" __attribute__((visibility("hidden"))) hipError_t vgxi_launch_lists_settle(const VgxDirectArgs *a, hipStream_t stream);
extern "C" __attribute__((visibility("hidden"))) hipError_t vgxi_launch_quad(const VgxDirectArgs *a, const double *cd,
                                                                            double *effMig, double *maxEBM, int32_t *has_mig,
                                                                            int long_lists, int plain_div, hipStream_t stream) {
    hipLaunchKernelGGL(vgx_quad_prep_kernel, dim3(1), dim3(64), 0, stream, a->p, cd, effMig, maxEBM, has_mig);
    hipError_t err = hipGetLastError();
    if (err != hipSuccess) return err;
    VgxQuadKArgs ka;
    ka.a = *a;
    ka.qa.effMig = effMig; ka.qa.maxEBM = maxEBM; ka.qa.has_mig = has_mig;
    const unsigned grid = (unsigned)((a->n_replicates + 3) / 4);
    if (long_lists) {
        const int64_t n = (int64_t)a->n_replicates * a->p.P * a->r.cap;
        hipLaunchKernelGGL(vgx_quad_counts8_kernel, dim3(4096), dim3(256), 0, stream, a->r.lcnt32, (uint8_t *)(a->r.lcnt32 + n), (n + 3) / 4);
        hipLaunchKernelGGL(plain_div ? vgx_quad_long_kernel_plaindiv : vgx_quad_long_kernel, dim3(grid), dim3(64), Q_LDS_BYTES, stream, ka);
        hipError_t e2 = vgxi_launch_lists_settle(a, stream);
        if (e2 != hipSuccess) return e2;
    }
    else hipLaunchKernelGGL(plain_div ? vgx_quad_kernel_plaindiv : vgx_quad_kernel, dim3(grid), dim3(64), Q_LDS_BYTES, stream, ka);
    return hipGetLastError();
}

extern "C" __global__ void __launch_bounds__(64) vgx_quad_scantest_kernel(const double *w, const double *carry, int64_t rows, double *pre16,
                                                                         double *tot16, double *pre64) {
    const int rl = threadIdx.x & 15;
    const int64_t row_raw = (int64_t)blockIdx.x * 4 + (threadIdx.x >> 4);
    const int64_t row = row_raw < rows ? row_raw : rows - 1;
    const double c = carry[row];
    double tot;
    const double p = row_scan16(w[row * 64 + rl], c, tot);
    const double *w4 = w + row * 64 + 4 * rl;
    double p0, p1, p2, p3;
    row_scan64(w4[0], w4[1], w4[2], w4[3], c, p0, p1, p2, p3);
    if (row_raw < rows) {
        pre16[row * 16 + rl] = p; tot16[row * 16 + rl] = tot;
        double *o = pre64 + row * 64 + 4 * rl;
        o[0] = p0; o[1] = p1; o[2] = p2; o[3] = p3;
    }
}
extern "C" int vgx_test_row_scans(const double *w, const double *carry, int64_t rows, double *pre16, double *tot16, double *pre64) {
    if (!w || !carry || !pre16 || !tot16 || !pre64 || rows < 0) return 1;
    if (rows == 0) return 0;
    double *d = nullptr;
    const size_t n = (size_t)rows;
    if (hipMalloc((void **)&d, n * (64 + 1 + 16 + 16 + 64) * 8) != hipSuccess) return 2;
    double *dw = d, *dc = dw + n * 64, *d16 = dc + n, *dt = d16 + n * 16, *d64 = dt + n * 16;
    int rc = 0;
    if (hipMemcpy(dw, w, n * 64 * 8, hipMemcpyHostToDevice) != hipSuccess || hipMemcpy(dc, carry, n * 8, hipMemcpyHostToDevice) != hipSuccess) rc = 2;
    if (!rc) {
        hipLaunchKernelGGL(vgx_quad_scantest_kernel, dim3((unsigned)((rows + 3) / 4)), dim3(64), 0, nullptr, dw, dc, rows, d16, dt, d64);
        if (hipGetLastError() != hipSuccess || hipDeviceSynchronize() != hipSuccess ||
            hipMemcpy(pre16, d16, n * 16 * 8, hipMemcpyDeviceToHost) != hipSuccess ||
            hipMemcpy(tot16, dt, n * 16 * 8, hipMemcpyDeviceToHost) != hipSuccess ||
            hipMemcpy(pre64, d64, n * 64 * 8, hipMemcpyDeviceToHost) != hipSuccess)
            rc = 2;
    }
    (void)hipFree(d);
    return rc;
}
```

Measured before the change: 1.004 billion events/s.

## Cache per-tile prefix sums from rate update to reuse in quad long-list selection

In the QT<4 quad path, the per-tile cumulative sums computed during the population rate sum are now kept in a register (tc, tagged by population tc_pi). The next selection reuses them to find the hit tile directly instead of rescanning all tiles. The 64-bit count list and tile-sum array are no longer maintained per event on this path. Migration source selection scans the 32-bit counts directly, and tile sums are rebuilt once at kernel exit. This removes redundant global loads and writes per event, at the cost of cache-invalidation bookkeeping and extra registers.

Measured after the change: 1.102 billion events/s, median of 6. 1.1x the previous value.

```diff
diff --git a/include/vgx.h b/include/vgx.h
--- a/include/vgx.h
+++ b/include/vgx.h
@@ -268,6 +268,7 @@
 int64_t vgx_device_bytes(const vgx_engine *e);
 int vgx_get_profile(vgx_engine *e, int64_t replicate, int64_t *out16);
 int vgx_get_list_counts_quad(vgx_engine *e, int64_t replicate, int64_t population, int64_t count, int32_t *out, int64_t *list_cap);
+int vgx_get_list_tile_sums(vgx_engine *e, int64_t replicate, int64_t population, int64_t count, int64_t *out, int64_t *tile_cap);
 
 typedef struct vgx_rowscan {
     int64_t rows, H, S;
@@ -296,6 +297,9 @@
 
 int vgx_test_row_scans(const double *w, const double *carry, int64_t rows, double *pre16, double *tot16, double *pre64);
 
+int vgx_test_quad_tile_choice(const int32_t *counts, const int32_t *haps, const int32_t *n, const double *tE, const double *r, int64_t rows,
+                              int64_t maxlen, int H, int32_t *k_hit, double *pre_hit, double *w_hit, int64_t *cnt_hit);
+
 #ifdef __cplusplus
 }
 #endif
diff --git a/vgsim_amd/_capi.py b/vgsim_amd/_capi.py
--- a/vgsim_amd/_capi.py
+++ b/vgsim_amd/_capi.py
@@ -177,6 +177,7 @@
     "vgx_device_bytes": (C.c_int64, [_H]),
     "vgx_get_profile": (C.c_int, [_H, C.c_int64, _I]),
     "vgx_get_list_counts_quad": (C.c_int, [_H, C.c_int64, C.c_int64, C.c_int64, C.POINTER(C.c_int32), _I]),
+    "vgx_get_list_tile_sums": (C.c_int, [_H, C.c_int64, C.c_int64, C.c_int64, _I, _I]),
     "vgx_get_genealogy": (C.c_int, [C.POINTER(VgxGenealogyIO), C.c_char_p, C.c_int64]),
     "vgx_get_genealogies": (C.c_int, [_H, C.POINTER(VgxGenealogiesIO)]),
     "vgx_genealogy_message": (C.c_int, [C.c_int64, C.c_int64, C.c_char_p, C.c_int64]),
@@ -197,6 +198,8 @@
     "vgx_test_poisson": (C.c_int, [C.c_double, C.c_int64, C.c_uint64, _I]),
     "vgx_test_div_by_const": (C.c_int, [_F, _F, C.c_int64, _F, _F, _F]),
     "vgx_test_row_scans": (C.c_int, [_F, _F, C.c_int64, _F, _F, _F]),
+    "vgx_test_quad_tile_choice": (C.c_int, [C.POINTER(C.c_int32), C.POINTER(C.c_int32), C.POINTER(C.c_int32), _F, _F, C.c_int64, C.c_int64, C.c_int,
+                                            C.POINTER(C.c_int32), _F, _F, _I]),
 }
 
 _lib = None
diff --git a/vgsim_amd/csrc/vgx_api.hip b/vgsim_amd/csrc/vgx_api.hip
--- a/vgsim_amd/csrc/vgx_api.hip
+++ b/vgsim_amd/csrc/vgx_api.hip
@@ -937,6 +937,17 @@
     if (!out || !e->dev_state_valid || !e->counts32_valid || !e->dr.lcnt32 || count > e->cap) return VGX_ERR_ARG;
     HIPCHECK(e, hipSetDevice(e->device));
     HIPCHECK(e, hipMemcpy(out, e->dr.lcnt32 + (replicate * e->d.popNum + population) * e->cap, (size_t)count * 4, hipMemcpyDeviceToHost));
+    return VGX_OK;
+}
+
+extern "C" int vgx_get_list_tile_sums(vgx_engine *e, int64_t replicate, int64_t population, int64_t count, int64_t *out, int64_t *tile_cap) {
+    if (!e || replicate < 0 || replicate >= e->R || population < 0 || population >= e->d.popNum || count < 0) return VGX_ERR_ARG;
+    if (tile_cap) *tile_cap = e->dev_state_valid ? e->dr.capT : 0;
+    if (count == 0) return VGX_OK;
+    if (!out || !e->dev_state_valid || !e->dr.ltsum || count > e->dr.capT) return VGX_ERR_ARG;
+    HIPCHECK(e, hipSetDevice(e->device));
+    HIPCHECK(e, hipStreamSynchronize(e->stream));
+    HIPCHECK(e, hipMemcpy(out, e->dr.ltsum + (replicate * e->d.popNum + population) * e->dr.capT, (size_t)count * 8, hipMemcpyDeviceToHost));
     return VGX_OK;
 }
 
diff --git a/vgsim_amd/csrc/vgx_direct_run.hip b/vgsim_amd/csrc/vgx_direct_run.hip
--- a/vgsim_amd/csrc/vgx_direct_run.hip
+++ b/vgsim_amd/csrc/vgx_direct_run.hip
@@ -518,9 +518,10 @@
         }
     }
 
+    bool on_counts32() const { return plan.leaves32 || plan.kernel == VGX_K_QUAD; }
     int sync_counts() {
         const bool row32 = plan.kernel == VGX_K_QUAD || plan.kernel == VGX_K_QUADF;
-        if (!e->counts64_valid && !(plan.leaves32 && e->counts32_valid)) {
+        if (!e->counts64_valid && !(on_counts32() && e->counts32_valid)) {
             HIPCHECK(e, vgxi_launch_counts64(e->dr.lcnt32, e->dr.lcnt, R * P * e->cap, e->stream));
             e->counts64_valid = true;
         }
@@ -552,7 +553,7 @@
         default: HIPCHECK(e, vgxi_launch_direct(&a, lds, e->stream)); break;
         }
         e->counts32_valid = plan.kernel == VGX_K_QUAD || plan.kernel == VGX_K_QUADF;
-        if (plan.leaves32) e->counts64_valid = false;
+        if (on_counts32()) e->counts64_valid = false;
         e->dev_clock_stale = (plan.kernel == VGX_K_SOLO || plan.kernel == VGX_K_LONE) && !dev_clock;
         HIPCHECK(e, hipEventRecord(e->ev1, e->stream));
         if (hipStreamSynchronize(e->stream) != hipSuccess) {
diff --git a/vgsim_amd/csrc/vgx_quad.hip b/vgsim_amd/csrc/vgx_quad.hip
--- a/vgsim_amd/csrc/vgx_quad.hip
+++ b/vgsim_amd/csrc/vgx_quad.hip
@@ -1,5 +1,6 @@
 #include <hip/hip_runtime.h>
 #include <stdint.h>
+#include <vector>
 #include "vgx_dev.h"
 #include "vgx_rng.h"
 #include "vgx_wave.h"
@@ -83,16 +84,16 @@
 struct QSel { int k_hit, hap_hit, err; double pre_hit, w_hit; int64_t cnt_hit; };
 template <int QT>
 static __device__ __forceinline__ void q_long_select(const int32_t *ln, const int32_t *lh, int n_sel, int maxn, double tE,
-                                                               double r2, bool evn, int H, QSel &o, const double *ltp) {
+                                                               double r2, bool evn, int H, QSel &o, const double *ltp, int pi, double tc,
+                                                               int tc_pi) {
     const int rl = threadIdx.x & 15;
     o.k_hit = -1; o.err = 0;
     QTile buf[QT];
-    QTile kc = {0, 0, 0, 0};
     double carry = 0.0, carry_hit = 0.0;
     int t_hit = -1;
-    const int nt = (n_sel + 63) >> 6, maxt = (maxn + 63) >> 6;
-    const int full = QT >= 4 ? -rows_max(n_sel > 0 ? -n_sel : -0x7fffffff) >> 6 : 0;
+    const int nt = (n_sel + 63) >> 6;
     const double tEz = n_sel > 0 ? tE : 0.0;
+    (void)maxn;
     if (QT >= 4) {
         const int ntc = nt > 1 ? nt : 0;
         const int maxtc = rows_max(ntc);
@@ -120,36 +121,35 @@
         if (ntc > 0) carry = ltp[lastc];
         else if (n_sel > 0) { t_hit = 0; carry_hit = 0.0; }
     } else {
-#pragma unroll
-    for (int d = 0; d < QT; ++d) buf[d] = tile_load(ln, d < nt ? d : 0, rl);
-    for (int tb = 0; tb < maxt; tb += QT) {
-#pragma unroll
-        for (int d = 0; d < QT; ++d) {
-            const int t = tb + d;
-            const QTile c = buf[d];
-            buf[d] = tile_load(ln, (t + QT < nt && t_hit < 0) ? t + QT : 0, rl);
-            double w0, w1, w2, w3;
-            if (QT < 4) {
-                const double tEt = t < nt ? tEz : 0.0;
-                w0 = tEt * (double)c.c0; w1 = tEt * (double)c.c1; w2 = tEt * (double)c.c2; w3 = tEt * (double)c.c3;
-            } else if (t < full) {
-                w0 = tEz * (double)c.c0; w1 = tEz * (double)c.c1; w2 = tEz * (double)c.c2; w3 = tEz * (double)c.c3;
-            } else {
-                const int e0 = t * 64 + 4 * rl;
-                w0 = e0 + 0 < n_sel ? tE * (double)c.c0 : 0.0; w1 = e0 + 1 < n_sel ? tE * (double)c.c1 : 0.0;
-                w2 = e0 + 2 < n_sel ? tE * (double)c.c2 : 0.0; w3 = e0 + 3 < n_sel ? tE * (double)c.c3 : 0.0;
-            }
-            const double acc = row_sum64(w0, w1, w2, w3, carry);
-            const bool own = t_hit < 0 && t < nt;
-            if (QT < 4 && own) kc = c;
-            if (own && !(acc < r2)) { t_hit = t; carry_hit = carry; }
-            carry = acc;
-        }
-        if (!__ballot(nt > tb + QT && t_hit < 0)) break;
-    }
+        const bool multi = nt > 1;
+        const bool hitc = multi && tc_pi == pi;
+        const int qc = row_min(hitc && rl < nt && !(tc < r2) ? rl : 16);
+        const double cs = rowget_f64(tc, (qc < 16 ? max(qc - 1, 0) : max(nt - 1, 0)) & 15);
+        if (hitc) {
+            if (qc < 16) { t_hit = qc; carry_hit = qc > 0 ? cs : 0.0; } else carry = cs;
+        } else if (!multi && n_sel > 0) t_hit = 0;
+        const bool need = multi && !hitc;
+        const int maxs = rows_max(need ? nt : 0);
+        if (__builtin_expect(maxs > 0, 0)) {
+#pragma unroll
+            for (int d = 0; d < QT; ++d) buf[d] = tile_load(ln, need && d < nt ? d : 0, rl);
+            for (int tb = 0; tb < maxs; tb += QT) {
+#pragma unroll
+                for (int d = 0; d < QT; ++d) {
+                    const int t = tb + d;
+                    const QTile c = buf[d];
+                    buf[d] = tile_load(ln, (need && t + QT < nt && t_hit < 0) ? t + QT : 0, rl);
+                    const double tEt = need && t < nt ? tEz : 0.0;
+                    const double acc = row_sum64(tEt * (double)c.c0, tEt * (double)c.c1, tEt * (double)c.c2, tEt * (double)c.c3, carry);
+                    if (need && t_hit < 0 && t < nt && !(acc < r2)) { t_hit = t; carry_hit = carry; }
+                    carry = acc;
+                }
+                if (!__ballot(need && nt > tb + QT && t_hit < 0)) break;
+            }
+        }
     }
     const int tt = t_hit >= 0 ? t_hit : max((n_sel - 1) >> 6, 0);
-    const QTile c = QT < 4 ? kc : tile_load(ln, tt, rl);
+    const QTile c = tile_load(ln, tt, rl);
     const int4 hv = *(const int4 *)(lh + (int64_t)tt * 64 + 4 * rl);
     const int e0 = tt * 64 + 4 * rl;
     double w0, w1, w2, w3;
@@ -174,7 +174,7 @@
     const double psel = qj == 0 ? p0 : qj == 1 ? p1 : qj == 2 ? p2 : p3;
     const double wsel = qj == 0 ? w0 : qj == 1 ? w1 : qj == 2 ? w2 : w3;
     const int64_t csel = (int64_t)(qj == 0 ? c.c0 : qj == 1 ? c.c1 : qj == 2 ? c.c2 : c.c3);
-    o.pre_hit = q < 64 ? rowget_f64(psel, ql) : (QT >= 4 && nt <= 1) ? rowget_f64(p3, 15) : carry;
+    o.pre_hit = q < 64 ? rowget_f64(psel, ql) : nt <= 1 ? rowget_f64(p3, 15) : carry;
     o.w_hit = rowget_f64(wsel, ql);
     o.cnt_hit = rowget_i64(csel, ql);
     o.hap_hit = rowget_i32(qj == 0 ? hv.x : qj == 1 ? hv.y : qj == 2 ? hv.z : hv.w, ql);
@@ -182,12 +182,12 @@
     else if (evn) {
         if (n_sel > 0 && o.hap_hit == H - 1 && (QT < 4 || o.cnt_hit != 0)) o.k_hit = n_sel - 1; else o.err = Q_ERR_ZERO_WEIGHT + 256 * 3;
     }
-            
 }
 
 #define VGX_QB8 6
 template <int QT>
-static __device__ __forceinline__ double q_long_sum(const int32_t *ln, const uint8_t *l8, int n, int maxn, double tE, double *ltp) {
+static __device__ __forceinline__ double q_long_sum(const int32_t *ln, const uint8_t *l8, int n, int maxn, double tE, double *ltp, bool act,
+                                                    int pi, double &tc, int &tc_pi) {
     const int rl = threadIdx.x & 15;
     double acc = 0.0;
     const int nt = (n + 63) >> 6, maxt = (maxn + 63) >> 6;
@@ -224,6 +224,7 @@
         }
         return acc;
     }
+    const bool fill = act && nt > 1 && nt <= 16;
     QTile buf[QT];
 #pragma unroll
     for (int d = 0; d < QT; ++d) buf[d] = tile_load(ln, d < nt ? d : 0, rl);
@@ -235,8 +236,10 @@
             buf[d] = tile_load(ln, t + QT < nt ? t + QT : 0, rl);
             const double tEt = t < nt ? tEz : 0.0;
             acc = row_sum64(tEt * (double)c.c0, tEt * (double)c.c1, tEt * (double)c.c2, tEt * (double)c.c3, acc);
-        }
-    }
+            if (fill && rl == t) tc = acc;
+        }
+    }
+    if (act) tc_pi = fill ? pi : tc_pi == pi ? -1 : tc_pi;
     return acc;
 }
 
@@ -345,7 +348,7 @@
             s_ts[pq] = ok ? (double)gI64[PI_TOTSUS * P + pq] : 0.0;
             s_ti[pq] = ok ? (double)gI64[PI_TOTINF * P + pq] : 0.0;
             s_nocc[pq] = ok ? gN[pq] : 0;
-            s_zero[pq] = 0;
+            s_zero[pq] = QT < 4 && ok ? gN[pq] : 0;
         }
     }
     WSYNC();
@@ -397,11 +400,13 @@
     double g_val = 0.0;
     int pos = 8;
     int32_t ch_cn[4] = {0, 0, 0, 0};
+    double tc = 0.0;
+    int tc_pi = -1;
 
 #ifdef VGX_PROFILE
     unsigned long long prof_acc[VGX_PROF_SLOTS], prof_t0 = __builtin_readcyclecounter();
     for (int i = 0; i < VGX_PROF_SLOTS; ++i) prof_acc[i] = 0;
-    int prof_tiles[7] = {0, 0, 0, 0, 0, 0, 0};
+    int prof_tiles[10] = {0, 0, 0, 0, 0, 0, 0, 0, 0, 0};
 #endif
     while (true) {
         QPROF(0);
@@ -512,7 +517,6 @@
             const double tE = ((bC + c_d) + smul) + c_tm;
             const int n_sel = evn ? s_nocc[pi] : 0;
             const int32_t *lh = lhap + (int64_t)pi * cap;
-            int64_t *ln = lcnt + (int64_t)pi * cap;
             int32_t *l3 = lcnt32 + (int64_t)pi * cap;
             int64_t *lt = ltsum + (int64_t)pi * capT;
             {
@@ -589,8 +593,16 @@
 #ifdef VGX_PROFILE
                 prof_acc[15] += 1;
 #endif
+#ifdef VGX_PROFILE
+                if (QT < 4) {
+                    const bool hit_ = n_sel > 64 && tc_pi == pi, miss_ = n_sel > 64 && tc_pi != pi;
+                    prof_tiles[7] += hit_; prof_tiles[8] += miss_;
+                    if (!__ballot(miss_) && row == 0) prof_tiles[9] += 1;
+                }
+#endif
                 QSel sel;
-                q_long_select<QT>(l3, lh, n_sel, maxn, tE, r2, evn, H, sel, (double *)(ltsum + (int64_t)pi * capT + R * P * capT))   ;
+                q_long_select<QT>(l3, lh, n_sel, maxn, tE, r2, evn, H, sel, (double *)(ltsum + (int64_t)pi * capT + R * P * capT) ,
+                                  pi, tc, tc_pi);
                 k_hit = sel.k_hit; pre_hit = sel.pre_hit; w_hit = sel.w_hit; hap_hit = sel.hap_hit; cnt_hit = sel.cnt_hit;
                 if (sel.err) err = sel.err;
 #ifdef VGX_PROFILE
@@ -622,7 +634,7 @@
                 if (ts_pi * c_sig == 0.0) err = Q_ERR_ZERO_WEIGHT + 256 * 6;
                 if (rl == 0) { s_ts[pi] = ts_pi - 1.0; s_ti[pi] = ti_pi + 1.0; }
                 gI += 1.0; QBUMP(QC_B);
-                if (live && rl == 0) { if (QT < 4) ln[k_hit] = cnt_hit + 1; l3[k_hit] = (int32_t)(cnt_hit + 1); if (QT >= 4) L8(pi)[k_hit] = B8(cnt_hit + 1); if (n_sel > 64) lt[k_hit >> 6] += 1; }
+                if (live && rl == 0) { l3[k_hit] = (int32_t)(cnt_hit + 1); if (QT >= 4) { L8(pi)[k_hit] = B8(cnt_hit + 1); if (n_sel > 64) lt[k_hit >> 6] += 1; } }
 #pragma unroll
                 for (int c = 0; c < 4; ++c)
                     if (c == (k_hit >> 4) && rl == (k_hit & 15)) ch_cn[c] += 1;
@@ -635,7 +647,7 @@
                 if (ei == 2) { cS += 1; e_type = QEV_SAMPLING; } else { QBUMP(QC_D); e_type = QEV_DEATH; }
                 if (QT < 4 && cnt_hit == 1) { op_n = 1; op_pi = pi; op_h0 = hap_hit; op_d0 = -1; ch_pi = -1; }
                 else {
-                    if (live && rl == 0) { if (QT < 4) ln[k_hit] = cnt_hit - 1; l3[k_hit] = (int32_t)(cnt_hit - 1); if (QT >= 4) L8(pi)[k_hit] = B8(cnt_hit - 1); if (n_sel > 64) lt[k_hit >> 6] -= 1; }
+                    if (live && rl == 0) { l3[k_hit] = (int32_t)(cnt_hit - 1); if (QT >= 4) { L8(pi)[k_hit] = B8(cnt_hit - 1); if (n_sel > 64) lt[k_hit >> 6] -= 1; } }
                     if (QT >= 4 && cnt_hit == 1 && rl == 0) s_zero[pi] += 1;
 #pragma unroll
                     for (int c = 0; c < 4; ++c)
@@ -731,9 +743,8 @@
                 {
                     const int n = evm ? s_nocc[spi] : 0;
                     const int32_t *lh2 = lhap + (int64_t)spi * cap;
-                    const int64_t *ln2 = lcnt + (int64_t)spi * cap;
                     const int32_t *l32 = lcnt32 + (int64_t)spi * cap;
-#define CN2(k) (QT >= 4 ? (int64_t)l32[k] : ln2[k])
+#define CN2(k) ((int64_t)l32[k])
                     const int64_t *lt2 = ltsum + (int64_t)spi * capT;
                     const double rr_ = s_ti[spi] * rm;
                     int64_t before = 0;
@@ -745,6 +756,16 @@
                         const int maxt = rows_max(nt);
                         int jt = -1;
                         int64_t carry = 0;
+                        if (QT < 4) {
+                            for (int t = 0; t < maxt; ++t) {
+                                const QTile c = tile_load(l32, t < nt ? t : 0, rl);
+                                const int64_t w = t < nt ? (int64_t)c.c0 + (int64_t)c.c1 + (int64_t)c.c2 + (int64_t)c.c3 : 0;
+                                const int64_t pre = rowget_i64(row_iscan(w), 15) + carry;
+                                if (jt < 0 && t < nt && !((double)pre < rr_)) { jt = t; before = carry; }
+                                carry = pre;
+                                if (!__ballot(jt < 0 && t + 1 < nt)) break;
+                            }
+                        } else
                         for (int tb = 0; tb < maxt; tb += 16) {
                             const int j = tb + rl;
                             const int64_t w = j < nt ? lt2[j] : 0;
@@ -853,12 +874,10 @@
             const int n = act ? s_nocc[op_pi] : 0;
             int32_t *lh = lhap + (int64_t)op_pi * cap;
             int32_t *lc = lcls + (int64_t)op_pi * cap;
-            int64_t *ln = lcnt + (int64_t)op_pi * cap;
             int32_t *l3 = lcnt32 + (int64_t)op_pi * cap;
-            int64_t *lt = ltsum + (int64_t)op_pi * capT;
             int posn = 0;
             bool found = false;
-            int64_t cur = 0;
+            int32_t cur = 0;
             {
                 int lo = 0;
                 const int maxn = rows_max(n);
@@ -877,36 +896,14 @@
                         lo = lo + (nle > 0 ? (nle - 1) * stride : 0);
                     }
                 }
-                if (act && found) cur = ln[posn];
+                if (act && found) cur = l3[posn];
             }
             const bool bump = act && found && cur + delta != 0;
             const bool rem = act && found && cur + delta == 0;
             const bool ins = act && !found;
             if (ins && n >= cap) { err = Q_ERR_CAPACITY; }
             const bool ins_ok = ins && err == 0;
-            if (bump && rl == 0) { ln[posn] = cur + delta; l3[posn] = (int32_t)(cur + delta); if (QT >= 4) L8(op_pi)[posn] = B8(cur + delta); if (n > 64) lt[posn >> 6] += delta; }
-            if (__builtin_expect(__ballot((ins_ok || rem) && n > 64) != 0, 0)) {
-                const bool tt = (ins_ok || rem) && n > 64;
-                const int jp = posn >> 6, jl = ins_ok ? (n >> 6) : ((n - 1) >> 6);
-                const int maxj = rows_max(tt ? jl + 1 : 0);
-                for (int tb = 0; tb < maxj; tb += 16) {
-                    const int j = tb + rl;
-                    if (tt && j >= jp && j <= jl) {
-                        int64_t in_, out_;
-                        if (ins_ok) {
-                            in_ = j == jp ? (int64_t)delta : ln[(int64_t)j * 64 - 1];
-                            const int kout = j * 64 + 63;
-                            out_ = kout < n ? ln[kout] : 0;
-                        } else {
-                            out_ = j == jp ? ln[posn] : ln[(int64_t)j * 64];
-                            const int kin = j * 64 + 64;
-                            in_ = kin < n ? ln[kin] : 0;
-                        }
-                        lt[j] += in_ - out_;
-                    }
-                }
-                WSYNC();
-            }
+            if (bump && rl == 0) l3[posn] = cur + delta;
             if (__builtin_expect(__ballot(ins_ok) != 0, 0)) {
                 enum { SU = 4 };
                 int hi_ = ins_ok ? n : 0;
@@ -914,30 +911,24 @@
                 while (__ballot(hi_ > lo_)) {
                     const int blo = max(lo_, hi_ - SU * 16);
                     int h[SU];
-                    int64_t ct[SU];
+                    int32_t ct[SU];
 #pragma unroll
                     for (int u = 0; u < SU; ++u) {
                         const int k = blo + u * 16 + rl;
                         h[u] = 0; ct[u] = 0;
-                        if (k < hi_) { h[u] = lh[k]; ct[u] = ln[k]; }
+                        if (k < hi_) { h[u] = lh[k]; ct[u] = l3[k]; }
                     }
                     WSYNC();
 #pragma unroll
                     for (int u = 0; u < SU; ++u) {
                         const int k = blo + u * 16 + rl;
-                        if (k < hi_) { lh[k + 1] = h[u]; lc[k + 1] = 0; ln[k + 1] = ct[u]; l3[k + 1] = (int32_t)ct[u]; if (QT >= 4) L8(op_pi)[k + 1] = B8(ct[u]); }
+                        if (k < hi_) { lh[k + 1] = h[u]; lc[k + 1] = 0; l3[k + 1] = ct[u]; }
                     }
                     WSYNC();
                     hi_ = blo;
                 }
-                if (ins_ok && rl == 0) { lh[posn] = hap; lc[posn] = 0; ln[posn] = delta; l3[posn] = delta; if (QT >= 4) L8(op_pi)[posn] = B8(delta); s_nocc[op_pi] = n + 1; }
-                q_zero_tail(l3, n + 1, cap, QT < 4 && ins_ok && ((n + 1) & 63) == 0);
-                WSYNC();
-                if (ins_ok && n == 64) {
-                    int64_t s0 = 0;
-                    for (int c4 = 0; c4 < 4; ++c4) s0 += rowget_i64(row_iscan(ln[c4 * 16 + rl]), 15);
-                    if (rl == 0) { lt[0] = s0; lt[1] = ln[64]; }
-                }
+                if (ins_ok && rl == 0) { lh[posn] = hap; lc[posn] = 0; l3[posn] = delta; s_nocc[op_pi] = n + 1; if (n + 1 > s_zero[op_pi]) s_zero[op_pi] = n + 1; }
+                q_zero_tail(l3, n + 1, cap, ins_ok && ((n + 1) & 63) == 0);
                 WSYNC();
             }
             if (__builtin_expect(__ballot(rem) != 0, 0)) {
@@ -946,23 +937,23 @@
                 const int hi_ = rem ? n : 0;
                 while (__ballot(lo_ < hi_)) {
                     int h[SU];
-                    int64_t ct[SU];
+                    int32_t ct[SU];
 #pragma unroll
                     for (int u = 0; u < SU; ++u) {
                         const int k = lo_ + u * 16 + rl;
                         h[u] = 0; ct[u] = 0;
-                        if (k < hi_) { h[u] = lh[k]; ct[u] = ln[k]; }
+                        if (k < hi_) { h[u] = lh[k]; ct[u] = l3[k]; }
                     }
                     WSYNC();
 #pragma unroll
                     for (int u = 0; u < SU; ++u) {
                         const int k = lo_ + u * 16 + rl;
-                        if (k < hi_) { lh[k - 1] = h[u]; ln[k - 1] = ct[u]; l3[k - 1] = (int32_t)ct[u]; if (QT >= 4) L8(op_pi)[k - 1] = B8(ct[u]); }
+                        if (k < hi_) { lh[k - 1] = h[u]; l3[k - 1] = ct[u]; }
                     }
                     WSYNC();
                     lo_ += SU * 16;
                 }
-                if (rem && rl == 0) { s_nocc[op_pi] = n - 1; if (QT < 4) l3[n - 1] = 0; }
+                if (rem && rl == 0) { s_nocc[op_pi] = n - 1; l3[n - 1] = 0; }
                 WSYNC();
             }
         }
@@ -1023,6 +1014,7 @@
                 if (__builtin_expect(maxn <= 64, QT < 4)) {
                     const int nch = (maxn + 15) >> 4;
                     const bool chave = act && pi == ch_pi;
+                    if (QT < 4 && act && pi == tc_pi) tc_pi = -1;
                     const double tEz = n > 0 ? tE : 0.0;
                     int32_t cn4[4];
 #pragma unroll
@@ -1040,7 +1032,7 @@
 #ifdef VGX_PROFILE
                     prof_tiles[4] += (n + 63) >> 6; prof_tiles[5] += (maxn + 63) >> 6; prof_tiles[6] += 1;
 #endif
-                    acc = q_long_sum<QT>(l3, L8(pi), n, maxn, tE, (double *)(ltsum + (int64_t)pi * capT + R * P * capT));
+                    acc = q_long_sum<QT>(l3, L8(pi), n, maxn, tE, (double *)(ltsum + (int64_t)pi * capT + R * P * capT), act, pi, tc, tc_pi);
                 }
                 if (act && rl == 0) { s_bc[pi] = bC; s_inf[pi] = acc; }
                 WSYNC();
@@ -1093,6 +1085,7 @@
                 t_now = 0.0; traj_next = 0;
                 restarts += 1; att += 1;
                 st = ST_REBUILD;
+                tc_pi = -1;
             } else {
                 good_attempt = (int64_t)att + 1;
                 st = ST_DONE;
@@ -1115,7 +1108,7 @@
                             if (rs) {
                                 lhap[(int64_t)pn * cap + k] = r.i_hap[(int64_t)pn * r.i_cap + k];
                                 lcls[(int64_t)pn * cap + k] = r.i_cls[(int64_t)pn * r.i_cap + k];
-                                lcnt[(int64_t)pn * cap + k] = ct;
+                                if (QT >= 4) lcnt[(int64_t)pn * cap + k] = ct;
                                 lcnt32[(int64_t)pn * cap + k] = (int32_t)ct;
                                 if (QT >= 4) L8(pn)[k] = B8(ct);
                             }
@@ -1128,7 +1121,7 @@
                 if (rs)
                     for (int j = (n + 63) / 64 + rl; j <= n_old / 64 && j < capT; j += 16) ltsum[(int64_t)pn * capT + j] = 0;
                 if (QT < 4) q_zero_tail(lcnt32 + (int64_t)pn * cap, n, cap, rs);
-                if (rs && rl == 0) { s_nocc[pn] = n; s_zero[pn] = 0; s_ts[pn] = (double)r.i_sus[pn]; s_ti[pn] = (double)ti; }
+                if (rs && rl == 0) { s_nocc[pn] = n; if (QT >= 4) s_zero[pn] = 0; else if (n > s_zero[pn]) s_zero[pn] = n; s_ts[pn] = (double)r.i_sus[pn]; s_ti[pn] = (double)ti; }
                 g += ti;
             }
             if (rs) gI = (double)g;
@@ -1154,7 +1147,7 @@
 #ifdef VGX_PROFILE
     if (lane == 0 && r.prof)
         for (int i = 0; i < VGX_PROF_SLOTS; ++i) r.prof[rep * VGX_PROF_SLOTS + i] = prof_acc[i];
-    for (int i = 0; i < 7; ++i) {
+    for (int i = 0; i < 10; ++i) {
         const long long t4 = (long long)__builtin_amdgcn_readlane(prof_tiles[i], 0) + __builtin_amdgcn_readlane(prof_tiles[i], 16) +
                              __builtin_amdgcn_readlane(prof_tiles[i], 32) + __builtin_amdgcn_readlane(prof_tiles[i], 48);
         if (lane == 0 && r.prof && rep_raw + 1 < R) r.prof[(rep_raw + 1) * VGX_PROF_SLOTS + i] = (unsigned long long)t4;
@@ -1162,6 +1155,23 @@
 #endif
     stage_flush(stage_n > 0);
     WSYNC();
+    if (QT < 4) {
+        for (int pn = 0; pn < P; ++pn) {
+            const int n = live ? s_nocc[pn] : 0, top = live ? s_zero[pn] : 0;
+            const int32_t *l3 = lcnt32 + (int64_t)pn * cap;
+            const int jmax = rows_max(top >> 6);
+            for (int j = 0; j <= jmax && j < capT; ++j) {
+                int64_t w = 0;
+#pragma unroll
+                for (int i = 0; i < 4; ++i) {
+                    const int k = j * 64 + 4 * rl + i;
+                    if (k < n) w += (int64_t)l3[k];
+                }
+                const int64_t tsum = rowget_i64(row_iscan(w), 15);
+                if (live && rl == 0 && j <= (top >> 6)) ltsum[(int64_t)pn * capT + j] = tsum;
+            }
+        }
+    }
     if (live) {
         double *gD = r.popD + rep * PD_COUNT * P;
         int64_t *gI64 = r.popI + rep * PI_COUNT * P;
@@ -1290,3 +1300,66 @@
     (void)hipFree(d);
     return rc;
 }
+
+extern "C" __global__ void __launch_bounds__(64) vgx_quad_tilechoice_kernel(const int32_t *cnt, const int32_t *hap, const int32_t *n,
+                                                                           const double *tE, const double *r, int64_t rows, int64_t stride,
+                                                                           int H, int32_t *k_hit, double *pre_hit, double *w_hit, int64_t *cnt_hit) {
+    const int wrow = threadIdx.x >> 4;
+    const int64_t row_raw = (int64_t)blockIdx.x * 4 + wrow;
+    const int64_t row = row_raw < rows ? row_raw : rows - 1;
+    const int32_t *l3 = cnt + row * stride, *lh = hap + row * stride;
+    const int nn = n[row], maxn = rows_max(nn), pi = 1 + wrow;
+    const double te = tE[row], rr = r[row];
+    double tc = 0.0;
+    int tc_pi = -1;
+    (void)q_long_sum<1>(l3, nullptr, nn, maxn, te, nullptr, true, pi, tc, tc_pi);
+    const bool act2 = (wrow & 1) == 0;
+    const int n2 = act2 ? nn : 0;
+    (void)q_long_sum<1>(l3, nullptr, n2, rows_max(n2), te, nullptr, act2, act2 ? pi : 0, tc, tc_pi);
+    QSel a, b;
+    q_long_select<1>(l3, lh, nn, maxn, te, rr, true, H, a, nullptr, pi, tc, tc_pi);
+    q_long_select<1>(l3, lh, nn, maxn, te, rr, true, H, b, nullptr, pi, tc, -1);
+    if (row_raw < rows && (threadIdx.x & 15) == 0) {
+        k_hit[row] = a.k_hit; pre_hit[row] = a.pre_hit; w_hit[row] = a.w_hit; cnt_hit[row] = a.cnt_hit;
+        k_hit[rows + row] = b.k_hit; pre_hit[rows + row] = b.pre_hit; w_hit[rows + row] = b.w_hit; cnt_hit[rows + row] = b.cnt_hit;
+    }
+}
+extern "C" int vgx_test_quad_tile_choice(const int32_t *counts, const int32_t *haps, const int32_t *n, const double *tE, const double *r,
+                                         int64_t rows, int64_t maxlen, int H, int32_t *k_hit, double *pre_hit, double *w_hit, int64_t *cnt_hit) {
+    if (!counts || !haps || !n || !tE || !r || !k_hit || !pre_hit || !w_hit || !cnt_hit || rows < 0 || maxlen < 1 || maxlen > (1 << 20)) return 1;
+    if (rows == 0) return 0;
+    for (int64_t i = 0; i < rows; ++i)
+        if (n[i] < 0 || n[i] > maxlen) return 1;
+    const size_t nr = (size_t)rows;
+    const int64_t stride = (maxlen + 63) / 64 * 64 + 64;
+    std::vector<int32_t> hc(nr * (size_t)stride, 0), hh(nr * (size_t)stride, 0);
+    for (size_t i = 0; i < nr; ++i)
+        for (int64_t k = 0; k < n[i]; ++k) {
+            hc[i * (size_t)stride + (size_t)k] = counts[i * (size_t)maxlen + (size_t)k];
+            hh[i * (size_t)stride + (size_t)k] = haps[i * (size_t)maxlen + (size_t)k];
+        }
+    const size_t lb = nr * (size_t)stride * 4;
+    char *d = nullptr;
+    if (hipMalloc((void **)&d, 2 * lb + nr * (8 + 8 + 8 + 16 + 16 + 16 + 8)) != hipSuccess) return 2;
+    int32_t *dc = (int32_t *)d, *dh = (int32_t *)(d + lb);
+    double *dte = (double *)(d + 2 * lb), *dr = dte + nr, *dpre = dr + nr, *dw = dpre + 2 * nr;
+    int64_t *dcnt = (int64_t *)(dw + 2 * nr);
+    int32_t *dn = (int32_t *)(dcnt + 2 * nr), *dk = dn + nr + (nr & 1);
+    int rc = 0;
+    if (hipMemcpy(dc, hc.data(), lb, hipMemcpyHostToDevice) != hipSuccess || hipMemcpy(dh, hh.data(), lb, hipMemcpyHostToDevice) != hipSuccess ||
+        hipMemcpy(dte, tE, nr * 8, hipMemcpyHostToDevice) != hipSuccess || hipMemcpy(dr, r, nr * 8, hipMemcpyHostToDevice) != hipSuccess ||
+        hipMemcpy(dn, n, nr * 4, hipMemcpyHostToDevice) != hipSuccess)
+        rc = 2;
+    if (!rc) {
+        hipLaunchKernelGGL(vgx_quad_tilechoice_kernel, dim3((unsigned)((rows + 3) / 4)), dim3(64), 0, nullptr, dc, dh, dn, dte, dr, rows, stride, H,
+                           dk, dpre, dw, dcnt);
+        if (hipGetLastError() != hipSuccess || hipDeviceSynchronize() != hipSuccess ||
+            hipMemcpy(k_hit, dk, 2 * nr * 4, hipMemcpyDeviceToHost) != hipSuccess ||
+            hipMemcpy(pre_hit, dpre, 2 * nr * 8, hipMemcpyDeviceToHost) != hipSuccess ||
+            hipMemcpy(w_hit, dw, 2 * nr * 8, hipMemcpyDeviceToHost) != hipSuccess ||
+            hipMemcpy(cnt_hit, dcnt, 2 * nr * 8, hipMemcpyDeviceToHost) != hipSuccess)
+            rc = 2;
+    }
+    (void)hipFree(d);
+    return rc;
+}
```
